# 10XGenomics/thermite

Hardware: AMD Instinct MI355X
Metric: aligned reads/sec (91 bp) (higher is better)
Workload: dtype i32

## Files before the change

### thermite_amd/csrc/aligner.hip

```cpp
#include <hip/hip_runtime.h>

#include <algorithm>
#include <cstdarg>
#include <cstdio>
#include <cstdlib>
#include <cstring>
#include <mutex>
#include <string>
#include <type_traits>
#include <vector>

#include "aligner_internal.h"

namespace thm {
const char* global_error_cstr();
}
using namespace thm;

static int swg_blocks_per_cu() {
  static const int v = [] {
    const char* e = getenv("THM_SWG_BPC");
    const int v = e ? atoi(e) : 4;
    return (v >= 1 && v <= 8) ? v : 4;
  }();
// ... 17 lines not shown
    auto* d = new thm_index::DevCopy();
    d->device = a->device;
    hipStream_t s = a->stream;
    hipError_t e = hipSuccess;
    auto up = [&](auto& buf, const auto& vec) {
      if (e == hipSuccess) e = upload(buf, vec, s);
    };
    d->wide = ix->wide;
    if (e == hipSuccess) e = d->text.ensure(ix->text.size() + 16 + 16);
    if (e == hipSuccess) e = hipMemsetAsync(d->text.p, '$', 16, s);
    if (e == hipSuccess && !ix->text.empty())
      e = hipMemcpyAsync(d->text.as<uint8_t>() + 16, ix->text.data(), ix->text.size(), hipMemcpyHostToDevice, s);
    if (ix->wide) {
      up(d->sa, ix->sa64);
      up(d->lut, ix->lut64);
    } else {
      up(d->sa, ix->sa);
      up(d->lut, ix->lut);
    }
    up(d->refs, ix->refs);
    up(d->name_rank, ix->name_rank);
    up(d->txs, ix->txs);
    up(d->exons, ix->exons);
    up(d->exon_txoff, ix->exon_txoff);
    if (e == hipSuccess) e = d->tx_seq.ensure(ix->tx_seq.size() + 32);
    if (e == hipSuccess) e = hipMemsetAsync(d->tx_seq.p, '$', 16, s);
    if (e == hipSuccess && !ix->tx_seq.empty())
      e = hipMemcpyAsync(d->tx_seq.as<uint8_t>() + 16, ix->tx_seq.data(), ix->tx_seq.size(), hipMemcpyHostToDevice, s);
    up(d->exon_grid_off, ix->exon_grid_off);
    up(d->gene_grid_off, ix->gene_grid_off);
    up(d->ref_bin, ix->ref_bin);
    if (ix->wide)
      up(d->ref_recs, ix->ref_recs64);
    else
      up(d->ref_recs, ix->ref_recs);
    if (ix->wide) {
      up(d->exon_grid, ix->exon_grid64);
      up(d->gene_grid, ix->gene_grid64);
    } else {
      up(d->exon_grid, ix->exon_grid);
      up(d->gene_grid, ix->gene_grid);
    }
    if (e == hipSuccess) e = hipStreamSynchronize(s);
    if (e != hipSuccess) {
      free_dev_copy(d);
      return fail(a, e == hipErrorOutOfMemory ? THM_ERR_OOM : THM_ERR_HIP, "index upload failed: %s",
                  hipGetErrorString(e));
    }
    auto fill_view = [&](auto& v) {
      typedef typename std::remove_reference<decltype(v)>::type::coord_t C;
      v.text = d->text.as<uint8_t>() + 16;
      v.sa = d->sa.as<C>();
      v.lut = d->lut.as<LutEntryT<C>>();
      v.refs = d->refs.as<thm_ref>();
      v.name_rank = d->name_rank.as<uint32_t>();
      v.ref_recs = d->ref_recs.as<RefRecT<C>>();
      v.ref_bin = d->ref_bin.as<uint32_t>();
      v.txs = d->txs.as<thm_tx>();
      v.exons = d->exons.as<thm_exon>();
      v.exon_txoff = d->exon_txoff.as<uint64_t>();
      v.tx_seq = d->tx_seq.as<uint8_t>() + 16;
      v.exon_grid_off = d->exon_grid_off.as<uint32_t>();
      v.exon_grid = d->exon_grid.as<ExonEntryT<C>>();
      v.gene_grid_off = d->gene_grid_off.as<uint32_t>();
      v.gene_grid = d->gene_grid.as<GridEntryT<C>>();
      v.n = ix->n;
      v.n_refs = (uint32_t)ix->refs.size();
      v.n_txs = (uint32_t)ix->txs.size();
      v.kt = ix->kt;
      v.max_tx_exons = ix->max_tx_exons;
    };
    memset(&d->view, 0, sizeof d->view);
    memset(&d->view64, 0, sizeof d->view64);
    if (ix->wide)
      fill_view(d->view64);
    else
      fill_view(d->view);
    ix->dev[a->device] = d;
  }
  a->dix = ix->dev[a->device];
  return THM_OK;
}

int reset_queue(thm_aligner* a) {
  HIPCHK(a, hipMemsetAsync(a->d_queue.p, 0, thm::QUEUE_BYTES, a->stream));
  HIPCHK(a, hipMemsetAsync(a->d_fault.p, 0, 64, a->stream));
  return THM_OK;
}

int grid_blocks(const thm_aligner* a, uint64_t n_items, int waves_per_block, int blocks_per_cu) {
  uint64_t need = (n_items + waves_per_block - 1) / waves_per_block;
  uint64_t cap = (uint64_t)a->n_cu * blocks_per_cu;
  return (int)std::max<uint64_t>(1, std::min(need, cap));
}

extern "C" {

const char* thm_version(void) { return "thermite_amd 0.1 (gfx950)"; }

int32_t thm_device_count(void) {
  int n = 0;
  if (hipGetDeviceCount(&n) != hipSuccess) return 0;
  return n;
}

void thm_index_free(thm_index* ix) {
  if (!ix) return;
  for (auto* d : ix->dev) free_dev_copy(d);
  delete (std::mutex*)ix->dev_mu;
  delete ix;
}

const char* thm_last_error(const thm_aligner* a) { return a ? a->err.c_str() : global_error_cstr(); }

int32_t thm_aligner_create(const thm_index* ix, const thm_align_opts* opts, int32_t device_id, thm_aligner** out) {
  if (!out) return THM_ERR_INVALID_ARG;
  *out = nullptr;
  if (!ix || !opts) return fail(nullptr, THM_ERR_INVALID_ARG, "thm_aligner_create: null index or opts");
  int n = 0;
  if (hipGetDeviceCount(&n) != hipSuccess || n <= 0)
    return fail(nullptr, THM_ERR_NO_DEVICE, "no HIP device visible: the MI355X path has no CPU fallback");
  if (device_id < 0 || device_id >= n) return fail(nullptr, THM_ERR_NO_DEVICE, "device id %d out of range", device_id);
  thm_aligner* a = new thm_aligner();
  a->ix = ix;
  a->device = device_id;
  a->opts = *opts;
  {
    const char* e = getenv("THM_TPR");
    if (e && e[0] == '0') a->use_tpr = false;
    if (e && e[0] == '1') a->use_tpr = true;
    e = getenv("THM_TPR_ROUNDS");
    if (e && atoi(e) >= 1 && atoi(e) <= TPR_MAX_ROUNDS) a->tpr_rounds = atoi(e);
  }
  auto bail = [&](int code) {
    thm_aligner_free(a);
    return code;
  };
  if (hipSetDevice(device_id) != hipSuccess) return bail(fail(nullptr, THM_ERR_HIP, "hipSetDevice failed"));
  hipDeviceProp_t prop;
  if (hipGetDeviceProperties(&prop, device_id) == hipSuccess) a->n_cu = prop.multiProcessorCount;
  if (hipStreamCreateWithFlags(&a->stream, hipStreamNonBlocking) != hipSuccess)
    return bail(fail(nullptr, THM_ERR_HIP, "hipStreamCreate failed"));
  for (auto& e : a->ev)
    if (hipEventCreate(&e) != hipSuccess) return bail(fail(nullptr, THM_ERR_HIP, "hipEventCreate failed"));
  if (hipStreamCreateWithFlags(&a->stream2, hipStreamNonBlocking) != hipSuccess ||
      hipStreamCreateWithFlags(&a->stream3, hipStreamNonBlocking) != hipSuccess ||
      hipStreamCreateWithFlags(&a->stream4, hipStreamNonBlocking) != hipSuccess ||
      hipEventCreateWithFlags(&a->ev_dpt_fork, hipEventDisableTiming) != hipSuccess ||
      hipEventCreateWithFlags(&a->ev_dpt_join, hipEventDisableTiming) != hipSuccess ||
      hipEventCreateWithFlags(&a->ev_join3, hipEventDisableTiming) != hipSuccess ||
      hipEventCreateWithFlags(&a->ev_fork, hipEventDisableTiming) != hipSuccess ||
      hipEventCreateWithFlags(&a->ev_join, hipEventDisableTiming) != hipSuccess)
    return bail(fail(nullptr, THM_ERR_HIP, "second stream / events: creation failed"));
  if (a->d_counters.ensure(THM_N_COUNTERS * 8 * 3) != hipSuccess || a->d_queue.ensure(thm::QUEUE_BYTES) != hipSuccess ||
      a->d_fault.ensure(64) != hipSuccess || a->d_cursors.ensure(64) != hipSuccess)
    return bail(fail(nullptr, THM_ERR_OOM, "scratch allocation failed"));
  (void)hipMemsetAsync(a->d_counters.p, 0, THM_N_COUNTERS * 8 * 3, a->stream);
  int rc = get_dev_copy(a);
  if (rc != THM_OK) return bail(rc);
  rc = thm_aligner_set_opts(a, opts);
  if (rc != THM_OK) return bail(rc);
  *out = a;
  return THM_OK;
}

void thm_aligner_free(thm_aligner* a) {
  if (!a) return;
  (void)hipSetDevice(a->device);
  if (a->stream) (void)hipStreamSynchronize(a->stream);
  if (a->stream2) (void)hipStreamSynchronize(a->stream2);
  if (a->stream3) (void)hipStreamSynchronize(a->stream3);
  if (a->stream4) (void)hipStreamSynchronize(a->stream4);
  DBuf* all[] = {&a->d_counters, &a->d_queue, &a->d_fault, &a->d_cursors, &a->b0, &a->b1, &a->b2, &a->b3, &a->b4,
                 &a->b5, &a->b6, &a->b7, &a->b8, &a->r_bases, &a->r_offsets, &a->r_san, &a->s_ms_end, &a->s_ms_lo, &a->s_ms_hi, &a->s_work_reads, &a->s_work_long, &a->s_work_cells, &a->s_work_counts, &a->s_fill_keys, &a->s_fill_perm, &a->s_fill_hist, &a->s_sel_scratch, &a->s_heavy, &a->s_slow, &a->s_team, &a->r_status, &a->e_slow, &a->e_recs, &a->e_wcnt, &a->t_memos, &a->t_recs, &a->t_dpops, &a->t_qlist, &a->t_act[0], &a->t_act[1], &a->t_ctl, &a->t_bail, &a->t_queue2, &a->t_trace, &a->t_ttrace, &a->t_hdr, &a->t_sums, &a->s_smems, &a->s_off, &a->s_cnt,
                 &a->s_hits, &a->s_cand_off, &a->scan_tmp, &a->e_cands, &a->e_heavy, &a->e_rel, &a->e_order, &a->e_ops, &a->e_nalns,
                 &a->e_nalns64, &a->e_opbytes, &a->e_aln_off, &a->e_ops_off, &a->e_trace, &a->o_alns, &a->o_ops, &a->o_mems,
                 &a->sh_bases, &a->sh_san, &a->sh_off, &a->sh_hits, &a->sh_read, &a->sh_bw, &a->sh_xd, &a->sh_list, &a->sh_out,
                 &a->sh_status, &a->sh_ops, &a->sh_ctl, &a->sh_trace, &a->sh_slow, &a->c_sums, &a->c_nwords, &a->c_woff,
                 &a->c_scan_tmp, &a->c_flags, &a->c_dig, &a->c_words, &a->c_in_ops, &a->c_in_off,
                 &a->bn_names, &a->bn_name_off, &a->bn_quals, &a->bt_tx_pool, &a->bt_tx_off, &a->bt_gid_pool, &a->bt_gid_off,
                 &a->bt_gname_pool, &a->bt_gname_off, &a->bt_tx_gene, &a->bt_ref_sq, &a->bm_cnt, &a->bm_first, &a->bm_qn,
                 &a->bm_rec_read, &a->bm_len, &a->bm_off, &a->bm_out, &a->bm_read_off, &a->bm_err, &a->bm_scan_tmp};
  for (DBuf* b : all) b->release();
  for (int k = 0; k < 2; k++) {
    a->r_off[k].release();
    a->r_alns[k].release();
    a->r_ops[k].release();
    a->r_stat[k].release();
    a->ch_off[k].release();
    a->ch_alns[k].release();
    a->ch_dig[k].release();
    a->ch_words[k].release();
    a->ch_stat[k].release();
    a->bh_data[k].release();
    a->bh_off[k].release();
    a->bh_stat[k].release();
  }
  for (auto& e : a->ev_cig)
    if (e) (void)hipEventDestroy(e);
  for (auto& e : a->ev_bam)
    if (e) (void)hipEventDestroy(e);
  for (auto& e : a->ev)
    if (e) (void)hipEventDestroy(e);
  if (a->ev_fork) (void)hipEventDestroy(a->ev_fork);
  if (a->ev_join) (void)hipEventDestroy(a->ev_join);
  if (a->ev_join3) (void)hipEventDestroy(a->ev_join3);
  if (a->ev_dpt_fork) (void)hipEventDestroy(a->ev_dpt_fork);
  if (a->ev_dpt_join) (void)hipEventDestroy(a->ev_dpt_join);
  if (a->stream4) (void)hipStreamDestroy(a->stream4);
  if (a->stream3) (void)hipStreamDestroy(a->stream3);
  if (a->stream2) (void)hipStreamDestroy(a->stream2);
  if (a->stream) (void)hipStreamDestroy(a->stream);
  delete a;
}

int32_t thm_aligner_set_opts(thm_aligner* a, const thm_align_opts* o) {
  if (!a || !o) return THM_ERR_INVALID_ARG;
  if (o->min_seed_len < 1 || o->min_seed_len > 65535) return fail(a, THM_ERR_INVALID_ARG, "min_seed_len out of range");
  if (!(o->min_aln_score_percent >= 0.0f && o->min_aln_score_percent <= 1.0f))
    return fail(a, THM_ERR_INVALID_ARG, "min_aln_score_percent must be within [0,1] (src/main.rs:46-49)");
  a->opts = *o;
  return THM_OK;
}

void* thm_aligner_stream(thm_aligner* a) { return a ? (void*)a->stream : nullptr; }

const thm_index* thm_aligner_index(const thm_aligner* a) { return a ? a->ix : nullptr; }

int32_t thm_counters_get(thm_aligner* a, uint64_t out[THM_N_COUNTERS]) {
  if (!a || !out) return THM_ERR_INVALID_ARG;
  HIPCHK(a, hipSetDevice(a->device));
  HIPCHK(a, hipMemcpyAsync(out, a->d_counters.p, THM_N_COUNTERS * 8, hipMemcpyDeviceToHost, a->stream));
  HIPCHK(a, hipStreamSynchronize(a->stream));
  return THM_OK;
}
int32_t thm_counters_reset(thm_aligner* a) {
  if (!a) return THM_ERR_INVALID_ARG;
  HIPCHK(a, hipSetDevice(a->device));
  HIPCHK(a, hipMemsetAsync(a->d_counters.p, 0, THM_N_COUNTERS * 8, a->stream));
  return THM_OK;
}
void* thm_counters_device_ptr(thm_aligner* a) { return a ? a->d_counters.p : nullptr; }

int32_t thm_timings_get(thm_aligner* a, float out[THM_N_TIMINGS]) {
  if (!a || !out) return THM_ERR_INVALID_ARG;
  memcpy(out, a->timings, sizeof(a->timings));
  return THM_OK;
}

int32_t thm_swg_extend_batch(thm_aligner* a, const uint8_t* x_bases, const uint64_t* x_off, const uint8_t* y_bases,
                             const uint64_t* y_off, const uint32_t* band_width, const int32_t* x_drop,
                             uint32_t max_band_width, uint64_t n, thm_swg_view* out) {
  if (!a || !out || !x_off || !y_off || !band_width || !x_drop) return THM_ERR_INVALID_ARG;
  memset(out, 0, sizeof(*out));
  if (n == 0) return THM_OK;
  if (n >= 0xFFFFFFFFull) return fail(a, THM_ERR_UNSUPPORTED, "more than 2^32-1 problems in one call");
  HIPCHK(a, hipSetDevice(a->device));
  uint32_t bw_max = 0, x_max = 0, y_max = 0;
  std::vector<uint64_t> ops_off(n + 1, 0);
  for (uint64_t i = 0; i < n; i++) {
    if (band_width[i] > max_band_width)
      return fail(a, THM_ERR_OUT_OF_CONTRACT, "problem %llu: band_width %u > max_band_width %u (src/swg.rs:32)",
                  (unsigned long long)i, band_width[i], max_band_width);
    if (x_drop[i] < (int64_t)band_width[i])
      return fail(a, THM_ERR_OUT_OF_CONTRACT, "problem %llu: x_drop < band_width is undefined in the reference",
                  (unsigned long long)i);
    uint64_t xl = x_off[i + 1] - x_off[i], yl = y_off[i + 1] - y_off[i];
    if (x_off[i + 1] < x_off[i] || y_off[i + 1] < y_off[i]) return fail(a, THM_ERR_INVALID_ARG, "offsets not monotone");
    if (xl > MAX_READ_LEN || band_width[i] > 2 * MAX_READ_LEN)
      return fail(a, THM_ERR_UNSUPPORTED, "x longer than %u or band wider than +-%u", MAX_READ_LEN, 2 * MAX_READ_LEN);
    uint64_t cols = std::min<uint64_t>(yl, xl + band_width[i] + 1);
    bw_max = std::max(bw_max, band_width[i]);
    x_max = std::max<uint32_t>(x_max, (uint32_t)xl);
    y_max = std::max<uint32_t>(y_max, (uint32_t)cols);
    ops_off[i + 1] = ops_off[i] + xl + cols + 8;
  }
  int cpl = (int)((2 * bw_max + 1 + 63) / 64);
  SwgBatchParams p;
  p.x_cap = (x_max + 15u) & ~15u;
  p.y_cap = (y_max + 15u) & ~15u;
  if (p.x_cap == 0) p.x_cap = 16;
  if (p.y_cap == 0) p.y_cap = 16;
  p.max_bw = bw_max;
  p.scratch = nullptr;
  p.scratch_per_wave = 0;
  if (cpl > 4 || swg_batch_lds_bytes(p, cpl) > EXTEND_LDS_LIMIT) cpl = 0;
  const uint64_t xb_n = x_off[n], yb_n = y_off[n], pool = ops_off[n];
  HIPCHK(a, a->b0.ensure(xb_n + 16));
  HIPCHK(a, a->b1.ensure((n + 1) * 8));
  HIPCHK(a, a->b2.ensure(yb_n + 16));
  HIPCHK(a, a->b3.ensure((n + 1) * 8));
  HIPCHK(a, a->b4.ensure(n * 4));
  HIPCHK(a, a->b5.ensure(n * 4));
  HIPCHK(a, a->b6.ensure((n + 1) * 8));
  HIPCHK(a, a->b7.ensure(pool + 16));
  HIPCHK(a, a->b8.ensure(n * sizeof(thm_swg_aln)));
  hipStream_t s = a->stream;
  if (xb_n) HIPCHK(a, hipMemcpyAsync(a->b0.p, x_bases, xb_n, hipMemcpyHostToDevice, s));
  HIPCHK(a, hipMemcpyAsync(a->b1.p, x_off, (n + 1) * 8, hipMemcpyHostToDevice, s));
  if (yb_n) HIPCHK(a, hipMemcpyAsync(a->b2.p, y_bases, yb_n, hipMemcpyHostToDevice, s));
  HIPCHK(a, hipMemcpyAsync(a->b3.p, y_off, (n + 1) * 8, hipMemcpyHostToDevice, s));
  HIPCHK(a, hipMemcpyAsync(a->b4.p, band_width, n * 4, hipMemcpyHostToDevice, s));
  HIPCHK(a, hipMemcpyAsync(a->b5.p, x_drop, n * 4, hipMemcpyHostToDevice, s));
  HIPCHK(a, hipMemcpyAsync(a->b6.p, ops_off.data(), (n + 1) * 8, hipMemcpyHostToDevice, s));
  int rc = reset_queue(a);
  if (rc != THM_OK) return rc;
  p.xb = a->b0.as<uint8_t>();
  p.xo = a->b1.as<uint64_t>();
  p.yb = a->b2.as<uint8_t>();
  p.yo = a->b3.as<uint64_t>();
  p.bw = a->b4.as<uint32_t>();
  p.xd = a->b5.as<int32_t>();
  p.ops_off = a->b6.as<uint64_t>();
  p.ops = a->b7.as<uint8_t>();
  p.out = a->b8.as<thm_swg_aln>();
  p.counters = a->d_counters.as<unsigned long long>();
  p.queue = a->d_queue.as<unsigned int>();
  p.fault = a->d_fault.as<int>();
  p.n = n;
  const int bpc = swg_blocks_per_cu();
  int n_blocks = grid_blocks(a, n, 4, bpc);
  if (cpl == 0) {
    p.scratch_per_wave = (swg_batch_scratch_bytes(p) + 255) & ~255ull;
    const uint64_t budget = 16ull << 30;
    if (p.scratch_per_wave > budget) return fail(a, THM_ERR_UNSUPPORTED, "DP trace of %llu bytes per problem exceeds the device-memory budget",
                                                 (unsigned long long)p.scratch_per_wave);
    n_blocks = (int)std::max<uint64_t>(1, std::min<uint64_t>((uint64_t)n_blocks, budget / p.scratch_per_wave / 4));
    HIPCHK(a, a->e_slow.ensure((size_t)n_blocks * 4 * p.scratch_per_wave + 256));
    p.scratch = a->e_slow.as<uint8_t>();
// ... 245 lines not shown
```

### thermite_amd/csrc/aligner_internal.h

```cpp
#ifndef THERMITE_ALIGNER_INTERNAL_H
#define THERMITE_ALIGNER_INTERNAL_H
#include <hip/hip_runtime.h>

#include <cstdarg>
#include <cstdio>
#include <string>
#include <vector>

#include "launch.h"
#include "thermite_internal.h"

struct DBuf {
  void* p = nullptr;
  size_t cap = 0;
  hipError_t ensure(size_t bytes) {
    if (bytes <= cap) return hipSuccess;
    if (p) (void)hipFree(p);
    p = nullptr;
    cap = 0;
    size_t want = bytes + bytes / 4 + 256;
    hipError_t e = hipMalloc(&p, want);
    if (e == hipSuccess) cap = want;
    return e;
  }
  void release() {
    if (p) (void)hipFree(p);
    p = nullptr;
    cap = 0;
  }
  template <class T>
  T* as() const {
    return (T*)p;
  }
};

struct HBuf {
  void* p = nullptr;
  size_t cap = 0;
  hipError_t ensure(size_t bytes) {
    if (bytes <= cap) return hipSuccess;
    if (p) (void)hipHostFree(p);
    p = nullptr;
    cap = 0;
    size_t want = bytes + bytes / 4 + 4096;
    hipError_t e = hipHostMalloc(&p, want, hipHostMallocDefault);
    if (e == hipSuccess) cap = want;
    return e;
  }
  void release() {
    if (p) (void)hipHostFree(p);
    p = nullptr;
    cap = 0;
  }
  template <class T>
  T* as() const {
    return (T*)p;
  }
};

struct thm_index::DevCopy {
  int device = -1;
  DBuf text, sa, lut, refs, name_rank, ref_recs, ref_bin, txs, exons, exon_txoff, tx_seq, exon_grid_off, exon_grid, gene_grid_off, gene_grid;
  bool wide = false;
  thm::DeviceIndexT<uint32_t> view;
  thm::DeviceIndexT<uint64_t> view64;
};

inline void free_dev_copy(thm_index::DevCopy* d) {
  if (!d) return;
  int cur = 0;
  (void)hipGetDevice(&cur);
  (void)hipSetDevice(d->device);
  DBuf* all[] = {&d->text, &d->sa,         &d->lut,    &d->refs,      &d->name_rank, &d->ref_recs, &d->ref_bin, &d->txs,
                 &d->exons, &d->exon_txoff, &d->tx_seq, &d->exon_grid_off, &d->exon_grid, &d->gene_grid_off, &d->gene_grid};
  for (DBuf* b : all) b->release();
  (void)hipSetDevice(cur);
  delete d;
}

struct thm_aligner {
  const thm_index* ix = nullptr;
  thm_index::DevCopy* dix = nullptr;
  int device = 0;
  int n_cu = 256;
  hipStream_t stream = nullptr;
  hipStream_t stream2 = nullptr;
  hipStream_t stream3 = nullptr;
  hipEvent_t ev_join3 = nullptr;
  hipStream_t stream4 = nullptr;
  hipEvent_t ev_dpt_fork = nullptr, ev_dpt_join = nullptr;
  hipEvent_t ev_fork = nullptr, ev_join = nullptr;
  thm_align_opts opts;
  std::string err;

  DBuf d_counters, d_queue, d_fault, d_cursors;
  DBuf b0, b1, b2, b3, b4, b5, b6, b7, b8;

  DBuf r_bases, r_offsets, r_san;
  DBuf r_status;
  uint64_t n_reads = 0, n_bases = 0;
  uint32_t max_read_len = 0;
  std::vector<std::pair<uint32_t, uint64_t>> len_hist;
  uint64_t n_over = 0;
  bool uploaded = false;
  DBuf s_smems, s_off, s_cnt, s_hits, s_cand_off, scan_tmp, s_ms_end, s_ms_lo, s_ms_hi, s_work_reads, s_work_long, s_work_cells,
      s_work_counts, s_sel_scratch, s_heavy, s_slow, s_team, s_fill_keys, s_fill_perm, s_fill_hist;
  uint64_t smem_cap = 0;
  DBuf e_heavy, e_rel;
  DBuf e_cands, e_order, e_ops, e_nalns, e_nalns64, e_opbytes, e_aln_off, e_ops_off, e_trace, e_slow, e_recs, e_wcnt;
  DBuf t_memos, t_recs, t_dpops, t_qlist, t_act[2], t_ctl, t_bail, t_queue2, t_trace, t_ttrace, t_hdr, t_sums;
  bool use_tpr = false;
  int tpr_rounds = 8;
  uint64_t n_slow_host = 0;
  uint32_t fast_max_len = 0, slow_max_len = 0;
  uint64_t cand_cap = 0, cand_ops_cap = 0;
  DBuf o_alns, o_ops, o_mems;
  uint64_t out_alns_cap = 0, out_ops_cap = 0;
  uint64_t dbg_smem_cap = 0, dbg_cand_cap = 0, dbg_ops_cap = 0;
  uint32_t dbg_band_clip = 0;
  bool dbg_seed_noinfer = false, dbg_seed_stats = false;
  uint32_t n_replays = 0;
  bool ran = false, synced = false;
  hipEvent_t ev[6] = {nullptr, nullptr, nullptr, nullptr, nullptr, nullptr};
  float timings[THM_N_TIMINGS] = {0};

  HBuf r_off[2], r_alns[2], r_ops[2], r_stat[2];
  int r_cur = 0;
  std::vector<uint64_t> h_off;
  std::vector<thm_aln> h_alns;
  std::vector<uint8_t> h_ops;
  std::vector<thm_mem> h_mems;
  std::vector<thm_swg_aln> h_swg;
  std::vector<thm_lr_aln> h_lr;
  DBuf sh_bases, sh_san, sh_off, sh_hits, sh_read, sh_bw, sh_xd, sh_list, sh_out, sh_status, sh_ops, sh_ctl, sh_trace, sh_slow;
  std::vector<thm_aln> h_hit_alns;
  std::vector<int32_t> h_hit_status;
  std::vector<uint8_t> h_hit_ops;
  DBuf c_sums, c_nwords, c_woff, c_scan_tmp, c_flags, c_dig, c_words, c_in_ops, c_in_off;
  HBuf ch_off[2], ch_alns[2], ch_dig[2], ch_words[2], ch_stat[2];
  int c_cur = 0;
  hipEvent_t ev_cig[4] = {nullptr, nullptr, nullptr, nullptr};
  std::vector<thm_aln_digest> h_cig_dig;
  std::vector<uint32_t> h_cig_words;
  DBuf bn_names, bn_name_off, bn_quals;
  bool reads_named = false, reads_have_quals = false;
  DBuf bt_tx_pool, bt_tx_off, bt_gid_pool, bt_gid_off, bt_gname_pool, bt_gname_off, bt_tx_gene, bt_ref_sq;
  bool bam_tables = false;
  DBuf bm_cnt, bm_first, bm_qn, bm_rec_read, bm_len, bm_off, bm_out, bm_read_off, bm_err, bm_scan_tmp;
  HBuf bh_data[2], bh_off[2], bh_stat[2];
  int b_cur = 0;
  int bam_stage = -1;
  hipEvent_t ev_bam[4] = {nullptr, nullptr, nullptr, nullptr};
};

inline int fail(thm_aligner* a, int code, const char* fmt, ...) {
  char buf[512];
  va_list ap;
  va_start(ap, fmt);
  vsnprintf(buf, sizeof buf, fmt, ap);
  va_end(ap);
  if (a) a->err = buf;
  thm::set_global_error(buf);
  return code;
}

#define HIPCHK(a, call)                                                                             \
  do {                                                                                              \
    hipError_t e_ = (call);                                                                         \
    if (e_ != hipSuccess)                                                                           \
      return fail(a, e_ == hipErrorOutOfMemory ? THM_ERR_OOM : THM_ERR_HIP, "%s failed: %s (%s:%d)", \
                  #call, hipGetErrorString(e_), __FILE__, __LINE__);                                \
  } while (0)

int run_cigar_passes(thm_aligner* a, thm::CigarParams p, uint64_t n_digests, uint64_t* n_words, unsigned* any_flags);
int cigar_ensure_events(thm_aligner* a);
int reset_queue(thm_aligner* a);
int grid_blocks(const thm_aligner* a, uint64_t n_items, int waves_per_block, int blocks_per_cu);
uint32_t seed_fill_mode();
unsigned team_div_per_cu();
#endif
```

### thermite_amd/csrc/kernels_extend.hip

```cpp
#include <hip/hip_runtime.h>

#include <cstdlib>

#include "launch.h"
#include "swg_device.h"

namespace thm {
namespace dev {

enum : int { FAULT_OPS_POOL = 1, FAULT_INTERNAL = 2, FAULT_CONTRACT = 4, FAULT_RETRY = 8, FAULT_BAND = 16 };

template <class C>
struct CoordTraits {
  typedef int S;
};
template <>
struct CoordTraits<uint64_t> {
  typedef long long S;
};
__device__ __forceinline__ uint32_t readlane_c(uint32_t v, int l) { return (uint32_t)__builtin_amdgcn_readlane((int)v, l); }
__device__ __forceinline__ uint64_t readlane_c(uint64_t v, int l) {
  return ((uint64_t)(unsigned)__builtin_amdgcn_readlane((int)(v >> 32), l) << 32) | (unsigned)__builtin_amdgcn_readlane((int)(v & 0xffffffffu), l);
}

// ... 1413 lines not shown
              less = b.ystart < a.ystart;
            else
              less = u < t;
            rank += less ? 1u : 0u;
          }
          lb[rank] = la[t];
        }
      }
      step();
      if (lead) {
      uint64_t max_end = 0;
      uint32_t l_rank = 0, l_strand = 0;
      int l_score = 0;
      uint64_t l_yend = 0;
      for (uint32_t s = 0; s < m; s++) {
        const uint32_t ci = (uint32_t)bcast_first((int)lb[s]);
        const Cand a = cands[ci];
        if (nres == 0 || a.ystart >= max_end || a.name_rank != l_rank || a.strand != l_strand) {
          max_end = a.yend;
          if (lane == 0) la[nres] = ci;
          nres++;
          l_rank = a.name_rank;
          l_strand = a.strand;
          l_score = a.score;
          l_yend = a.yend;
        } else {
          if (a.score > l_score) {
            if (lane == 0) la[nres - 1] = ci;
            l_score = a.score;
            l_yend = a.yend;
          }
          max_end = max(max_end, l_yend);
        }
      }
      if (TM && lane == 0) t_ctl[1] = nres;
      }
      step();
      if constexpr (TM) nres = t_ctl[1];
      #pragma unroll 1
      for (uint32_t t0 = t0_first; t0 < nres; t0 += t0_step) {
        const uint32_t t = t0 + lane;
        if (t < nres) {
          const int sa_ = cands[la[t]].score;
          uint32_t rank = 0;
          for (uint32_t u = 0; u < nres; u++) {
            const int sb = cands[la[u]].score;
            rank += (sb > sa_ || (sb == sa_ && u < t)) ? 1u : 0u;
          }
          lb[rank] = la[t];
        }
      }
      step();
      #pragma unroll 1
      for (uint32_t t = t0_first + lane; t < nres; t += t0_step) la[t] = lb[t];
      step();
    }
      #pragma unroll 1
      for (uint32_t t0 = 0; lead && t0 < nres; t0 += 64) {
        const uint32_t t = t0 + (uint32_t)lane;
        int ty = -1;
        if (t < nres) {
          const Cand a = cands[la[t]];
          opb += a.ops_len + a.tx_ops_len;
          ty = a.aln_type;
        }
        k_type[0] += (unsigned)__popcll(__ballot(ty == THM_ALN_EXONIC));
        k_type[1] += (unsigned)__popcll(__ballot(ty == THM_ALN_INTRONIC));
        k_type[2] += (unsigned)__popcll(__ballot(ty == THM_ALN_INTERGENIC));
      }
      for (int o = 32; o > 0; o >>= 1) opb += __shfl_xor(opb, o);
    }
#ifdef THM_PROF_FINAL
    const unsigned long long tf2 = __builtin_amdgcn_s_memtime();
#endif
    if (lead && lane == 0) {
      p.read_n_alns[idx] = nres;
      p.read_op_bytes[idx] = opb;
    }
#ifdef THM_PROF_FINAL
    {
      const unsigned long long tf3 = __builtin_amdgcn_s_memtime();
      c.prof_cols[3] += tf1 - tf0;
      c.prof_cols[4] += tf2 - tf1;
      c.prof_cols[5] += tf3 - tf2;
      c.prof_cols[1] += (n_acc > 1) ? 1 : 0;
      c.prof_cols[2] += 1;
    }
#endif
    PROF_MARK(c, PS_FINAL);
    if (lead) {
      k_reads++;
      if (nres)
        k_aligned++;
      else
        k_unmapped++;
      k_alns += nres;
      k_opb += opb;
    }
    k_cells += c.cells;
    k_cols += c.cols;
    k_calls += c.calls;
    k_win += c.winbytes;
    c.cells = c.cols = c.calls = c.winbytes = 0;
    wsync(c);
  }
#ifdef THM_TIMELINE
  if (!TM && !GS && lane == 0 && p.prof && tl_reads) {
    const unsigned long long tl_end = __builtin_amdgcn_s_memrealtime();
    atomicMax(&p.prof[0], ~tl_start);
    atomicMax(&p.prof[1], ~tl_end);
    atomicMax(&p.prof[2], tl_end);
    atomicMax(&p.prof[3], (tl_end << 20) | min((tl_end - tl_last) / 100ull, 1048575ull));
    tl_close(tl_end);
    atomicMax(&p.prof[4], tl_longest);
    atomicAdd(&p.prof[5], 1ull);
    atomicAdd(&p.prof[6], tl_end - tl_start);
    atomicAdd(&p.prof[7], (unsigned long long)tl_reads);
    if (p.list_only == 0) {
      const unsigned long long t0 = ~atomicMax(&p.prof[0], 0ull);
      const unsigned long long rel = (tl_end - t0) / 10000ull;
      const int b = rel < 30 ? 0 : (int)min(rel - 29ull, 7ull);
      atomicAdd(&p.prof[8 + b], 1ull);
    }
  }
#endif
#ifdef THM_PROF
  if (lane == 0 && p.prof)
    {
      for (int t = 0; t < 10; t++) atomicAdd(&p.prof[t], c.prof_acc[t]);
      for (int t = 0; t < 6; t++) atomicAdd(&p.prof[10 + t], c.prof_cols[t]);
    }
#endif
  batch_fault |= c.fault & (FAULT_OPS_POOL | FAULT_INTERNAL);
  if (lane == 0) {
    if (batch_fault) atomicOr(p.fault, batch_fault & (FAULT_OPS_POOL | FAULT_INTERNAL));
    if (k_reads | k_calls | k_cells | k_win) {
      unsigned long long* row = p.wave_counters + (size_t)wave_global * THM_N_COUNTERS;
      row[THM_CNT_READS] = k_reads;
      row[THM_CNT_ALIGNED] = k_aligned;
      row[THM_CNT_UNMAPPED] = k_unmapped;
      row[THM_CNT_ALNS] = k_alns;
      row[THM_CNT_EXONIC] = (unsigned long long)k_type[0];
      row[THM_CNT_INTRONIC] = (unsigned long long)k_type[1];
      row[THM_CNT_INTERGENIC] = (unsigned long long)k_type[2];
      row[THM_CNT_SWG_CALLS] = k_calls;
      row[THM_CNT_DP_CELLS] = k_cells;
      row[THM_CNT_DP_COLS] = k_cols;
      row[THM_CNT_OP_BYTES] = k_opb;
      row[THM_CNT_WINDOW_BYTES] = k_win;
    }
  }
}

__global__ __launch_bounds__(1024) void counters_reduce_kernel(const unsigned long long* rows, uint32_t n_rows, unsigned long long* counters) {
  __shared__ unsigned long long part[64][THM_N_COUNTERS];
  static_assert(THM_N_COUNTERS == 16, "one thread per counter and row group");
  const int k = (int)(threadIdx.x & 15u), g = (int)(threadIdx.x >> 4);
  unsigned long long sum = 0;
  for (uint32_t r = (uint32_t)g; r < n_rows; r += 64) sum += rows[(size_t)r * THM_N_COUNTERS + k];
  part[g][k] = sum;
  __syncthreads();
  if (g == 0) {
    unsigned long long t = 0;
    for (int i = 0; i < 64; i++) t += part[i][k];
    if (t) counters[k] += t;
  }
}

constexpr uint32_t COMPACT_HEAVY_N = 8, COMPACT_CHUNK = 4;

struct CandRegs {
  uint32_t lo, hi;
};
static_assert(sizeof(Cand) == 112 && sizeof(thm_aln) == 112, "compact_emit permutes the dwords of these layouts");
static_assert(offsetof(Cand, ops_off) == 48 && offsetof(Cand, tx_ops_off) == 56 && offsetof(Cand, score) == 64 &&
                  offsetof(Cand, ops_len) == 80 && offsetof(Cand, tx_ops_len) == 84 && offsetof(Cand, strand) == 108 &&
                  offsetof(thm_aln, ops_off) == 24 && offsetof(thm_aln, tx_ops_off) == 56 && offsetof(thm_aln, xlen) == 80 &&
                  offsetof(thm_aln, ops_len) == 84 && offsetof(thm_aln, tx_ops_len) == 104 && offsetof(thm_aln, strand) == 108,
              "compact_emit permutes the dwords of these layouts");

__device__ __forceinline__ CandRegs cand_load(const Cand* c, int sub) {
  const uint32_t* w = reinterpret_cast<const uint32_t*>(c);
  CandRegs r;
  r.lo = w[sub];
  r.hi = sub < 12 ? w[16 + sub] : 0u;
  return r;
}

__device__ __forceinline__ uint32_t compact_emit(const CompactParams& p, const CandRegs c, uint64_t ai, uint64_t o, uint32_t xlen, bool primary, int sub) {
  const uint64_t ops_off = (uint64_t)__shfl(c.lo, 12, 16) | ((uint64_t)__shfl(c.lo, 13, 16) << 32);
  const uint64_t tx_ops_off = (uint64_t)__shfl(c.lo, 14, 16) | ((uint64_t)__shfl(c.lo, 15, 16) << 32);
  const uint32_t ops_len = __shfl(c.hi, 4, 16), tx_ops_len = __shfl(c.hi, 5, 16), flags = __shfl(c.hi, 11, 16);
  if (ai >= p.alns_cap || o + ops_len + tx_ops_len > p.ops_cap) return ops_len + tx_ops_len;
  auto copy_ops = [&](const uint8_t* src, uint8_t* dst, uint32_t len) {
    #pragma unroll 1
    for (uint32_t b0 = 0; b0 < len; b0 += 64) {
      uint8_t v[4];
      #pragma unroll
      for (int k = 0; k < 4; k++) {
        const uint32_t b = b0 + (uint32_t)sub + 16u * (uint32_t)k;
        v[k] = (b < len) ? src[b] : (uint8_t)0;
      }
      #pragma unroll
      for (int k = 0; k < 4; k++) {
        const uint32_t b = b0 + (uint32_t)sub + 16u * (uint32_t)k;
        if (b < len) dst[b] = v[k];
      }
    }
  };
  copy_ops(p.cand_ops + ops_off, p.ops + o, ops_len);
  const uint64_t go = o, to = o + ops_len;
  copy_ops(p.cand_ops + tx_ops_off, p.ops + to, tx_ops_len);
  const int src_lo = (int)((0x00BA987600543210ull >> (4 * sub)) & 15u);
  const int src_hi = (int)((0x0000B59876403210ull >> (4 * sub)) & 15u);
  uint32_t w0 = __shfl(c.lo, src_lo, 16), w1 = __shfl(c.hi, src_hi, 16);
  const uint64_t txo = ((flags >> 8) & 0xFFu) == THM_ALN_EXONIC ? to : 0ull;
  if (sub == 6) w0 = (uint32_t)go;
  if (sub == 7) w0 = (uint32_t)(go >> 32);
  if (sub == 14) w0 = (uint32_t)txo;
  if (sub == 15) w0 = (uint32_t)(txo >> 32);
  if (sub == 4) w1 = xlen;
  if (sub == 11) w1 = (flags & 0xFFu) | ((primary ? 1u : 0u) << 8) | (((flags >> 8) & 0xFFu) << 16);
  uint32_t* out = reinterpret_cast<uint32_t*>(p.alns + ai);
  out[sub] = w0;
  if (sub < 12) out[16 + sub] = w1;
  return ops_len + tx_ops_len;
}

__device__ __forceinline__ bool compact_faulted(const CompactParams& p) { return p.fault[0] != 0 || (p.fault[1] & FAULT_OPS_POOL) != 0; }

template <int K>
__global__ __launch_bounds__(256) void compact_kernel(CompactParams p) {
  const int sub = (int)(threadIdx.x & 15u);
  if (compact_faulted(p)) return;
  const uint64_t n_groups = (uint64_t)gridDim.x * 16, g = ((uint64_t)blockIdx.x * 256 + threadIdx.x) >> 4;
  for (uint64_t rb = g; rb < p.n_reads; rb += (uint64_t)K * n_groups) {
    uint32_t n[K], xlen[K], l0[K];
    uint64_t cand0[K], a0[K], o[K];
    #pragma unroll
    for (int k = 0; k < K; k++) {
      const uint64_t r = rb + (uint64_t)k * n_groups;
      n[k] = r < p.n_reads ? p.read_n_alns[r] : 0u;
    }
    #pragma unroll
    for (int k = 0; k < K; k++) {
      const uint64_t r = rb + (uint64_t)k * n_groups;
      if (n[k] > COMPACT_HEAVY_N) {
        if (sub == 0) {
          const unsigned long long h = atomicAdd(&p.heavy_cnt[0], 1ull);
          if (h < p.heavy_cap) p.heavy_list[h] = r;
        }
        n[k] = 0;
      }
      if (n[k]) {
        cand0[k] = p.read_cand_off[r];
        a0[k] = p.read_aln_off[r];
        o[k] = p.read_ops_off[r];
        xlen[k] = (uint32_t)(p.read_offsets[r + 1] - p.read_offsets[r]);
      }
    }
    #pragma unroll
    for (int k = 0; k < K; k++)
      if (n[k]) l0[k] = p.order[2 * cand0[k]];
    CandRegs cd[K];
    #pragma unroll
    for (int k = 0; k < K; k++)
      if (n[k]) cd[k] = cand_load(p.cands + cand0[k] + l0[k], sub);
    #pragma unroll
    for (int k = 0; k < K; k++) {
      if (!n[k]) continue;
      uint64_t ok = o[k] + compact_emit(p, cd[k], a0[k], o[k], xlen[k], true, sub);
      const uint32_t* la = p.order + 2 * cand0[k];
      for (uint32_t t = 1; t < n[k]; t++)
        ok += compact_emit(p, cand_load(p.cands + cand0[k] + la[t], sub), a0[k] + t, ok, xlen[k], false, sub);
    }
  }
}

__global__ __launch_bounds__(256) void compact_heavy_scan_kernel(CompactParams p) {
  __shared__ uint32_t wave_sum[4];
  __shared__ unsigned long long desc_base;
  if (compact_faulted(p)) return;
  const uint64_t H = min((unsigned long long)p.heavy_cap, p.heavy_cnt[0]);
  const int tid = (int)threadIdx.x, lane = tid & 63, wv = tid >> 6;
  for (uint64_t h = blockIdx.x; h < H; h += gridDim.x) {
    const uint64_t r = p.heavy_list[h];
    const uint32_t n = p.read_n_alns[r];
    const uint64_t cand0 = p.read_cand_off[r], a0 = p.read_aln_off[r];
    const Cand* cands = p.cands + cand0;
    const uint32_t* la = p.order + 2 * cand0;
    uint32_t carry = 0;
    for (uint32_t tile = 0; tile < n; tile += 256) {
      const uint32_t t = tile + (uint32_t)tid;
      uint32_t len = 0;
      if (t < n) {
        const Cand* cd = &cands[la[t]];
        len = cd->ops_len + cd->tx_ops_len;
      }
      uint32_t inc = len;
      #pragma unroll
      for (int o = 1; o < 64; o <<= 1) {
        const uint32_t v = __shfl_up(inc, o);
        if (lane >= o) inc += v;
      }
      if (lane == 63) wave_sum[wv] = inc;
      __syncthreads();
      uint32_t before = carry, total = 0;
      #pragma unroll
      for (int k = 0; k < 4; k++) {
        if (k < wv) before += wave_sum[k];
        total += wave_sum[k];
      }
      if (t < n && a0 + t < p.alns_cap) p.rel[a0 + t] = before + inc - len;
      carry += total;
      __syncthreads();
    }
    const uint32_t nd = (n + COMPACT_CHUNK - 1) / COMPACT_CHUNK;
    if (tid == 0) desc_base = atomicAdd(&p.heavy_cnt[1], (unsigned long long)nd);
// ... 324 lines not shown
      atomicAdd(&p.counters[THM_CNT_SWG_CALLS], k_calls);
      atomicAdd(&p.counters[THM_CNT_DP_CELLS], k_cells);
      atomicAdd(&p.counters[THM_CNT_DP_COLS], k_cols);
      atomicAdd(&p.counters[THM_CNT_OP_BYTES], k_opb);
      atomicAdd(&p.counters[THM_CNT_WINDOW_BYTES], k_win);
    }
  }
}

}

template <class C>
static hipError_t launch_seed_hits_t(const SeedHitParamsT<C>& p, int cpl, int n_blocks, hipStream_t s) {
  const size_t lds = cpl == 0 ? 0 : extend_lds_bytes(p.max_read_len, p.max_bw, cpl);
  auto go = [&](auto kern) -> hipError_t {
    if (lds > 48 * 1024) {
      hipError_t e = hipFuncSetAttribute((const void*)kern, hipFuncAttributeMaxDynamicSharedMemorySize, (int)lds);
      if (e != hipSuccess) return e;
    }
    hipLaunchKernelGGL(kern, dim3(n_blocks), dim3(256), lds, s, p);
    return hipGetLastError();
  };
  switch (cpl) {
    case 0: return go(dev::seed_hit_kernel<C, 0>);
    case 1: return go(dev::seed_hit_kernel<C, 1>);
    case 2: return go(dev::seed_hit_kernel<C, 2>);
    case 3: return go(dev::seed_hit_kernel<C, 3>);
    case 4: return go(dev::seed_hit_kernel<C, 4>);
    default: return hipErrorInvalidValue;
  }
}
hipError_t launch_seed_hits(const SeedHitParamsT<uint32_t>& p, int cpl, int n_blocks, hipStream_t s) { return launch_seed_hits_t(p, cpl, n_blocks, s); }
hipError_t launch_seed_hits(const SeedHitParamsT<uint64_t>& p, int cpl, int n_blocks, hipStream_t s) { return launch_seed_hits_t(p, cpl, n_blocks, s); }

size_t extend_lds_bytes(uint32_t max_read_len, uint32_t max_bw, int cpl) {
  const dev::ExtCaps k = dev::ext_caps(max_read_len, max_bw, cpl);
  const uint32_t per_wave = k.lcap + 2u * k.wcap + k.trb + 3u * k.opcap + 8u * FAST_MAX_YCLIPS + (uint32_t)(dev::KEYCAP * sizeof(dev::CandKey));
  return 4 * (size_t)per_wave;
}

size_t extend_trace_scratch_bytes(uint32_t max_read_len, uint32_t max_bw, int cpl) {
  return cpl > 1 ? (size_t)(max_read_len + max_bw + 3u) * (size_t)cpl * 16u : 0;
}

size_t extend_slow_scratch_bytes(uint32_t max_read_len, uint32_t max_bw, uint32_t mk_cap) {
  return (size_t)dev::slow_layout(max_read_len, max_bw, mk_cap).total;
}

constexpr int EXT_MINW_CPL34 = 4;
static int ext_minw_env() {
  static const int v = [] {
    const char* e = getenv("THM_EXT_MINW");
    const int v = e ? atoi(e) : 0;
    return (v >= 4 && v <= 8) ? v : 0;
  }();
  return v;
}
static int ext_minw_cpl3_env() {
  static const int v = [] {
    const char* e = getenv("THM_EXT_MINW_CPL3");
    const int v = e ? atoi(e) : 0;
    return (v >= 3 && v <= 6) ? v : 0;
  }();
  return v;
}
static int ext_minw_wide_env() {
  static const int v = [] {
    const char* e = getenv("THM_EXT_MINW_WIDE");
    const int v = e ? atoi(e) : 0;
    return (v == 4 || v == 5) ? v : 0;
  }();
  return v;
}
int extend_waves_per_simd(int cpl, bool wide) {
  const int minw_env = ext_minw_env();
  if (cpl == 0) return 2;
  if (cpl > 2) {
    const int v34 = ext_minw_cpl3_env();
    return (v34 && !wide) ? v34 : EXT_MINW_CPL34;
  }
  if (wide) {
    const int wide_env = ext_minw_wide_env();
    return wide_env ? wide_env : 5;
  }
  if (minw_env) {
    if (cpl == 1) return (minw_env == 4 || minw_env == 5 || minw_env == 6) ? minw_env : 8;
    return (minw_env == 4 || minw_env == 5 || minw_env == 8) ? minw_env : 6;
  }
  return cpl == 1 ? 6 : 5;
}

template <class C>
static hipError_t launch_extend_t(const ExtendParamsT<C>& p, int cpl, int n_blocks, hipStream_t s, bool team) {
  const size_t lds4 = cpl == 0 ? 0 : extend_lds_bytes(p.max_read_len, p.max_bw, cpl);
  const size_t lds = team ? lds4 / 4 * TEAM_WAVES : lds4;
  const unsigned threads = team ? 64u * TEAM_WAVES : 256u;
  auto go = [&](auto kern) -> hipError_t {
    if (lds > 48 * 1024) {
      hipError_t e = hipFuncSetAttribute((const void*)kern, hipFuncAttributeMaxDynamicSharedMemorySize, (int)lds);
      if (e != hipSuccess) return e;
    }
    hipLaunchKernelGGL(kern, dim3(n_blocks), dim3(threads), lds, s, p);
    return hipGetLastError();
  };
  if (team) {
    if (cpl == 1) return go(dev::extend_kernel<C, 1, 4, TEAM_WAVES>);
    if (cpl == 2) return go(dev::extend_kernel<C, 2, 4, TEAM_WAVES>);
    return hipErrorInvalidValue;
  }
  if (cpl == 0) return go(dev::extend_kernel<C, 0, 2>);
  if constexpr (sizeof(C) == 8) {
    const int minw = extend_waves_per_simd(cpl, true);
    switch (cpl) {
      case 1: return minw == 5 ? go(dev::extend_kernel<C, 1, 5>) : go(dev::extend_kernel<C, 1, 4>);
      case 2: return minw == 5 ? go(dev::extend_kernel<C, 2, 5>) : go(dev::extend_kernel<C, 2, 4>);
      case 3: return go(dev::extend_kernel<C, 3, 4>);
      case 4: return go(dev::extend_kernel<C, 4, 4>);
      default: return hipErrorInvalidValue;
    }
  } else {
    const int minw = extend_waves_per_simd(cpl, false);
    switch (cpl) {
      case 1:
        if (minw == 4) return go(dev::extend_kernel<C, 1, 4>);
        if (minw == 5) return go(dev::extend_kernel<C, 1, 5>);
        if (minw == 6) return go(dev::extend_kernel<C, 1, 6>);
        return go(dev::extend_kernel<C, 1, 8>);
      case 2:
        if (minw == 4) return go(dev::extend_kernel<C, 2, 4>);
        if (minw == 5) return go(dev::extend_kernel<C, 2, 5>);
        if (minw == 8) return go(dev::extend_kernel<C, 2, 8>);
        return go(dev::extend_kernel<C, 2, 6>);
      case 3:
      case 4: {
        const int minw = extend_waves_per_simd(cpl, false);
        if (cpl == 3) {
          if (minw == 3) return go(dev::extend_kernel<C, 3, 3>);
          if (minw == 5) return go(dev::extend_kernel<C, 3, 5>);
          if (minw == 6) return go(dev::extend_kernel<C, 3, 6>);
          return go(dev::extend_kernel<C, 3, 4>);
        }
        if (minw == 3) return go(dev::extend_kernel<C, 4, 3>);
        if (minw == 5) return go(dev::extend_kernel<C, 4, 5>);
        if (minw == 6) return go(dev::extend_kernel<C, 4, 6>);
        return go(dev::extend_kernel<C, 4, 4>);
      }
      default: return hipErrorInvalidValue;
    }
  }
}
hipError_t launch_extend(const ExtendParamsT<uint32_t>& p, int cpl, int n_blocks, hipStream_t s, bool team) { return launch_extend_t(p, cpl, n_blocks, s, team); }
hipError_t launch_extend(const ExtendParamsT<uint64_t>& p, int cpl, int n_blocks, hipStream_t s, bool team) { return launch_extend_t(p, cpl, n_blocks, s, team); }

hipError_t launch_counters_reduce(const unsigned long long* wave_counters, uint32_t n_rows, unsigned long long* counters, hipStream_t s) {
  if (n_rows == 0) return hipSuccess;
  hipLaunchKernelGGL(dev::counters_reduce_kernel, dim3(1), dim3(1024), 0, s, wave_counters, n_rows, counters);
  return hipGetLastError();
}

int compact_k() {
  static const int v = [] {
    const char* e = getenv("THM_COMPACT_K");
    const int v = e ? atoi(e) : 2;
    return v == 1 || v == 2 || v == 4 ? v : 2;
  }();
  return v;
}

hipError_t launch_compact(const CompactParams& p, hipStream_t s) {
  static const unsigned n_cu = [] {
    int dev = 0, cu = 256;
    if (hipGetDevice(&dev) == hipSuccess) (void)hipDeviceGetAttribute(&cu, hipDeviceAttributeMultiprocessorCount, dev);
    return (unsigned)cu;
  }();
  const unsigned blocks = (unsigned)std::min<uint64_t>((p.n_reads + 15) / 16, (uint64_t)n_cu * 8);
  if (blocks == 0) return hipSuccess;
  const int k_reads = compact_k();
  if (k_reads == 1)
    hipLaunchKernelGGL(dev::compact_kernel<1>, dim3(blocks), dim3(256), 0, s, p);
  else if (k_reads == 2)
    hipLaunchKernelGGL(dev::compact_kernel<2>, dim3(blocks), dim3(256), 0, s, p);
  else
    hipLaunchKernelGGL(dev::compact_kernel<4>, dim3(blocks), dim3(256), 0, s, p);
  hipLaunchKernelGGL(dev::compact_heavy_scan_kernel, dim3(n_cu), dim3(256), 0, s, p);
  hipLaunchKernelGGL(dev::compact_heavy_copy_kernel, dim3(n_cu * 4), dim3(256), 0, s, p);
  return hipGetLastError();
}

}
```

### thermite_amd/csrc/kernels_seed.hip

```cpp
#include <hip/hip_runtime.h>

#include <algorithm>

#include "launch.h"
#include "swg_device.h"

namespace thm {
namespace dev {

__device__ __forceinline__ int base_code(uint8_t c) {
  return c == 'A' ? 0 : c == 'C' ? 1 : c == 'G' ? 2 : c == 'T' ? 3 : -1;
}
__device__ __forceinline__ uint8_t sanitize_base(uint8_t c) {
  if (c >= 'a' && c <= 'z') c = (uint8_t)(c - 32);
  return (c == 'A' || c == 'C' || c == 'G' || c == 'T' || c == 'N') ? c : (uint8_t)0;
}
__device__ __forceinline__ uint64_t load8_global(const uint8_t* p) {
  uint64_t v;
  __builtin_memcpy(&v, p, 8);
  return v;
}
__device__ __forceinline__ uint64_t load8_lds(const uint8_t* base16, int off) {
  const uint64_t* q = (const uint64_t*)(base16 + (off & ~7));
  const unsigned sh = (unsigned)(off & 7) * 8u;
// ... 16 lines not shown
      }
      return cap;
    }
    o = 8;
  }
  while (o < cap) {
    uint64_t tw[8];
#pragma unroll
    for (int u = 0; u < 8; u++) tw[u] = load8_global(tp + o + 8 * u);
#pragma unroll
    for (int u = 0; u < 8; u++) {
      const int oo = o + 8 * u;
      if (oo < cap) {
        const uint64_t qw = load8_global(q + oo);
        const uint64_t x = tw[u] ^ qw;
        if (x) {
          const int idx = __builtin_ctzll(x) >> 3;
          if (oo + idx < cap) {
            *less = ((tw[u] >> (8 * idx)) & 0xff) < ((qw >> (8 * idx)) & 0xff);
            return oo + idx;
          }
          return cap;
        }
      }
    }
    o += 64;
  }
  return cap;
}

template <class C>
__device__ bool ms_search(const DeviceIndexT<C>& ix, const uint8_t* rd, int L, int pos, int k, int known_end, int& out_d, C& out_lo,
                          C& out_hi) {
  C lo = 0, hi = (C)ix.n;
  int d = 0;
  const int kt = (int)ix.kt;
  if (kt <= k) {
    uint32_t code = 0;
    bool acgt = true;
    const uint64_t w0 = load8_global(rd + pos), w1 = load8_global(rd + pos + 8);
    for (int t = 0; t < kt; t++) {
      const int c = base_code((uint8_t)((t < 8 ? (w0 >> (8 * t)) : (w1 >> (8 * (t - 8)))) & 0xff));
      acgt = acgt && (c >= 0);
      code = (code << 2) | (uint32_t)(c & 3);
    }
    if (acgt) {
      const LutEntryT<C> e = ix.lut[code];
      lo = e.lo;
      hi = e.hi;
      d = kt;
      if (known_end != 0 && hi - lo == 1 && pos + kt <= known_end) {
        out_d = known_end - pos;
        out_lo = lo;
        out_hi = hi;
        return true;
      }
    }
  }
  if (lo < hi && pos + d < L) {
    const int cap = L - (pos + d);
    const uint8_t* q = rd + pos + d;
    bool less;
    const C sz = hi - lo;
    if (sz == 1) {
      d += lcp_cmp<false>(ix.text + ix.sa[lo] + d, q, cap, &less);
    } else if (q[0] != 0) {
      if (sz <= 8) {
        C sav[8];
        uint64_t tw[8];
        int lc[8];
#pragma unroll
        for (int u = 0; u < 8; u++) sav[u] = (lo + u < hi) ? ix.sa[lo + u] : (C)0;
#pragma unroll
        for (int u = 0; u < 8; u++) tw[u] = load8_global(ix.text + sav[u] + d);
        const uint64_t qw = load8_global(q);
        int ms = 0;
#pragma unroll
        for (int u = 0; u < 8; u++) {
          const uint64_t x = tw[u] ^ qw;
          int l = x ? (__builtin_ctzll(x) >> 3) : 8;
          l = min(l, cap);
          if (lo + u >= hi) l = -1;
          lc[u] = l;
        }
#pragma unroll
        for (int u = 0; u < 8; u++) {
          if (lc[u] == 8 && cap > 8) lc[u] = 8 + lcp_cmp<false>(ix.text + sav[u] + d + 8, q + 8, cap - 8, &less);
          ms = max(ms, lc[u]);
        }
        if (ms > 0) {
          C nlo = hi, nhi = lo;
#pragma unroll
          for (int u = 0; u < 8; u++) {
            if (lc[u] == ms) {
              nlo = min(nlo, (C)(lo + u));
              nhi = max(nhi, (C)(lo + u + 1));
            }
          }
          lo = nlo;
          hi = nhi;
          d += ms;
        }
      } else {
        C a = lo, b = hi;
        while (a < b) {
          const C m = a + ((b - a) >> 1);
          (void)lcp_cmp<true>(ix.text + ix.sa[m] + d, q, cap, &less);
          if (less)
            a = m + 1;
          else
            b = m;
        }
        int l1 = -1, l2 = -1;
        if (a > lo) l1 = lcp_cmp<true>(ix.text + ix.sa[a - 1] + d, q, cap, &less);
        if (a < hi) l2 = lcp_cmp<true>(ix.text + ix.sa[a] + d, q, cap, &less);
        const int ms = max(l1, l2);
        if (ms > 0) {
          C nlo = a, nhi = a;
          if (l1 >= ms) {
            C x = lo, y = a - 1;
            while (x < y) {
              const C m = x + ((y - x) >> 1);
              if (lcp_cmp<true>(ix.text + ix.sa[m] + d, q, ms, &less) >= ms)
                y = m;
              else
                x = m + 1;
            }
            nlo = x;
          }
          if (l2 >= ms) {
            C x = a + 1, y = hi;
            while (x < y) {
              const C m = x + ((y - x) >> 1);
              if (lcp_cmp<true>(ix.text + ix.sa[m] + d, q, ms, &less) >= ms)
                x = m + 1;
              else
                y = m;
            }
            nhi = x;
          }
          lo = nlo;
          hi = nhi;
          d += ms;
        }
      }
    }
  }
  out_d = (lo < hi) ? d : 0;
  out_lo = lo;
  out_hi = hi;
  return false;
}

__global__ void sanitize_kernel(const uint8_t* in, uint8_t* out, uint64_t n, uint64_t n_padded) {
  const uint64_t i = ((uint64_t)blockIdx.x * blockDim.x + threadIdx.x) * 16;
  if (i >= n_padded) return;
  uint4 v = make_uint4(0, 0, 0, 0);
  if (i < n) v = *(const uint4*)(in + i);
  uint32_t w[4] = {v.x, v.y, v.z, v.w};
#pragma unroll
  for (int j = 0; j < 4; j++) {
    uint32_t r = 0;
#pragma unroll
    for (int b = 0; b < 4; b++) {
      const uint64_t at = i + (uint64_t)(4 * j + b);
      const uint8_t c = (at < n) ? sanitize_base((uint8_t)(w[j] >> (8 * b))) : (uint8_t)0;
      r |= (uint32_t)c << (8 * b);
    }
    w[j] = r;
  }
  *(uint4*)(out + i) = make_uint4(w[0], w[1], w[2], w[3]);
}

constexpr int PROBE_STRIDE = 8;

__device__ __forceinline__ void block_append(bool flag, unsigned long long value, unsigned long long* list,
                                             unsigned long long* count) {
  __shared__ unsigned w_cnt[4];
  __shared__ unsigned long long b_base;
  const unsigned long long m = __ballot(flag);
  const int lane = lane_id(), wv = (int)(threadIdx.x >> 6);
  if (lane == 0) w_cnt[wv] = (unsigned)__popcll(m);
  __syncthreads();
  if (threadIdx.x == 0) {
    const unsigned total = w_cnt[0] + w_cnt[1] + w_cnt[2] + w_cnt[3];
    b_base = total ? atomicAdd(count, (unsigned long long)total) : 0ull;
  }
  __syncthreads();
  unsigned before = 0;
  for (int w = 0; w < wv; w++) before += w_cnt[w];
  if (flag) list[b_base + before + (unsigned long long)__popcll(m & ((1ull << lane) - 1ull))] = value;
  __syncthreads();
}

__device__ __forceinline__ unsigned* seed_stats_lds() {
  __shared__ unsigned s_cnt[2];
  return s_cnt;
}
__device__ __forceinline__ void seed_stats_begin() {
  unsigned* c = seed_stats_lds();
  if (threadIdx.x == 0) c[0] = c[1] = 0;
  __syncthreads();
}
__device__ __forceinline__ void seed_stats_note(bool decided) {
  const unsigned long long here = __ballot(1), dec = __ballot(decided);
  if (lane_id() == (int)__builtin_ctzll(here)) {
    unsigned* c = seed_stats_lds();
    if (dec) atomicAdd(&c[0], (unsigned)__popcll(dec));
    if (here & ~dec) atomicAdd(&c[1], (unsigned)__popcll(here & ~dec));
  }
}
template <class C>
__device__ __forceinline__ void seed_stats_end(const SeedParamsT<C>& p) {
  unsigned* c = seed_stats_lds();
  __syncthreads();
  if (threadIdx.x == 0) {
    if (c[0]) atomicAdd(&p.work_counts[8], (unsigned long long)c[0]);
    if (c[1]) atomicAdd(&p.work_counts[9], (unsigned long long)c[1]);
  }
}

template <class C>
__device__ __forceinline__ int probe_store(const SeedParamsT<C>& p, const uint8_t* rd, int L, int pos, uint64_t item0, int hint,
                                           bool& decided) {
  const int k = (int)p.min_seed_len;
  int d = 0;
  C lo = 0, hi = 0;
  decided = ms_search(p.ix, rd, L, pos, k, hint, d, lo, hi);
  if (p.flags & SEED_STATS) seed_stats_note(decided);
  const int e = (d >= k) ? pos + d : 0;
  const uint64_t item = item0 + (uint64_t)pos;
  p.ms_end[item] = (uint16_t)e;
  if (hint == 0 || e > hint) {
    p.ms_lo[item] = lo;
    p.ms_hi[item] = hi;
  }
  return e;
}

template <class C>
__global__ __launch_bounds__(256) void seed_first_kernel(SeedParamsT<C> p) {
  const uint64_t read = (uint64_t)blockIdx.x * 256 + threadIdx.x;
  const int lane = lane_id();
  const bool active = read < p.reads.n_reads;
  const int k = (int)p.min_seed_len;
  if (p.flags & SEED_STATS) seed_stats_begin();
  int d = 0, L = 0;
  C lo = 0, hi = 0;
  bool too_long = false;
  if (active) {
    const uint64_t r0 = p.reads.offsets[read];
    const uint64_t Lfull = p.reads.offsets[read + 1] - r0;
    too_long = Lfull > MAX_READ_LEN;
    L = too_long ? 0 : (int)Lfull;
    if (too_long) p.read_status[read] = THM_ERR_UNSUPPORTED;
    if (k <= L) (void)ms_search(p.ix, p.reads.bases + r0, L, 0, k, 0, d, lo, hi);
    if (L > 0) {
      const uint64_t item = ms_row(r0, read);
      p.ms_end[item] = (uint16_t)((d >= k) ? d : 0);
      p.ms_lo[item] = lo;
      p.ms_hi[item] = hi;
    }
  }
  if (p.flags & SEED_STATS) {
    if (active && k <= L) seed_stats_note(false);
    seed_stats_end(p);
  }
  const bool covered = active && d >= k && d == L;
  const bool more = active && !covered && L - k + 1 >= 1;
  block_append(more && L <= (int)SHORT_READ_MAX, read, p.work_short, &p.work_counts[0]);
  block_append(more && L > (int)SHORT_READ_MAX, read, p.work_long, &p.work_counts[4]);
  if (active && !covered && !more) {
    p.read_smem_off[read] = 0;
    p.read_smem_cnt[read] = 0;
    p.read_hits[read] = 0;
  }
  const unsigned long long m = __ballot(covered);
  if (m) {
    const int leader = (int)__builtin_ctzll(m);
    unsigned long long base = 0;
    if (lane == leader) base = atomicAdd(p.cursor, (unsigned long long)__popcll(m));
    base = ((unsigned long long)(unsigned)__shfl((int)(base >> 32), leader) << 32) | (unsigned)__shfl((int)(base & 0xffffffffu), leader);
    const bool fits = base + (unsigned long long)__popcll(m) <= p.smem_cap;
    unsigned long long hits = 0;
    if (covered) {
      const unsigned long long slot = base + (unsigned long long)__popcll(m & ((1ull << lane) - 1ull));
      if (fits) {
        SmemT<C> sm;
        sm.lo = lo;
        sm.hi = hi;
        sm.qpos = 0;
        sm.len = (uint16_t)L;
        p.smems[slot] = sm;
      }
      hits = (unsigned long long)(hi - lo);
      p.read_smem_off[read] = slot;
      p.read_smem_cnt[read] = 1u;
      p.read_hits[read] = hits;
    }
    for (int o = 32; o > 0; o >>= 1) hits += __shfl_xor(hits, o);
    if (lane == leader) {
      if (!fits) atomicExch(p.fault, 1);
      atomicAdd(&p.counters[THM_CNT_SMEMS], (unsigned long long)__popcll(m));
      atomicAdd(&p.counters[THM_CNT_HITS], hits);
    }
  }
}

template <class C>
__global__ __launch_bounds__(256) void seed_grid_kernel(SeedParamsT<C> p, const unsigned long long* list,
                                                        const unsigned long long* count, uint32_t G) {
  const uint64_t tid = (uint64_t)blockIdx.x * 256 + threadIdx.x;
  const uint64_t wi = tid / G;
  if (p.flags & SEED_STATS) seed_stats_begin();
  if (wi < *count) {
    const uint64_t read = list[wi];
    const int g = (int)(tid - wi * G);
    const uint64_t r0 = p.reads.offsets[read];
    const int L = (int)(p.reads.offsets[read + 1] - r0);
    const int k = (int)p.min_seed_len;
    const int npos = L - k + 1;
    const int pos = (g + 1 == (int)G) ? npos - 1 : g * PROBE_STRIDE;
    if (!(pos <= 0 || pos >= npos || (g + 1 != (int)G && pos == npos - 1))) {
      const uint64_t item0 = ms_row(r0, read);
// ... 334 lines not shown
    for (int t0 = 0; t0 < n_sm; t0 += 64) {
      const int t = t0 + lane;
      if (t < n_sm) {
        const int len = s_len[t], em = s_em[t];
        int rank = 0;
        for (int u = 0; u < n_sm; u++) {
          const int lu = s_len[u], eu = s_em[u];
          rank += (lu > len || (lu == len && eu > em)) ? 1 : 0;
        }
        if (fits) {
          SmemT<C> sm;
          sm.lo = s_lo[t];
          sm.hi = s_hi[t];
          sm.qpos = s_pos[t];
          sm.len = (uint16_t)len;
          p.smems[base_out + rank] = sm;
        }
        hits += (unsigned long long)(s_hi[t] - s_lo[t]);
      }
    }
    for (int o = 32; o > 0; o >>= 1) hits += __shfl_xor(hits, o);
    if (lane == 0) {
      if (!fits) atomicExch(p.fault, 1);
      p.read_smem_off[idx] = base_out;
      p.read_smem_cnt[idx] = (uint32_t)n_sm;
      p.read_hits[idx] = hits;
    }
    c_smems += (unsigned long long)n_sm;
    c_hits += hits;
    sync();
  }
  if (lane == 0 && (c_smems | c_hits)) {
    atomicAdd(&p.counters[THM_CNT_SMEMS], c_smems);
    atomicAdd(&p.counters[THM_CNT_HITS], c_hits);
  }
}

constexpr int SEL_CAP = 6;

template <class C>
__global__ __launch_bounds__(256) void seed_select_thread_kernel(SeedParamsT<C> p, unsigned long long* over_list,
                                                                 unsigned long long* over_count) {
  extern __shared__ __attribute__((aligned(16))) uint8_t smem[];
  const unsigned T = blockDim.x, tid = threadIdx.x;
  C* l_lo = (C*)smem;
  C* l_hi = l_lo + (size_t)SEL_CAP * T;
  uint32_t* l_pl = (uint32_t*)(l_hi + (size_t)SEL_CAP * T);
  const int lane = lane_id();
  const uint64_t wi = (uint64_t)blockIdx.x * T + tid;
  const bool active = wi < p.work_counts[0];
  const int k = (int)p.min_seed_len;
  int n_sm = 0;
  bool overflow = false;
  uint64_t read = 0;
  if (active) {
    read = p.work_short[wi];
    const uint64_t r0 = p.reads.offsets[read];
    const int L = (int)(p.reads.offsets[read + 1] - r0);
    const int npos = max(L - k + 1, 0);
    const uint64_t item0 = ms_row(r0, read);
    int prev = 0;
    const uint4* row = (const uint4*)(p.ms_end + item0);
    for (int c0 = 0; c0 < npos; c0 += 8) {
      const uint4 v = row[c0 >> 3];
      const uint32_t w[4] = {v.x, v.y, v.z, v.w};
#pragma unroll
      for (int j = 0; j < 8; j++) {
        const int pos = c0 + j;
        const int e = (int)((w[j >> 1] >> (16 * (j & 1))) & 0xffffu);
        if (pos < npos && e > 0 && e > prev) {
          if (n_sm < SEL_CAP) {
            l_lo[(size_t)n_sm * T + tid] = p.ms_lo[item0 + (uint64_t)pos];
            l_hi[(size_t)n_sm * T + tid] = p.ms_hi[item0 + (uint64_t)pos];
            l_pl[(size_t)n_sm * T + tid] = (uint32_t)pos | ((uint32_t)(e - pos) << 8);
          } else {
            overflow = true;
          }
          n_sm++;
        }
        prev = e;
      }
    }
    if (overflow) n_sm = 0;
  }
  block_append(overflow, read, over_list, over_count);

  if (n_sm > 1) {
    int t = 0, em = 0, i0 = 0;
    while (t < n_sm) {
      const int st = (int)(l_pl[(size_t)t * T + tid] & 0xffu);
      if (st > i0) i0 = st;
      int u = t;
      while (u < n_sm && (int)(l_pl[(size_t)u * T + tid] & 0xffu) <= i0) u++;
      for (int v = u - 1; v >= t; v--) l_pl[(size_t)v * T + tid] |= (uint32_t)(em + (u - 1 - v)) << 16;
      em += u - t;
      const uint32_t z = l_pl[(size_t)(u - 1) * T + tid];
      i0 = (int)(z & 0xffu) + (int)((z >> 8) & 0xffu);
      t = u;
    }
  }
  int incl = n_sm;
  for (int o = 1; o < 64; o <<= 1) {
    const int v = __shfl_up(incl, o);
    if (lane >= o) incl += v;
  }
  const int total = __shfl(incl, 63);
  unsigned long long base = 0;
  if (total > 0) {
    if (lane == 0) base = atomicAdd(p.cursor, (unsigned long long)total);
    base = ((unsigned long long)(unsigned)bcast_first((int)(base >> 32)) << 32) | (unsigned)bcast_first((int)(base & 0xffffffffu));
  }
  const bool fits = base + (unsigned long long)total <= p.smem_cap;
  const unsigned long long mine = base + (unsigned long long)(incl - n_sm);
  unsigned long long hits = 0;
  for (int t = 0; t < n_sm; t++) {
    const uint32_t a = l_pl[(size_t)t * T + tid];
    const int len = (int)((a >> 8) & 0xffu), em = (int)(a >> 16);
    int rank = 0;
    for (int u = 0; u < n_sm; u++) {
      const uint32_t b = l_pl[(size_t)u * T + tid];
      const int lu = (int)((b >> 8) & 0xffu), eu = (int)(b >> 16);
      rank += (lu > len || (lu == len && eu > em)) ? 1 : 0;
    }
    const C slo = l_lo[(size_t)t * T + tid], shi = l_hi[(size_t)t * T + tid];
    if (fits) {
      SmemT<C> sm;
      sm.lo = slo;
      sm.hi = shi;
      sm.qpos = (uint16_t)(a & 0xffu);
      sm.len = (uint16_t)len;
      p.smems[mine + rank] = sm;
    }
    hits += (unsigned long long)(shi - slo);
  }
  if (active && !overflow) {
    p.read_smem_off[read] = mine;
    p.read_smem_cnt[read] = (uint32_t)n_sm;
    p.read_hits[read] = hits;
  }
  int fault = (total > 0 && !fits) ? 1 : 0;
  for (int o = 32; o > 0; o >>= 1) {
    hits += __shfl_xor(hits, o);
    fault |= __shfl_xor(fault, o);
  }
  if (lane == 0) {
    if (fault) atomicExch(p.fault, 1);
    if (total > 0) {
      atomicAdd(&p.counters[THM_CNT_SMEMS], (unsigned long long)total);
      atomicAdd(&p.counters[THM_CNT_HITS], hits);
    }
  }
}

__global__ __launch_bounds__(256) void plan_kernel(PlanParams p) {
  const uint64_t r = (uint64_t)blockIdx.x * 256 + threadIdx.x;
  const bool active = r < p.n_reads;
  uint64_t L = 0, hits = 0;
  if (active) {
    L = p.offsets[r + 1] - p.offsets[r];
    hits = p.read_hits[r];
  }
  const bool fast = active && L <= p.fast_max_len;
  const bool slow = active && !fast && L <= p.slow_max_len;
  if (active && !fast && !slow) {
    p.read_status[r] = THM_ERR_UNSUPPORTED;
    p.read_n_alns[r] = 0;
    p.read_op_bytes[r] = 0;
  }
  const uint64_t team_thr = p.tpr_max_hits ? (uint64_t)max(p.tpr_max_hits, TEAM_MIN_HITS)
                                           : min((uint64_t)TEAM_HITS, max((uint64_t)TEAM_MIN_HITS, *p.total_hits / max(p.team_div, 1u)));
  const bool team = fast && p.team_ok && hits >= team_thr && hits <= TEAM_MAX_HITS;
  block_append(fast && !team && hits >= (p.tpr_max_hits ? (uint64_t)p.tpr_max_hits : (uint64_t)HEAVY_HITS), r, p.heavy, &p.counts[2]);
  block_append(slow, r, p.slow, &p.counts[5]);
  block_append(team, r, p.team, &p.counts[7]);
}

template <class C>
__global__ __launch_bounds__(256) void pack_reads_kernel(PackParamsT<C> p) {
  const uint64_t r = (uint64_t)blockIdx.x * 256 + threadIdx.x;
  if (r >= p.n_reads) return;
  ReadRecT<C> rec;
  const uint64_t b0 = p.offsets[r], L = p.offsets[r + 1] - b0;
  rec.base_off = b0;
  rec.len = L > 0xFFFFFFFEull ? 0xFFFFFFFFu : (uint32_t)L;
  rec.smem_off = p.read_smem_off[r];
  rec.smem_cnt = p.read_smem_cnt[r];
  const uint64_t c0 = p.read_cand_off[r], nh = p.read_cand_off[r + 1] - c0;
  rec.cand_off = c0;
  rec.n_hits = nh > 0xFFFFFFFFull ? 0xFFFFFFFFu : (uint32_t)nh;
  rec.qpos0 = rec.len0 = 0;
  rec.lo0 = rec.hi0 = rec.sa0 = 0;
  if (rec.smem_cnt > 0 && *p.fault_seed == 0) {
    const SmemT<C> sm = p.smems[rec.smem_off];
    rec.qpos0 = sm.qpos;
    rec.len0 = sm.len;
    rec.lo0 = sm.lo;
    rec.hi0 = sm.hi;
    if (sm.hi > sm.lo) rec.sa0 = p.sa[sm.hi - 1];
  }
  p.recs[r] = rec;
}

template <class C>
__global__ __launch_bounds__(256) void expand_kernel(ExpandParamsT<C> p) {
  const int lane = lane_id();
  const uint64_t r = (uint64_t)blockIdx.x * 4 + (threadIdx.x >> 6);
  if (r >= p.n_reads) return;
  const uint64_t s0 = p.read_smem_off[r];
  const uint32_t ns = p.read_smem_cnt[r];
  uint64_t out = p.read_mem_off[r];
  for (uint32_t s = 0; s < ns; s++) {
    const SmemT<C> sm = p.smems[s0 + s];
    const uint64_t cnt = (uint64_t)(sm.hi - sm.lo);
    for (uint64_t t = lane; t < cnt; t += 64) {
      thm_mem m;
      m.ref_idx = p.ix.sa[sm.hi - 1 - t];
      m.query_idx = sm.qpos;
      m.len = sm.len;
      p.mems[out + t] = m;
    }
    out += cnt;
  }
}

}

static uint32_t sel_lcap(uint32_t max_read_len) { return (max_read_len + 31u) & ~15u; }
size_t seed_select_scratch_bytes(uint32_t max_read_len) { return (size_t)sel_lcap(max_read_len) * (2 * 8 + 8); }
size_t seed_select_lds_bytes(uint32_t max_read_len) { return 4 * seed_select_scratch_bytes(max_read_len); }

hipError_t launch_sanitize(const uint8_t* in, uint8_t* out, uint64_t n, uint64_t n_padded, hipStream_t s) {
  if (n_padded == 0) return hipSuccess;
  hipLaunchKernelGGL(dev::sanitize_kernel, dim3((unsigned)((n_padded / 16 + 255) / 256 + 1)), dim3(256), 0, s, in, out, n, n_padded);
  return hipGetLastError();
}

template <class C>
static hipError_t launch_seed_t(const SeedParamsT<C>& p, int n_blocks, hipStream_t s) {
  const uint64_t n = p.reads.n_reads;
  if (n == 0) return hipSuccess;
  const uint32_t k = p.min_seed_len;
  auto blocks = [](uint64_t threads) { return dim3((unsigned)((threads + 255) / 256)); };
  auto cells_of = [&](uint32_t max_len) -> uint64_t {
    const uint32_t P = (max_len >= k) ? max_len - k + 1 : 1;
    return (P + dev::PROBE_STRIDE - 1) / dev::PROBE_STRIDE;
  };
  hipError_t e;
  hipLaunchKernelGGL(dev::seed_first_kernel<C>, blocks(n), dim3(256), 0, s, p);
  if ((e = hipGetLastError()) != hipSuccess) return e;
  const uint64_t n_short = n - p.n_long;
  struct Cls {
    uint64_t n;
    uint32_t max_len;
    const unsigned long long* list;
    const unsigned long long* count;
    bool fused;
  } cls[2] = {{n_short, p.max_len_short, p.work_short, p.work_counts + 0, true},
              {p.n_long, p.max_len_long, p.work_long, p.work_counts + 4, false}};
  uint64_t fill_cells = 0;
  for (const Cls& c : cls) {
    if (c.n == 0 || c.max_len < k + 1) continue;
    const uint64_t NC = cells_of(c.max_len), G = NC + 1;
    if (c.fused && G <= 256) {
      const uint64_t per = 256 / G;
      hipLaunchKernelGGL(dev::seed_grid_cells_kernel<C>, dim3((unsigned)((c.n + per - 1) / per)), dim3(256), 0, s, p, c.list, c.count,
                         (uint32_t)G);
      if ((e = hipGetLastError()) != hipSuccess) return e;
    } else {
      hipLaunchKernelGGL(dev::seed_grid_kernel<C>, blocks(c.n * G), dim3(256), 0, s, p, c.list, c.count, (uint32_t)G);
      if ((e = hipGetLastError()) != hipSuccess) return e;
      hipLaunchKernelGGL(dev::seed_cells_kernel<C>, blocks(c.n * NC), dim3(256), 0, s, p, c.list, c.count, (uint32_t)NC);
      if ((e = hipGetLastError()) != hipSuccess) return e;
    }
    fill_cells += c.n * NC;
  }
  if (fill_cells) {
    const dim3 worst = blocks(fill_cells * dev::PROBE_STRIDE);
    const dim3 fixed(std::min<unsigned>(worst.x, 256u * 8u * 4u));
    if (p.fill_mode == 2 && fill_cells * dev::PROBE_STRIDE < (1ull << 32)) {
      hipLaunchKernelGGL(dev::seed_fill_keys_kernel<C>, fixed, dim3(256), 0, s, p);
      hipLaunchKernelGGL(dev::seed_fill_scan_kernel, dim3(1), dim3(1024), 0, s, p.fill_hist);
      hipLaunchKernelGGL(dev::seed_fill_scatter_kernel<C>, fixed, dim3(256), 0, s, p);
      hipLaunchKernelGGL(dev::seed_fill_bucketed_kernel<C>, fixed, dim3(256), 0, s, p);
    } else {
      hipLaunchKernelGGL(dev::seed_fill_kernel<C>, p.fill_mode == 1 ? fixed : worst, dim3(256), 0, s, p);
    }
    if ((e = hipGetLastError()) != hipSuccess) return e;
  }
  auto select_waves = [&](const unsigned long long* list, const unsigned long long* count, unsigned int* queue, uint32_t max_len,
                          int nb) -> hipError_t {
    const uint32_t lcap = sel_lcap(max_len);
    const size_t lds = 4 * (size_t)lcap * (2 * sizeof(C) + 8);
    if (lds <= SEED_SELECT_LDS_LIMIT) {
      hipLaunchKernelGGL((dev::seed_select_kernel<C, false>), dim3(nb), dim3(256), lds, s, p, list, count, queue, lcap);
    } else {
      hipLaunchKernelGGL((dev::seed_select_kernel<C, true>), dim3(nb), dim3(256), 0, s, p, list, count, queue, lcap);
    }
    return hipGetLastError();
  };
  if (n_short) {
    unsigned long long* over_list = p.work_cells;
    unsigned long long* over_count = p.work_counts + 3;
    hipLaunchKernelGGL(dev::seed_select_thread_kernel<C>, dim3((unsigned)((n_short + 255) / 256)), dim3(256),
                       (size_t)256 * (2 * sizeof(C) + 4) * dev::SEL_CAP, s, p, over_list, over_count);
    if ((e = hipGetLastError()) != hipSuccess) return e;
    if ((e = select_waves(over_list, over_count, p.queue, p.max_len_short, std::min(n_blocks, 256))) != hipSuccess) return e;
  }
  if (p.n_long) {
    const int nb = (int)std::min<uint64_t>((uint64_t)n_blocks, (p.n_long + 3) / 4);
    if ((e = select_waves(p.work_long, p.work_counts + 4, p.queue + 1, p.max_len_long, std::max(nb, 1))) != hipSuccess) return e;
  }
  return hipSuccess;
}
hipError_t launch_seed(const SeedParamsT<uint32_t>& p, int n_blocks, hipStream_t s) { return launch_seed_t(p, n_blocks, s); }
hipError_t launch_seed(const SeedParamsT<uint64_t>& p, int n_blocks, hipStream_t s) { return launch_seed_t(p, n_blocks, s); }

hipError_t launch_plan(const PlanParams& p, hipStream_t s) {
  if (p.n_reads == 0) return hipSuccess;
  hipLaunchKernelGGL(dev::plan_kernel, dim3((unsigned)((p.n_reads + 255) / 256)), dim3(256), 0, s, p);
  return hipGetLastError();
}

template <class C>
static hipError_t launch_pack_reads_t(const PackParamsT<C>& p, hipStream_t s) {
  if (p.n_reads == 0) return hipSuccess;
  hipLaunchKernelGGL(dev::pack_reads_kernel<C>, dim3((unsigned)((p.n_reads + 255) / 256)), dim3(256), 0, s, p);
  return hipGetLastError();
}
hipError_t launch_pack_reads(const PackParamsT<uint32_t>& p, hipStream_t s) { return launch_pack_reads_t(p, s); }
hipError_t launch_pack_reads(const PackParamsT<uint64_t>& p, hipStream_t s) { return launch_pack_reads_t(p, s); }

template <class C>
static hipError_t launch_expand_t(const ExpandParamsT<C>& p, hipStream_t s) {
  const unsigned blocks = (unsigned)((p.n_reads + 3) / 4);
  if (blocks == 0) return hipSuccess;
  hipLaunchKernelGGL(dev::expand_kernel<C>, dim3(blocks), dim3(256), 0, s, p);
  return hipGetLastError();
}
hipError_t launch_expand(const ExpandParamsT<uint32_t>& p, hipStream_t s) { return launch_expand_t(p, s); }
hipError_t launch_expand(const ExpandParamsT<uint64_t>& p, hipStream_t s) { return launch_expand_t(p, s); }

}
```

### thermite_amd/csrc/kernels_util.hip

```cpp
#include <hip/hip_runtime.h>

#include "launch.h"

namespace thm {
namespace dev {

constexpr int SCAN_THREADS = 256;
constexpr int SCAN_ITEMS = 8;
constexpr int SCAN_TILE = SCAN_THREADS * SCAN_ITEMS;

__device__ uint64_t block_excl_scan(uint64_t v, uint64_t* sh, uint64_t* tot) {
  const int t = (int)threadIdx.x;
  sh[t] = v;
  __syncthreads();
  for (int o = 1; o < SCAN_THREADS; o <<= 1) {
    uint64_t a = (t >= o) ? sh[t - o] : 0;
    __syncthreads();
    sh[t] += a;
    __syncthreads();
  }
  const uint64_t incl = sh[t];
  *tot = sh[SCAN_THREADS - 1];
  __syncthreads();
  return incl - v;
}

__global__ __launch_bounds__(SCAN_THREADS) void scan_tiles_kernel(const uint64_t* in, uint64_t* out, uint64_t n,
                                                                  uint64_t* tile_sums) {
  __shared__ uint64_t sh[SCAN_THREADS];
  const uint64_t base = (uint64_t)blockIdx.x * SCAN_TILE + (uint64_t)threadIdx.x * SCAN_ITEMS;
  uint64_t v[SCAN_ITEMS], s = 0;
#pragma unroll
  for (int k = 0; k < SCAN_ITEMS; k++) {
    v[k] = (base + k < n) ? in[base + k] : 0;
    s += v[k];
  }
  uint64_t tot;
  uint64_t pre = block_excl_scan(s, sh, &tot);
#pragma unroll
  for (int k = 0; k < SCAN_ITEMS; k++) {
    if (base + k < n) out[base + k] = pre;
    pre += v[k];
  }
  if (threadIdx.x == 0) tile_sums[blockIdx.x] = tot;
}

__global__ __launch_bounds__(SCAN_THREADS) void scan_sums_kernel(uint64_t* tile_sums, uint64_t n_tiles,
                                                                 uint64_t* total_out) {
  __shared__ uint64_t sh[SCAN_THREADS];
  uint64_t carry = 0;
  for (uint64_t b0 = 0; b0 < n_tiles; b0 += SCAN_THREADS) {
    const uint64_t i = b0 + threadIdx.x;
    const uint64_t v = (i < n_tiles) ? tile_sums[i] : 0;
    uint64_t tot;
    const uint64_t pre = block_excl_scan(v, sh, &tot);
    if (i < n_tiles) tile_sums[i] = carry + pre;
    carry += tot;
  }
  if (threadIdx.x == 0) *total_out = carry;
}

__global__ __launch_bounds__(SCAN_THREADS) void scan_add_kernel(uint64_t* out, uint64_t n, const uint64_t* tile_offs) {
  const uint64_t base = (uint64_t)blockIdx.x * SCAN_TILE + (uint64_t)threadIdx.x * SCAN_ITEMS;
  const uint64_t add = tile_offs[blockIdx.x];
#pragma unroll
  for (int k = 0; k < SCAN_ITEMS; k++)
    if (base + k < n) out[base + k] += add;
}

__global__ void widen_kernel(const uint32_t* in, uint64_t* out, uint64_t n) {
  const uint64_t i = (uint64_t)blockIdx.x * blockDim.x + threadIdx.x;
  if (i < n) out[i] = in[i];
}

__device__ __forceinline__ uint64_t mix64(uint64_t x) {
  x ^= x >> 33;
  x *= 0xff51afd7ed558ccdull;
  x ^= x >> 33;
  x *= 0xc4ceb9fe1a85ec53ull;
  x ^= x >> 33;
  return x;
}
__global__ __launch_bounds__(256) void calib_gather_kernel(const uint8_t* table, uint64_t span, uint64_t n_threads, int pattern,
                                                           unsigned long long* sink) {
  const uint64_t tid = (uint64_t)blockIdx.x * 256 + threadIdx.x;
  if (tid >= n_threads) return;
  unsigned long long acc = 0;
  if (pattern == 0) {
    const uint64_t o = (mix64(tid) % (span / 8)) * 8;
    acc = *(const unsigned long long*)(table + o);
  } else if (pattern == 1) {
    const uint64_t o = (mix64(tid) % (span / 4)) * 4;
    acc = *(const unsigned*)(table + o);
  } else {
    const uint64_t o = (mix64(tid >> 4) % ((span - 256) / 16)) * 16 + (tid & 15) * 16;
    const uint4 v = *(const uint4*)(table + o);
    acc = v.x ^ v.y ^ v.z ^ v.w;
  }
  if (acc == 0x7f4a7c15ull) *sink = acc;
}

}

hipError_t launch_calib_gather(const uint8_t* table, uint64_t span, uint64_t n_threads, int pattern, unsigned long long* sink,
                               hipStream_t s) {
  if (n_threads == 0) return hipSuccess;
  hipLaunchKernelGGL(dev::calib_gather_kernel, dim3((unsigned)((n_threads + 255) / 256)), dim3(256), 0, s, table, span, n_threads,
                     pattern, sink);
  return hipGetLastError();
}

size_t scan_tmp_entries(uint64_t n) { return (size_t)((n + dev::SCAN_TILE - 1) / dev::SCAN_TILE) + 1; }

hipError_t launch_exclusive_scan_u64(const uint64_t* in, uint64_t* out, uint64_t n, uint64_t* tmp, hipStream_t s) {
  if (n == 0) return hipMemsetAsync(out, 0, 8, s);
  const uint64_t tiles = (n + dev::SCAN_TILE - 1) / dev::SCAN_TILE;
  hipLaunchKernelGGL(dev::scan_tiles_kernel, dim3((unsigned)tiles), dim3(dev::SCAN_THREADS), 0, s, in, out, n, tmp);
  hipLaunchKernelGGL(dev::scan_sums_kernel, dim3(1), dim3(dev::SCAN_THREADS), 0, s, tmp, tiles, out + n);
  hipLaunchKernelGGL(dev::scan_add_kernel, dim3((unsigned)tiles), dim3(dev::SCAN_THREADS), 0, s, out, n, tmp);
  return hipGetLastError();
}

hipError_t launch_widen_u32_to_u64(const uint32_t* in, uint64_t* out, uint64_t n, hipStream_t s) {
  if (n == 0) return hipSuccess;
  hipLaunchKernelGGL(dev::widen_kernel, dim3((unsigned)((n + 255) / 256)), dim3(256), 0, s, in, out, n);
  return hipGetLastError();
}

}
```

### thermite_amd/csrc/launch.h

```cpp
#ifndef THERMITE_LAUNCH_H
#define THERMITE_LAUNCH_H

#include <hip/hip_runtime.h>

#include "thermite_internal.h"

namespace thm {

struct SwgBatchParams {
  const uint8_t* xb;
  const uint64_t* xo;
  const uint8_t* yb;
  const uint64_t* yo;
  const uint32_t* bw;
  const int32_t* xd;
  const uint64_t* ops_off;
  uint8_t* ops;
  thm_swg_aln* out;
  unsigned long long* counters;
  unsigned int* queue;
  int* fault;
  uint64_t n;
  uint32_t x_cap, y_cap;
  uint8_t* scratch;
  uint64_t scratch_per_wave;
  uint32_t max_bw;
};
size_t swg_batch_lds_bytes(const SwgBatchParams& p, int cpl);
size_t swg_batch_scratch_bytes(const SwgBatchParams& p);
hipError_t launch_swg_batch(const SwgBatchParams& p, int cpl, int n_blocks, hipStream_t s);
hipError_t launch_wave_prims(const int* in, int* out, hipStream_t s);

struct ElrBatchParams {
  const uint8_t* xb;
  const uint64_t* xo;
  const uint8_t* yb;
  const uint64_t* yo;
  const thm_mem* hits;
  const uint32_t* bw;
  const int32_t* xd;
  const uint64_t* ops_off;
  uint8_t* ops;
  thm_lr_aln* out;
  unsigned long long* counters;
  unsigned int* queue;
  int* fault;
  uint64_t n;
  uint32_t x_cap, y_cap;
  uint8_t* scratch;
  uint64_t scratch_per_wave;
  uint32_t max_bw;
};
size_t elr_batch_lds_bytes(const ElrBatchParams& p, int cpl);
size_t elr_batch_scratch_bytes(const ElrBatchParams& p);
hipError_t launch_elr_batch(const ElrBatchParams& p, int cpl, int n_blocks, hipStream_t s);

struct ReadBatch {
  const uint8_t* bases;
  const uint64_t* offsets;
  uint64_t n_reads;
};

constexpr uint32_t MAX_READ_LEN = 65535;
constexpr uint32_t SHORT_READ_MAX = 255;

__host__ __device__ inline uint64_t ms_row(uint64_t base_off, uint64_t r) { return (base_off + 8 * r) & ~7ull; }

template <class C>
struct SeedParamsT {
  DeviceIndexT<C> ix;
  ReadBatch reads;
  uint32_t min_seed_len;
  uint32_t max_len_short;
  uint32_t max_len_long;
  uint64_t n_long;
  uint16_t* ms_end;
  C* ms_lo;
  C* ms_hi;
  unsigned long long* work_short;
  unsigned long long* work_long;
  unsigned long long* work_cells;
  unsigned long long* work_counts;
  uint32_t flags;
  SmemT<C>* smems;
  uint64_t smem_cap;
  unsigned long long* cursor;
  uint64_t* read_smem_off;
  uint32_t* read_smem_cnt;
  uint64_t* read_hits;
  int32_t* read_status;
  unsigned long long* counters;
  unsigned int* queue;
  int* fault;
  uint8_t* sel_scratch;
  uint64_t sel_scratch_per_wave;
  uint32_t fill_mode;
  uint16_t* fill_keys;
  uint32_t* fill_perm;
  unsigned int* fill_hist;
};
constexpr uint32_t SEED_INFER = 1u, SEED_STATS = 2u;
constexpr int FILL_KEY_BASES = 7;
constexpr unsigned FILL_BUCKETS = 1u << (2 * FILL_KEY_BASES);
size_t seed_select_lds_bytes(uint32_t max_read_len);
size_t seed_select_scratch_bytes(uint32_t max_read_len);
constexpr size_t SEED_SELECT_LDS_LIMIT = 64 * 1024;
hipError_t launch_seed(const SeedParamsT<uint32_t>& p, int n_blocks, hipStream_t s);
hipError_t launch_seed(const SeedParamsT<uint64_t>& p, int n_blocks, hipStream_t s);
hipError_t launch_sanitize(const uint8_t* in, uint8_t* out, uint64_t n, uint64_t n_padded, hipStream_t s);

struct PlanParams {
  const uint64_t* offsets;
  const uint64_t* read_hits;
  uint64_t n_reads;
  uint32_t fast_max_len;
  uint32_t slow_max_len;
  unsigned long long* heavy;
  unsigned long long* slow;
  unsigned long long* team;
  uint32_t team_ok;
  const uint64_t* total_hits;
  uint32_t team_div;
  uint32_t tpr_max_hits;
  unsigned long long* counts;
  int32_t* read_status;
  uint32_t* read_n_alns;
  uint64_t* read_op_bytes;
};
hipError_t launch_plan(const PlanParams& p, hipStream_t s);

template <class C>
struct ReadRecT {
  uint64_t base_off;
  uint64_t smem_off;
  uint64_t cand_off;
  uint32_t len;
  uint32_t smem_cnt;
  uint32_t n_hits;
  uint16_t qpos0, len0;
  C lo0, hi0;
  C sa0;
};
static_assert(sizeof(ReadRecT<uint32_t>) == 56 && sizeof(ReadRecT<uint64_t>) == 64, "ReadRec layout");
template <class C>
struct PackParamsT {
  const C* sa;
  const uint64_t* offsets;
  uint64_t n_reads;
  const SmemT<C>* smems;
  const uint64_t* read_smem_off;
  const uint32_t* read_smem_cnt;
  const uint64_t* read_cand_off;
  const int* fault_seed;
  ReadRecT<C>* recs;
};
hipError_t launch_pack_reads(const PackParamsT<uint32_t>& p, hipStream_t s);
hipError_t launch_pack_reads(const PackParamsT<uint64_t>& p, hipStream_t s);

template <class C>
struct ExpandParamsT {
  DeviceIndexT<C> ix;
  uint64_t n_reads;
  const SmemT<C>* smems;
  const uint64_t* read_smem_off;
  const uint32_t* read_smem_cnt;
  const uint64_t* read_mem_off;
  thm_mem* mems;
};
hipError_t launch_expand(const ExpandParamsT<uint32_t>& p, hipStream_t s);
hipError_t launch_expand(const ExpandParamsT<uint64_t>& p, hipStream_t s);

hipError_t launch_exclusive_scan_u64(const uint64_t* in, uint64_t* out, uint64_t n, uint64_t* block_tmp,
                                     hipStream_t s);
size_t scan_tmp_entries(uint64_t n);

struct Cand {
  uint64_t ystart, yend, ylen;
  uint64_t tx_ystart, tx_yend, tx_ylen;
  uint64_t ops_off;
  uint64_t tx_ops_off;
  int32_t score;
  uint32_t ref_id;
  uint32_t xstart, xend;
  uint32_t ops_len, tx_ops_len;
  uint32_t tx_or_gene_idx;
  int32_t tx_score;
  uint32_t tx_xstart, tx_xend;
  uint32_t name_rank;
  uint8_t strand, aln_type, primary, pad_;
};

constexpr unsigned EXT_NQ = 8, EXT_QSTRIDE = 64;
constexpr size_t QUEUE_BYTES = (EXT_NQ + 3) * EXT_QSTRIDE * 4;
constexpr unsigned HEAVY_HITS = 8;
constexpr unsigned TEAM_HITS = 256;
constexpr unsigned TEAM_MIN_HITS = 32;
constexpr unsigned TEAM_DIV_PER_CU = 22;
constexpr int TEAM_WAVES = 16;
constexpr unsigned TEAM_MAX_HITS = 60000;
constexpr int FAST_MAX_YCLIPS = 64;

template <class C>
struct ExtendParamsT {
  DeviceIndexT<C> ix;
  ReadBatch reads;
  thm_align_opts opts;
  const SmemT<C>* smems;
  const ReadRecT<C>* read_recs;
  const unsigned long long* heavy;
  const unsigned long long* heavy_count;
  const unsigned long long* team;
  const unsigned long long* team_count;
  uint32_t team_limit;
  Cand* cands;
  uint64_t cand_cap;
  uint32_t* order;
  uint8_t* cand_ops;
  uint64_t cand_ops_cap;
  unsigned long long* ops_cursor;
  uint32_t* read_n_alns;
  uint64_t* read_op_bytes;
  int32_t* read_status;
  unsigned long long* retry;
  unsigned long long* retry_count;
  unsigned long long* n_contract;
  unsigned long long* counters;
  unsigned long long* wave_counters;
  unsigned int* queue;
  int* fault;
  const int* fault_seed;
  uint32_t max_read_len;
  uint32_t max_bw;
  uint32_t mk_cap;
  uint32_t list_only;
  uint32_t skip_scan;
  unsigned long long* trace_scratch;
  uint8_t* slow_scratch;
  uint64_t slow_scratch_per_wave;
  unsigned long long* prof;
};
size_t extend_lds_bytes(uint32_t max_read_len, uint32_t max_bw, int cpl);
int extend_waves_per_simd(int cpl, bool wide);
int compact_k();
int hit_gl();
size_t extend_trace_scratch_bytes(uint32_t max_read_len, uint32_t max_bw, int cpl);
size_t extend_slow_scratch_bytes(uint32_t max_read_len, uint32_t max_bw, uint32_t mk_cap);
constexpr size_t EXTEND_LDS_LIMIT = 160 * 1024;
constexpr size_t TEAM_STATIC_LDS = 16384 + TEAM_WAVES * 32 + 64;
inline bool team_fits_lds(size_t lds4) { return lds4 / 4 * TEAM_WAVES + TEAM_STATIC_LDS + 256 <= EXTEND_LDS_LIMIT; }
hipError_t launch_extend(const ExtendParamsT<uint32_t>& p, int cpl, int n_blocks, hipStream_t s, bool team = false);
hipError_t launch_extend(const ExtendParamsT<uint64_t>& p, int cpl, int n_blocks, hipStream_t s, bool team = false);
enum : uint16_t {
  SK_EMPTY = 0,
  SK_SINGLE = 1,
  SK_SHORTCUT = 2,
  SK_UNK_DEL = 3,
  SK_UNK = 4,
  SK_UNK_EQ = 5
};
struct HitSide {
  uint16_t kind;
  uint16_t eq;
  uint32_t A;
};
struct HitTgt {
  uint32_t tx, ent;
  int32_t tr;
  uint16_t t_q, t_len;
  HitSide r, l;
  uint32_t pos;
};
constexpr int HIT_MAX_OPEN = 3;
constexpr int HIT_MAX_VAR = 4;
enum : uint8_t { HF_COMPLEX = 1, HF_KNOWN = 2 };
struct HitSum {
  uint64_t hr;
  uint32_t ref_id;
  uint16_t q, len;
  HitSide gr, gl;
  uint32_t win_fixed;
  uint8_t win_nl, win_nr, win_nvl, win_nvr;
  uint16_t win_var[HIT_MAX_VAR];
  uint8_t n_tgt;
  uint8_t n_open;
  uint8_t flags;
  uint8_t why;
  HitTgt known;
  HitTgt open[HIT_MAX_OPEN];
  uint32_t pad_;
};
static_assert(sizeof(HitSide) == 8 && sizeof(HitTgt) == 36 && sizeof(HitSum) == 200, "hit summary layout");
struct HitHdr {
  uint64_t hr;
  uint32_t read;
  uint16_t q, len;
};
template <class C>
struct HitParamsT {
  DeviceIndexT<C> ix;
  ReadBatch reads;
  thm_align_opts opts;
  const SmemT<C>* smems;
  const ReadRecT<C>* read_recs;
  uint32_t max_read_len, max_hits;
  HitHdr* hdr;
  HitSum* sums;
  const uint64_t* total_hits;
  uint64_t slot_cap;
  const int* fault_seed;
};
hipError_t launch_hit_expand(const HitParamsT<uint32_t>& p, hipStream_t s);
hipError_t launch_hit_expand(const HitParamsT<uint64_t>& p, hipStream_t s);
hipError_t launch_hit_summaries(const HitParamsT<uint32_t>& p, int n_blocks, hipStream_t s);
hipError_t launch_hit_summaries(const HitParamsT<uint64_t>& p, int n_blocks, hipStream_t s);

constexpr int DP_MAX_EDITS = 8;
struct DpRec {
  const uint8_t* x0;
  const uint8_t* y0;
  uint64_t pad0_;
  uint16_t xlen, ylen, bw, xd;
  int8_t dir;
  uint8_t cls;
  uint16_t n_edits;
  uint32_t read;
  int32_t score;
  uint16_t xend, yend, nops;
  uint16_t done;
  uint32_t cells, cols;
  uint32_t pad2_;
};
static_assert(sizeof(DpRec) == 64, "DpRec layout");
constexpr int DPT_SLOTS = 16;
constexpr int DP_NQ = 5;
constexpr int TPR_MAX_ROUNDS = 8;
constexpr unsigned TPR_MAX_HITS = 32;
struct ReadMemo {
  uint32_t base[TPR_MAX_ROUNDS];
  uint16_t cnt[TPR_MAX_ROUNDS];
  uint16_t first_hit[TPR_MAX_ROUNDS];
  uint8_t n_rounds;
  uint8_t pad_[7];
};
static_assert(sizeof(ReadMemo) == 72, "ReadMemo layout");
template <class C>
struct TprParamsT {
  ReadRecT<C>* recs_rw;
  ReadMemo* memos;
  DpRec* recs;
  uint64_t rec_cap;
  unsigned long long* rec_cursor;
  uint32_t* q_list;
  uint64_t q_stride;
  unsigned long long* q_cur;
  const uint32_t* act_in;
  const unsigned long long* n_act_in;
  uint32_t* act_out;
  unsigned long long* n_act_out;
  unsigned long long* bail;
  unsigned long long* bail_count;
  unsigned long long* team;
  unsigned long long* team_count;
  uint32_t max_hits;
  uint32_t dpt_cols;
  const HitSum* sums;
  uint32_t round;
  uint32_t last_round;
  unsigned long long* stats;
};
struct DpParams {
  DpRec* recs;
  const uint32_t* q_list;
  uint64_t q_stride;
  const unsigned long long* q_cur;
  const unsigned long long* q_done;
  unsigned int* work;
  int* fault;
  uint32_t x_cap, y_cap;
  unsigned long long* trace_scratch;
  uint64_t trace_per_wave;
  uint32_t tcols;
};
size_t extend_dpt_lds_bytes(uint32_t tcols);
hipError_t launch_extend_dpt(const DpParams& p, int n_blocks, hipStream_t s);
size_t extend_dp_lds_bytes(uint32_t x_cap, uint32_t y_cap);
size_t extend_dp_trace_bytes(uint32_t y_cap, int cpl_max);
hipError_t launch_extend_ctl(const ExtendParamsT<uint32_t>& p, const TprParamsT<uint32_t>& tp, int n_blocks, hipStream_t s);
hipError_t launch_extend_ctl(const ExtendParamsT<uint64_t>& p, const TprParamsT<uint64_t>& tp, int n_blocks, hipStream_t s);
hipError_t launch_extend_dp(const DpParams& p, int cpl_max, int n_blocks, hipStream_t s);
hipError_t launch_tpr_order(const ReadRecT<uint32_t>* recs, uint64_t n, uint32_t max_len, uint32_t max_hits, unsigned long long* bins, uint32_t* out,
                            unsigned long long* n_out, const int* fault_seed, hipStream_t s);
hipError_t launch_tpr_order(const ReadRecT<uint64_t>* recs, uint64_t n, uint32_t max_len, uint32_t max_hits, unsigned long long* bins, uint32_t* out,
                            unsigned long long* n_out, const int* fault_seed, hipStream_t s);
constexpr int TPR_CTL_BLOCKS_PER_CU = 4, TPR_DP_BLOCKS_PER_CU = 8;
enum { TPRC_REC_CUR = 0, TPRC_Q_CUR = 2 , TPRC_Q_DONE = 7 , TPRC_N_ACT = 12 , TPRC_STATS = 24 , TPRC_BAIL_CNT = 23,
       TPRC_BINS = 40 ,
       TPRC_WORK_BYTES = 2048  };
constexpr size_t TPRC_BYTES = TPRC_WORK_BYTES + (size_t)(TPR_MAX_ROUNDS + 1) * 4 * 64;

struct CompactParams {
  uint64_t n_reads;
  const uint64_t* read_cand_off;
  const Cand* cands;
  const uint32_t* order;
  const uint8_t* cand_ops;
  const uint32_t* read_n_alns;
  const uint64_t* read_aln_off;
  const uint64_t* read_ops_off;
  const uint64_t* read_offsets;
  thm_aln* alns;
  uint8_t* ops;
  const int* fault;
  uint64_t alns_cap, ops_cap;
  unsigned long long* heavy_cnt;
  uint64_t* heavy_list;
  uint64_t* heavy_desc;
  uint32_t* rel;
  uint64_t heavy_cap;
};
hipError_t launch_compact(const CompactParams& p, hipStream_t s);
hipError_t launch_counters_reduce(const unsigned long long* wave_counters, uint32_t n_rows, unsigned long long* counters, hipStream_t s);

template <class C>
struct SeedHitParamsT {
  DeviceIndexT<C> ix;
  ReadBatch reads;
  const thm_mem* hits;
  const uint32_t* hit_read;
  const uint32_t* bw;
  const int32_t* xd;
  const uint32_t* list;
  uint64_t n_list;
  const unsigned long long* n_list_dev;
  uint32_t* retry;
  unsigned long long* retry_count;
  thm_aln* out;
  int32_t* status;
  uint8_t* cand_ops;
  uint64_t cand_ops_cap;
  unsigned long long* ops_cursor;
  unsigned long long* counters;
  unsigned int* queue;
  int* fault;
  uint32_t max_read_len, max_bw, mk_cap;
  unsigned long long* trace_scratch;
  uint8_t* slow_scratch;
  uint64_t slow_scratch_per_wave;
};
hipError_t launch_seed_hits(const SeedHitParamsT<uint32_t>& p, int cpl, int n_blocks, hipStream_t s);
hipError_t launch_seed_hits(const SeedHitParamsT<uint64_t>& p, int cpl, int n_blocks, hipStream_t s);

hipError_t launch_calib_gather(const uint8_t* table, uint64_t span, uint64_t n_threads, int pattern, unsigned long long* sink,
                               hipStream_t s);
hipError_t launch_widen_u32_to_u64(const uint32_t* in, uint64_t* out, uint64_t n, hipStream_t s);

struct CigarSum {
  uint64_t ref_len;
  uint32_t n_match, n_subst, n_not_yclip, flags;
};
struct CigarParams {
  const uint8_t* ops;
  uint64_t ops_bytes;
  uint64_t n_streams;
  const thm_aln* alns;
  const uint64_t* off;
  CigarSum* sums;
  uint64_t* n_words;
  const uint64_t* word_off;
  uint32_t* words;
  thm_aln_digest* digests;
  unsigned int* any_flags;
};
hipError_t launch_cigar_count(const CigarParams& p, int n_cu, hipStream_t s);
hipError_t launch_cigar_emit(const CigarParams& p, int n_cu, hipStream_t s);

constexpr uint32_t THM_BAM_FLAG_NO_ANNOTATION = 1u;
constexpr unsigned BAM_ERR_QNAME = 1u, BAM_ERR_CIGAR_WORDS = 2u, BAM_ERR_DIGEST_FLAGS = 4u, BAM_ERR_RANGE = 8u;
struct BamParams {
  uint64_t n_reads, n_rec;
  uint32_t flags;
  uint32_t n_refs, n_txs, n_genes;
  const uint8_t* bases;
  const uint64_t* offsets;
  const uint8_t* quals;
  const uint8_t* names;
  const uint64_t* name_off;
  const uint64_t* aln_off;
  const thm_aln* alns;
  const thm_aln_digest* digests;
  const uint32_t* words;
  uint64_t n_words;
  const uint8_t *tx_pool, *gid_pool, *gname_pool;
  const uint32_t *tx_off, *gid_off, *gname_off;
  const uint32_t* tx_gene;
  const int32_t* ref_sq;
  uint64_t* rec_cnt;
  const uint64_t* rec_first;
  uint32_t* qn;
  uint32_t* rec_read;
  uint64_t* rec_len;
  const uint64_t* rec_off;
  uint8_t* out;
  uint64_t* read_rec_off;
  unsigned int* err;
};
hipError_t launch_bam_prep(const BamParams& p, hipStream_t s);
hipError_t launch_bam_size(const BamParams& p, hipStream_t s);
hipError_t launch_bam_emit(const BamParams& p, bool stage, int n_cu, hipStream_t s);
hipError_t launch_bam_offsets(const BamParams& p, hipStream_t s);

}
#endif
```

### thermite_amd/csrc/pipeline.hip

```cpp
#include <hip/hip_runtime.h>

#include <algorithm>
#include <cstring>

#include "aligner_internal.h"

using namespace thm;

uint32_t seed_fill_mode() {
  static const uint32_t v = [] {
    const char* e = getenv("THM_SEED_FILL");
    const int v = e ? atoi(e) : 0;
    return (uint32_t)(v >= 0 && v <= 2 ? v : 0);
  }();
  return v;
}
unsigned team_div_per_cu() {
  static const unsigned v = [] {
    const char* e = getenv("THM_TEAM_DIV_PER_CU");
    const int v = e ? atoi(e) : 0;
    return v > 0 ? (unsigned)v : TEAM_DIV_PER_CU;
  }();
  return v;
}

namespace {

int band_for_len(const thm_align_opts& o, uint32_t L) {
  volatile float prod = o.min_aln_score_percent * (float)L;
  float pv = prod;
  int pct = (pv != pv) ? 0 : (pv >= 2147483648.0f ? 2147483647 : (pv <= -2147483648.0f ? (-2147483647 - 1) : (int)pv));
  int ms = std::max(pct, o.min_aln_score);
  if (ms < 0) return 0;
  return std::max((int)L - ms, 0);
}

int blocks_for(const thm_aligner* a, uint64_t n, size_t lds_per_block) {
  int per_cu = 8;
  if (lds_per_block > 0) per_cu = (int)std::min<size_t>(8, (160 * 1024) / lds_per_block);
  if (per_cu < 1) per_cu = 1;
  return grid_blocks(a, n, 4, per_cu);
}

constexpr uint64_t SLOW_SCRATCH_BUDGET = 24ull << 30;

template <class C>
const DeviceIndexT<C>& dev_view(const thm_aligner* a);
template <>
const DeviceIndexT<uint32_t>& dev_view<uint32_t>(const thm_aligner* a) {
  return a->dix->view;
}
template <>
const DeviceIndexT<uint64_t>& dev_view<uint64_t>(const thm_aligner* a) {
  return a->dix->view64;
}

template <class C>
int enqueue_seed_t(thm_aligner* a, uint32_t min_seed_len) {
  const uint64_t n = a->n_reads;
  hipStream_t s = a->stream;
  HIPCHK(a, a->s_off.ensure((n + 1) * 8));
  HIPCHK(a, a->s_cnt.ensure((n + 1) * 4));
  HIPCHK(a, a->s_hits.ensure((n + 1) * 8));
  HIPCHK(a, a->s_cand_off.ensure((n + 2) * 8));
  HIPCHK(a, a->scan_tmp.ensure(scan_tmp_entries(n + 1) * 8 + 64));
  HIPCHK(a, a->r_status.ensure((n + 1) * 4));
  HIPCHK(a, hipMemsetAsync(a->r_status.p, 0, (n + 1) * 4, s));
  const uint64_t smem_min = a->dbg_smem_cap ? a->dbg_smem_cap : n * 4 + (4u << 20);
  if (a->smem_cap < smem_min) a->smem_cap = smem_min;
  HIPCHK(a, a->s_smems.ensure(a->smem_cap * sizeof(SmemT<C>)));
  if (!a->dbg_smem_cap) a->smem_cap = std::max<uint64_t>(a->smem_cap, a->s_smems.cap / sizeof(SmemT<C>));
  HIPCHK(a, a->r_san.ensure(a->n_bases + 256 + 16));
  HIPCHK(a, hipMemsetAsync(a->r_san.p, 0, 16, s));
  HIPCHK(a, launch_sanitize(a->r_bases.as<uint8_t>(), a->r_san.as<uint8_t>() + 16, a->n_bases, a->n_bases + 128, s));
  uint64_t n_long = 0;
  uint32_t max_short = 0, max_long = 0;
  for (const auto& lc : a->len_hist) {
    if (lc.first <= SHORT_READ_MAX) {
      max_short = std::max(max_short, lc.first);
    } else {
      max_long = std::max(max_long, lc.first);
      n_long += lc.second;
    }
  }
  const uint64_t n_short = n - n_long;
  const uint64_t items = ms_row(a->n_bases, n) + 64;
  HIPCHK(a, a->s_ms_end.ensure(items * 2 + 64));
  HIPCHK(a, a->s_ms_lo.ensure(items * sizeof(C) + 64));
  HIPCHK(a, a->s_ms_hi.ensure(items * sizeof(C) + 64));
  auto cells_of = [&](uint32_t max_len) -> uint64_t {
    const uint32_t P = (max_len >= min_seed_len) ? max_len - min_seed_len + 1 : 1;
    return (P + 7) / 8;
  };
  const uint64_t cells = n_short * cells_of(max_short) + n_long * cells_of(max_long);
  HIPCHK(a, a->s_work_reads.ensure((n + 1) * 8));
  HIPCHK(a, a->s_work_long.ensure((n_long + 1) * 8));
  HIPCHK(a, a->s_work_cells.ensure((std::max(cells, n) + 1) * 8));
  HIPCHK(a, a->s_work_counts.ensure(128));
  HIPCHK(a, hipMemsetAsync(a->s_work_counts.p, 0, 128, s));
  int rc = reset_queue(a);
  if (rc != THM_OK) return rc;
  HIPCHK(a, hipMemsetAsync(a->d_cursors.p, 0, 64, s));
  const int n_blocks = blocks_for(a, n, std::min(seed_select_lds_bytes(std::max(max_short, 1u)), SEED_SELECT_LDS_LIMIT));
  SeedParamsT<C> sp;
  sp.ix = dev_view<C>(a);
  sp.reads.bases = a->r_san.as<uint8_t>() + 16;
  sp.reads.offsets = a->r_offsets.as<uint64_t>();
  sp.reads.n_reads = n;
  sp.min_seed_len = min_seed_len;
  sp.max_len_short = max_short;
  sp.max_len_long = max_long;
  sp.n_long = n_long;
  sp.ms_end = a->s_ms_end.as<uint16_t>();
  sp.ms_lo = a->s_ms_lo.as<C>();
  sp.ms_hi = a->s_ms_hi.as<C>();
  sp.work_short = a->s_work_reads.as<unsigned long long>();
  sp.work_long = a->s_work_long.as<unsigned long long>();
  sp.work_cells = a->s_work_cells.as<unsigned long long>();
  sp.work_counts = a->s_work_counts.as<unsigned long long>();
  sp.flags = (a->dbg_seed_noinfer ? 0u : SEED_INFER) | (a->dbg_seed_stats ? SEED_STATS : 0u);
  sp.smems = a->s_smems.as<SmemT<C>>();
  sp.smem_cap = a->smem_cap;
  sp.cursor = a->d_cursors.as<unsigned long long>();
  sp.read_smem_off = a->s_off.as<uint64_t>();
  sp.read_smem_cnt = a->s_cnt.as<uint32_t>();
  sp.read_hits = a->s_hits.as<uint64_t>();
  sp.read_status = a->r_status.as<int32_t>();
  sp.counters = a->d_counters.as<unsigned long long>();
  sp.queue = a->d_queue.as<unsigned int>();
  sp.fault = a->d_fault.as<int>();
  sp.sel_scratch = nullptr;
  sp.sel_scratch_per_wave = 0;
  const uint32_t fill_mode = seed_fill_mode();
  sp.fill_mode = fill_mode;
  sp.fill_keys = nullptr;
  sp.fill_perm = nullptr;
  sp.fill_hist = nullptr;
  if (fill_mode == 2) {
    const uint64_t slots = (std::max(cells, n) + 1) * 8;
    HIPCHK(a, a->s_fill_keys.ensure(slots * 2));
    HIPCHK(a, a->s_fill_perm.ensure(slots * 4));
    HIPCHK(a, a->s_fill_hist.ensure((2 * (FILL_BUCKETS + 1) + 1) * 4));
    HIPCHK(a, hipMemsetAsync(a->s_fill_hist.p, 0, (2 * (FILL_BUCKETS + 1) + 1) * 4, s));
    sp.fill_keys = a->s_fill_keys.as<uint16_t>();
    sp.fill_perm = a->s_fill_perm.as<uint32_t>();
    sp.fill_hist = a->s_fill_hist.as<unsigned int>();
  }
  if (n_long && seed_select_lds_bytes(max_long) > SEED_SELECT_LDS_LIMIT) {
    const int nb = (int)std::max<uint64_t>(1, std::min<uint64_t>((uint64_t)n_blocks, (n_long + 3) / 4));
    sp.sel_scratch_per_wave = (seed_select_scratch_bytes(max_long) + 255) & ~255ull;
    HIPCHK(a, a->s_sel_scratch.ensure((size_t)nb * 4 * sp.sel_scratch_per_wave + 256));
    sp.sel_scratch = a->s_sel_scratch.as<uint8_t>();
  }
  HIPCHK(a, launch_seed(sp, n_blocks, s));
  HIPCHK(a, launch_exclusive_scan_u64(a->s_hits.as<uint64_t>(), a->s_cand_off.as<uint64_t>(), n,
                                      a->scan_tmp.as<uint64_t>(), s));
  return THM_OK;
}

int enqueue_seed(thm_aligner* a, uint32_t min_seed_len) {
  return a->dix->wide ? enqueue_seed_t<uint64_t>(a, min_seed_len) : enqueue_seed_t<uint32_t>(a, min_seed_len);
}

struct ExtClasses {
  uint32_t fast_max = 0, fast_len = 0, fast_bw = 0;
  uint32_t slow_max = 0, slow_len = 0, slow_bw = 0;
  uint64_t n_slow = 0;
};
ExtClasses classify(const thm_aligner* a, uint32_t mk_cap_slow) {
  ExtClasses c;
  bool fast_open = true;
  for (const auto& lc : a->len_hist) {
    const uint32_t L = lc.first;
    const uint32_t bw = (uint32_t)band_for_len(a->opts, L);
    const int cpl = (int)((2 * bw + 1 + 63) / 64);
    if (fast_open && cpl <= 4 && extend_lds_bytes(L, bw, cpl) <= EXTEND_LDS_LIMIT) {
      c.fast_len = L;
      c.fast_bw = bw;
      continue;
    }
    fast_open = false;
    if (extend_slow_scratch_bytes(L, bw, mk_cap_slow) > SLOW_SCRATCH_BUDGET) break;
    c.slow_len = L;
    c.slow_bw = bw;
    c.n_slow += lc.second;
  }
  c.fast_max = c.fast_len;
  c.slow_max = std::max(c.slow_len, c.fast_len);
  return c;
}

template <class C>
int enqueue_extend_t(thm_aligner* a, const ExtClasses& cls, uint32_t mk_cap_slow, bool retry_possible) {
  const uint64_t n = a->n_reads;
  hipStream_t s = a->stream;
  ExtendParamsT<C> ep;
  ep.ix = dev_view<C>(a);
  ep.reads.bases = a->r_san.as<uint8_t>() + 16;
  ep.reads.offsets = a->r_offsets.as<uint64_t>();
  ep.reads.n_reads = n;
  ep.opts = a->opts;
  ep.smems = a->s_smems.as<SmemT<C>>();
  HIPCHK(a, a->e_recs.ensure((n + 1) * sizeof(ReadRecT<C>)));
  {
    PackParamsT<C> pk;
    pk.sa = ep.ix.sa;
    pk.offsets = a->r_offsets.as<uint64_t>();
    pk.n_reads = n;
    pk.smems = ep.smems;
    pk.read_smem_off = a->s_off.as<uint64_t>();
    pk.read_smem_cnt = a->s_cnt.as<uint32_t>();
    pk.read_cand_off = a->s_cand_off.as<uint64_t>();
    pk.fault_seed = a->d_fault.as<int>();
    pk.recs = a->e_recs.as<ReadRecT<C>>();
    HIPCHK(a, launch_pack_reads(pk, s));
  }
  ep.read_recs = a->e_recs.as<ReadRecT<C>>();
  ep.heavy = a->s_heavy.as<unsigned long long>();
  ep.heavy_count = a->s_work_counts.as<unsigned long long>() + 2;
  ep.team = a->s_team.as<unsigned long long>();
  ep.team_count = a->s_work_counts.as<unsigned long long>() + 7;
  ep.team_limit = 2u * (uint32_t)a->n_cu;
  ep.cands = a->e_cands.as<Cand>();
  ep.cand_cap = a->cand_cap;
  ep.order = a->e_order.as<uint32_t>();
  ep.cand_ops = a->e_ops.as<uint8_t>();
  ep.cand_ops_cap = a->cand_ops_cap;
  ep.ops_cursor = a->d_cursors.as<unsigned long long>() + 1;
  ep.read_n_alns = a->e_nalns.as<uint32_t>();
  ep.read_op_bytes = a->e_opbytes.as<uint64_t>();
  ep.read_status = a->r_status.as<int32_t>();
  ep.retry = a->s_slow.as<unsigned long long>();
  ep.retry_count = a->s_work_counts.as<unsigned long long>() + 5;
  ep.n_contract = a->s_work_counts.as<unsigned long long>() + 6;
  ep.counters = a->d_counters.as<unsigned long long>();
  ep.queue = a->d_queue.as<unsigned int>();
  ep.fault = a->d_fault.as<int>() + 1;
  ep.fault_seed = a->d_fault.as<int>();
  ep.prof = a->d_counters.as<unsigned long long>() + 2 * THM_N_COUNTERS;
  ep.slow_scratch = nullptr;
  ep.slow_scratch_per_wave = 0;
  ep.trace_scratch = nullptr;
  ep.max_read_len = cls.fast_len;
  ep.max_bw = cls.fast_bw;
  if (a->dbg_band_clip) ep.max_bw = std::min<uint32_t>(ep.max_bw, a->dbg_band_clip - 1);
  ep.mk_cap = FAST_MAX_YCLIPS;
  ep.list_only = 0;
  const int cpl = std::max(1, (int)((2 * cls.fast_bw + 1 + 63) / 64));
  const size_t lds = extend_lds_bytes(cls.fast_len, cls.fast_bw, cpl);
  const int ext_blocks = std::min(blocks_for(a, n, lds), a->n_cu * extend_waves_per_simd(cpl, sizeof(C) == 8));
  const bool team_ok = cpl <= 2 && team_fits_lds(lds);
  const size_t trace_per_wave = extend_trace_scratch_bytes(cls.fast_len, cls.fast_bw, cpl);
  const size_t main_trace_waves = (size_t)ext_blocks * 4, team_trace_waves = team_ok ? (size_t)a->n_cu * TEAM_WAVES : 0;
  HIPCHK(a, a->e_trace.ensure((main_trace_waves + team_trace_waves) * trace_per_wave + 64));
  ep.trace_scratch = a->e_trace.as<unsigned long long>();
  uint64_t slow_waves = 0, slow_per_wave = 0;
  if (cls.n_slow || retry_possible) {
    const uint32_t sl_len = std::max(cls.slow_len, cls.fast_len), sl_bw = std::max(cls.slow_bw, cls.fast_bw);
    slow_per_wave = (extend_slow_scratch_bytes(sl_len, sl_bw, mk_cap_slow) + 255) & ~255ull;
    slow_waves = std::max<uint64_t>(1, std::min<uint64_t>(SLOW_SCRATCH_BUDGET / std::max<uint64_t>(slow_per_wave, 1), (uint64_t)a->n_cu * 8));
    if (!retry_possible) slow_waves = std::min(slow_waves, std::max<uint64_t>(cls.n_slow, 1));
    slow_waves = (slow_waves + 3) / 4 * 4;
  }
  const uint64_t main_rows = (uint64_t)ext_blocks * 4, team_rows = team_ok ? (uint64_t)a->n_cu * TEAM_WAVES : 0;
  const bool tpr = a->use_tpr && n > 0 && cpl <= 4;
  const int ctl_blocks = tpr ? (int)std::min<uint64_t>((n + 255) / 256, (uint64_t)a->n_cu * TPR_CTL_BLOCKS_PER_CU) : 0;
  const uint32_t dp_x_cap = (cls.fast_len + 64u + 15u) & ~15u, dp_y_cap = (cls.fast_len + cls.fast_bw + 2u + 64u + 15u) & ~15u;
  const int dp_per_cu = (int)std::max<size_t>(1, std::min<size_t>(TPR_DP_BLOCKS_PER_CU, EXTEND_LDS_LIMIT / std::max<size_t>(1, extend_dp_lds_bytes(dp_x_cap, dp_y_cap))));
  const int dp_blocks = tpr ? a->n_cu * dp_per_cu : 0;
  const uint32_t dpt_tcols = std::min<uint32_t>(std::min<uint32_t>(dp_y_cap, 128u), std::max<uint32_t>(cls.fast_len + DPT_SLOTS / 2 + 2, DPT_SLOTS + cls.fast_bw + 2));
  const int dpt_per_cu = (int)std::max<size_t>(1, std::min<size_t>(8, EXTEND_LDS_LIMIT / std::max<size_t>(1, extend_dpt_lds_bytes(dpt_tcols))));
  const int dpt_blocks = tpr ? a->n_cu * dpt_per_cu : 0;
  const int bail_blocks = tpr ? std::min(ext_blocks, a->n_cu) : 0;
  const uint64_t tpr_rows = (uint64_t)ctl_blocks + (uint64_t)bail_blocks * 4;
  const uint64_t n_rows = main_rows + team_rows + slow_waves + tpr_rows;
  HIPCHK(a, a->e_wcnt.ensure(n_rows * THM_N_COUNTERS * 8 + 64));
  HIPCHK(a, hipMemsetAsync(a->e_wcnt.p, 0, n_rows * THM_N_COUNTERS * 8, s));
  ep.wave_counters = a->e_wcnt.as<unsigned long long>();
  ep.skip_scan = 0;
  if (tpr) {
    const uint64_t rec_cap = std::min<uint64_t>(4 * n + 65536, 64ull << 20);
    HIPCHK(a, a->t_memos.ensure(n * sizeof(ReadMemo) + 64));
    HIPCHK(a, a->t_recs.ensure(rec_cap * sizeof(DpRec) + 64));
    HIPCHK(a, a->t_qlist.ensure((size_t)DP_NQ * rec_cap * 4 + 64));
    HIPCHK(a, a->t_act[0].ensure(n * 4 + 64));
    HIPCHK(a, a->t_act[1].ensure(n * 4 + 64));
    HIPCHK(a, a->t_bail.ensure((n + 1) * 8));
    HIPCHK(a, a->t_queue2.ensure(thm::QUEUE_BYTES));
    HIPCHK(a, hipMemsetAsync(a->t_queue2.p, 0, thm::QUEUE_BYTES, s));
    HIPCHK(a, a->t_ctl.ensure(TPRC_BYTES));
    HIPCHK(a, hipMemsetAsync(a->t_ctl.p, 0, TPRC_BYTES, s));
    unsigned long long* ctl = a->t_ctl.as<unsigned long long>();
    TprParamsT<C> tq;
    tq.recs_rw = a->e_recs.as<ReadRecT<C>>();
    tq.memos = a->t_memos.as<ReadMemo>();
    tq.recs = a->t_recs.as<DpRec>();
    tq.rec_cap = rec_cap;
    tq.rec_cursor = ctl + TPRC_REC_CUR;
    tq.q_list = a->t_qlist.as<uint32_t>();
    tq.q_stride = rec_cap;
    tq.q_cur = ctl + TPRC_Q_CUR;
    tq.bail = a->t_bail.as<unsigned long long>();
    tq.bail_count = ctl + TPRC_BAIL_CNT;
    tq.team = nullptr;
    tq.team_count = nullptr;
    tq.max_hits = TPR_MAX_HITS;
    tq.dpt_cols = dpt_tcols;
    tq.stats = ctl + TPRC_STATS;
    ExtendParamsT<C> zp = ep;
    zp.wave_counters = ep.wave_counters + (main_rows + team_rows + slow_waves) * THM_N_COUNTERS;
    DpParams dq;
    dq.recs = tq.recs;
    dq.q_list = tq.q_list;
    dq.q_stride = tq.q_stride;
    dq.q_cur = ctl + TPRC_Q_CUR;
    dq.q_done = ctl + TPRC_Q_DONE;
    dq.fault = ep.fault;
    dq.x_cap = dp_x_cap;
    dq.y_cap = dp_y_cap;
    {
      const size_t tb = extend_dp_trace_bytes(dp_y_cap, cpl);
      HIPCHK(a, a->t_trace.ensure((size_t)dp_blocks * 4 * tb + 64));
      dq.trace_scratch = a->t_trace.as<unsigned long long>();
      dq.trace_per_wave = tb / 8;
      dq.tcols = dpt_tcols;
    }
    {
      const uint64_t slot_cap = a->cand_cap;
      HIPCHK(a, a->t_hdr.ensure(slot_cap * sizeof(HitHdr) + 64));
      HIPCHK(a, a->t_sums.ensure(slot_cap * sizeof(HitSum) + 64));
      HIPCHK(a, hipMemsetAsync(a->t_hdr.p, 0xFF, slot_cap * sizeof(HitHdr), s));
      HitParamsT<C> hq;
      hq.ix = ep.ix;
      hq.reads = ep.reads;
      hq.opts = ep.opts;
      hq.smems = ep.smems;
      hq.read_recs = ep.read_recs;
      hq.max_read_len = cls.fast_len;
      hq.max_hits = TPR_MAX_HITS;
      hq.hdr = a->t_hdr.as<HitHdr>();
      hq.sums = a->t_sums.as<HitSum>();
      hq.total_hits = a->s_cand_off.as<uint64_t>() + n;
      hq.slot_cap = slot_cap;
      hq.fault_seed = a->d_fault.as<int>();
      HIPCHK(a, launch_hit_expand(hq, s));
      HIPCHK(a, launch_hit_summaries(hq, a->n_cu * 12, s));
      tq.sums = a->t_sums.as<HitSum>();
    }
    {
      ExtendParamsT<C> hp = ep;
      hp.skip_scan = 1;
      hp.team_limit = 16u * (uint32_t)a->n_cu;
      HIPCHK(a, hipEventRecord(a->ev_fork, s));
      HIPCHK(a, hipStreamWaitEvent(a->stream2, a->ev_fork, 0));
      HIPCHK(a, hipStreamWaitEvent(a->stream3, a->ev_fork, 0));
      if (team_ok) {
        ExtendParamsT<C> tp = hp;
        tp.list_only = 1;
        tp.wave_counters = ep.wave_counters + main_rows * THM_N_COUNTERS;
        tp.trace_scratch = ep.trace_scratch + main_trace_waves * trace_per_wave / 8;
        HIPCHK(a, launch_extend(tp, cpl, a->n_cu, a->stream2, true));
      }
      HIPCHK(a, launch_extend(hp, cpl, std::min(ext_blocks, a->n_cu), a->stream3));
      HIPCHK(a, hipEventRecord(a->ev_join, a->stream2));
      HIPCHK(a, hipEventRecord(a->ev_join3, a->stream3));
    }
    HIPCHK(a, launch_tpr_order(a->e_recs.as<ReadRecT<C>>(), n, cls.fast_len, TPR_MAX_HITS, ctl + TPRC_BINS, a->t_act[0].as<uint32_t>(), ctl + TPRC_N_ACT,
                               a->d_fault.as<int>(), s));
    const int n_rounds = a->tpr_rounds;
    for (int r = 0; r <= n_rounds; r++) {
      tq.round = (uint32_t)r;
      tq.act_in = a->t_act[r & 1].as<uint32_t>();
      tq.n_act_in = ctl + TPRC_N_ACT + r;
      tq.act_out = a->t_act[(r + 1) & 1].as<uint32_t>();
      tq.n_act_out = ctl + TPRC_N_ACT + r + 1;
      tq.last_round = r == n_rounds ? 1u : 0u;
      HIPCHK(a, launch_extend_ctl(zp, tq, ctl_blocks, s));
      if (r == n_rounds) break;
      dq.work = (unsigned int*)((uint8_t*)a->t_ctl.p + TPRC_WORK_BYTES + (size_t)r * 4 * 64);
      HIPCHK(a, hipEventRecord(a->ev_dpt_fork, s));
      HIPCHK(a, hipStreamWaitEvent(a->stream4, a->ev_dpt_fork, 0));
      HIPCHK(a, launch_extend_dpt(dq, dpt_blocks, a->stream4));
      HIPCHK(a, hipEventRecord(a->ev_dpt_join, a->stream4));
      HIPCHK(a, launch_extend_dp(dq, cpl, dp_blocks, s));
      HIPCHK(a, hipStreamWaitEvent(s, a->ev_dpt_join, 0));
      HIPCHK(a, hipMemcpyAsync(ctl + TPRC_Q_DONE, ctl + TPRC_Q_CUR, DP_NQ * 8, hipMemcpyDeviceToDevice, s));
    }
    HIPCHK(a, hipStreamWaitEvent(s, a->ev_join, 0));
    HIPCHK(a, hipStreamWaitEvent(s, a->ev_join3, 0));
    {
      ExtendParamsT<C> bp = ep;
      bp.skip_scan = 1;
      bp.heavy = a->t_bail.as<unsigned long long>();
      bp.heavy_count = ctl + TPRC_BAIL_CNT;
      bp.team = nullptr;
      bp.team_count = nullptr;
      bp.queue = a->t_queue2.as<unsigned int>();
      bp.wave_counters = zp.wave_counters + (uint64_t)ctl_blocks * THM_N_COUNTERS;
      HIPCHK(a, launch_extend(bp, cpl, bail_blocks, s));
    }
  } else if (team_ok) {
    ExtendParamsT<C> tp = ep;
    tp.list_only = 1;
    tp.wave_counters = ep.wave_counters + main_rows * THM_N_COUNTERS;
    tp.trace_scratch = ep.trace_scratch + main_trace_waves * trace_per_wave / 8;
    HIPCHK(a, hipEventRecord(a->ev_fork, s));
    HIPCHK(a, launch_extend(tp, cpl, a->n_cu, s, true));
    HIPCHK(a, hipStreamWaitEvent(a->stream2, a->ev_fork, 0));
    HIPCHK(a, launch_extend(ep, cpl, ext_blocks, a->stream2));
    HIPCHK(a, hipEventRecord(a->ev_join, a->stream2));
    HIPCHK(a, hipStreamWaitEvent(s, a->ev_join, 0));
  } else {
    HIPCHK(a, launch_extend(ep, cpl, ext_blocks, s));
  }
  if (cls.n_slow || retry_possible) {
    const uint32_t sl_len = std::max(cls.slow_len, cls.fast_len), sl_bw = std::max(cls.slow_bw, cls.fast_bw);
    const uint64_t per_wave = slow_per_wave;
    const int blocks = (int)(slow_waves / 4);
    ep.wave_counters = a->e_wcnt.as<unsigned long long>() + (main_rows + team_rows) * THM_N_COUNTERS;
    HIPCHK(a, a->e_slow.ensure((size_t)blocks * 4 * per_wave + 256));
    ep.max_read_len = sl_len;
    ep.max_bw = sl_bw;
    ep.mk_cap = mk_cap_slow;
    ep.list_only = 1;
    ep.heavy = a->s_slow.as<unsigned long long>();
    ep.heavy_count = a->s_work_counts.as<unsigned long long>() + 5;
    ep.team = nullptr;
    ep.team_count = nullptr;
    ep.slow_scratch = a->e_slow.as<uint8_t>();
    ep.slow_scratch_per_wave = per_wave;
    HIPCHK(a, launch_extend(ep, 0, blocks, s));
  }
  HIPCHK(a, launch_counters_reduce(a->e_wcnt.as<unsigned long long>(), (uint32_t)n_rows, a->d_counters.as<unsigned long long>(), s));
  return THM_OK;
}

int enqueue_run(thm_aligner* a) {
  const uint64_t n = a->n_reads;
  hipStream_t s = a->stream;
  HIPCHK(a, hipMemcpyAsync(a->d_counters.as<uint8_t>() + THM_N_COUNTERS * 8, a->d_counters.p, THM_N_COUNTERS * 8,
                           hipMemcpyDeviceToDevice, s));
  HIPCHK(a, hipEventRecord(a->ev[0], s));
  int rc = enqueue_seed(a, (uint32_t)a->opts.min_seed_len);
  if (rc != THM_OK) return rc;
  HIPCHK(a, hipEventRecord(a->ev[1], s));

  const uint64_t cand_min = a->dbg_cand_cap ? a->dbg_cand_cap : n * 3 + 1024;
  const uint64_t ops_min = a->dbg_ops_cap ? a->dbg_ops_cap : std::max<uint64_t>(n * 384, a->n_bases * 3) + 65536;
  if (a->cand_cap < cand_min) a->cand_cap = cand_min;
  if (a->cand_ops_cap < ops_min) a->cand_ops_cap = ops_min;
  HIPCHK(a, a->e_cands.ensure(a->cand_cap * sizeof(Cand)));
  HIPCHK(a, a->e_order.ensure(a->cand_cap * 2 * 4));
  HIPCHK(a, a->e_heavy.ensure((a->cand_cap / 2 + 16) * 2 * 8));
  HIPCHK(a, a->e_rel.ensure(a->cand_cap * 4));
  HIPCHK(a, a->e_ops.ensure(a->cand_ops_cap + 64));
  HIPCHK(a, a->e_nalns.ensure((n + 1) * 4));
  HIPCHK(a, a->e_nalns64.ensure((n + 1) * 8));
  HIPCHK(a, a->e_opbytes.ensure((n + 1) * 8));
  HIPCHK(a, a->e_aln_off.ensure((n + 2) * 8));
  HIPCHK(a, a->e_ops_off.ensure((n + 2) * 8));
  HIPCHK(a, a->o_alns.ensure(a->cand_cap * sizeof(thm_aln)));
  HIPCHK(a, a->o_ops.ensure(a->cand_ops_cap + 64));
  HIPCHK(a, a->s_heavy.ensure((n + 1) * 8));
  HIPCHK(a, a->s_slow.ensure((n + 1) * 8));
  HIPCHK(a, a->s_team.ensure((n + 1) * 8));
  HIPCHK(a, hipMemsetAsync(a->d_queue.p, 0, thm::QUEUE_BYTES, s));

  const uint32_t mk_cap_slow = std::max<uint32_t>(a->ix->max_tx_exons, 1);
  const bool retry_possible = a->ix->max_tx_exons > (uint32_t)FAST_MAX_YCLIPS + 1;
  const ExtClasses cls = classify(a, mk_cap_slow);
  a->n_slow_host = cls.n_slow;
  a->fast_max_len = cls.fast_max;
  a->slow_max_len = cls.slow_max;
  PlanParams pp;
  pp.offsets = a->r_offsets.as<uint64_t>();
  pp.read_hits = a->s_hits.as<uint64_t>();
  pp.n_reads = n;
  pp.fast_max_len = cls.fast_max;
  pp.slow_max_len = cls.slow_max;
  pp.heavy = a->s_heavy.as<unsigned long long>();
  pp.slow = a->s_slow.as<unsigned long long>();
  pp.team = a->s_team.as<unsigned long long>();
  {
    const int cpl_f = std::max(1, (int)((2 * cls.fast_bw + 1 + 63) / 64));
    pp.team_ok = (cpl_f <= 2 && team_fits_lds(extend_lds_bytes(cls.fast_len, cls.fast_bw, cpl_f))) ? 1u : 0u;
  }
  pp.total_hits = a->s_cand_off.as<uint64_t>() + n;
  pp.team_div = team_div_per_cu() * (uint32_t)std::max(a->n_cu, 1);
  pp.tpr_max_hits = (a->use_tpr && std::max(1, (int)((2 * cls.fast_bw + 1 + 63) / 64)) <= 4) ? TPR_MAX_HITS : 0u;
  pp.counts = a->s_work_counts.as<unsigned long long>();
  pp.read_status = a->r_status.as<int32_t>();
  pp.read_n_alns = a->e_nalns.as<uint32_t>();
  pp.read_op_bytes = a->e_opbytes.as<uint64_t>();
  HIPCHK(a, launch_plan(pp, s));
  HIPCHK(a, hipEventRecord(a->ev[2], s));

  rc = a->dix->wide ? enqueue_extend_t<uint64_t>(a, cls, mk_cap_slow, retry_possible)
                    : enqueue_extend_t<uint32_t>(a, cls, mk_cap_slow, retry_possible);
  if (rc != THM_OK) return rc;
  HIPCHK(a, hipEventRecord(a->ev[3], s));

  HIPCHK(a, launch_widen_u32_to_u64(a->e_nalns.as<uint32_t>(), a->e_nalns64.as<uint64_t>(), n, s));
  HIPCHK(a, launch_exclusive_scan_u64(a->e_nalns64.as<uint64_t>(), a->e_aln_off.as<uint64_t>(), n,
                                      a->scan_tmp.as<uint64_t>(), s));
  HIPCHK(a, launch_exclusive_scan_u64(a->e_opbytes.as<uint64_t>(), a->e_ops_off.as<uint64_t>(), n,
                                      a->scan_tmp.as<uint64_t>(), s));
  CompactParams cp;
  cp.n_reads = n;
  cp.read_cand_off = a->s_cand_off.as<uint64_t>();
  cp.cands = a->e_cands.as<Cand>();
  cp.order = a->e_order.as<uint32_t>();
  cp.cand_ops = a->e_ops.as<uint8_t>();
  cp.read_n_alns = a->e_nalns.as<uint32_t>();
  cp.read_aln_off = a->e_aln_off.as<uint64_t>();
  cp.read_ops_off = a->e_ops_off.as<uint64_t>();
  cp.read_offsets = a->r_offsets.as<uint64_t>();
  cp.alns = a->o_alns.as<thm_aln>();
  cp.ops = a->o_ops.as<uint8_t>();
  cp.fault = a->d_fault.as<int>();
  cp.alns_cap = a->cand_cap;
  cp.ops_cap = a->cand_ops_cap;
  cp.heavy_cap = a->cand_cap / 2 + 16;
  cp.heavy_cnt = a->d_cursors.as<unsigned long long>() + 2;
  cp.heavy_list = a->e_heavy.as<uint64_t>();
  cp.heavy_desc = a->e_heavy.as<uint64_t>() + cp.heavy_cap;
  cp.rel = a->e_rel.as<uint32_t>();
  HIPCHK(a, launch_compact(cp, s));
  HIPCHK(a, hipEventRecord(a->ev[4], s));
  return THM_OK;
}

struct RunStatus {
  int fault_seed = 0, fault_ext = 0;
  unsigned long long smem_used = 0, ops_used = 0, total_hits = 0;
};
int read_status(thm_aligner* a, RunStatus* st) {
  hipStream_t s = a->stream;
  int f[2] = {0, 0};
  unsigned long long cur[2] = {0, 0};
  HIPCHK(a, hipMemcpyAsync(f, a->d_fault.p, 8, hipMemcpyDeviceToHost, s));
  HIPCHK(a, hipMemcpyAsync(cur, a->d_cursors.p, 16, hipMemcpyDeviceToHost, s));
  HIPCHK(a, hipMemcpyAsync(&st->total_hits, a->s_cand_off.as<uint64_t>() + a->n_reads, 8, hipMemcpyDeviceToHost, s));
  HIPCHK(a, hipStreamSynchronize(s));
  st->fault_seed = f[0];
  st->fault_ext = f[1];
  st->smem_used = cur[0];
  st->ops_used = cur[1];
  return THM_OK;
}

template <class C>
int expand_mems_t(thm_aligner* a, uint64_t n) {
  ExpandParamsT<C> xp;
  xp.ix = dev_view<C>(a);
  xp.n_reads = n;
  xp.smems = a->s_smems.as<SmemT<C>>();
  xp.read_smem_off = a->s_off.as<uint64_t>();
  xp.read_smem_cnt = a->s_cnt.as<uint32_t>();
  xp.read_mem_off = a->s_cand_off.as<uint64_t>();
  xp.mems = a->o_mems.as<thm_mem>();
  HIPCHK(a, launch_expand(xp, a->stream));
  return THM_OK;
}

}

extern "C" {

int32_t thm_batch_upload(thm_aligner* a, const uint8_t* bases, const uint64_t* offsets, uint64_t n_reads) {
  if (!a || !offsets || (!bases && n_reads && offsets[n_reads] > 0)) return THM_ERR_INVALID_ARG;
  HIPCHK(a, hipSetDevice(a->device));
  a->uploaded = a->ran = a->synced = false;
  a->reads_named = false;
  if (n_reads >= 0xFFFFFFF0ull) return fail(a, THM_ERR_UNSUPPORTED, "more than 2^32-16 reads in one batch");
  if (offsets[0] != 0) return fail(a, THM_ERR_INVALID_ARG, "offsets[0] must be 0");
  uint32_t lmax = 0;
  uint64_t n_over = 0;
  a->len_hist.clear();
  {
    std::vector<uint64_t> cnt(1024, 0);
    std::vector<std::pair<uint32_t, uint64_t>> big;
    for (uint64_t i = 0; i < n_reads; i++) {
      if (offsets[i + 1] < offsets[i]) return fail(a, THM_ERR_INVALID_ARG, "read offsets are not monotone");
      const uint64_t L = offsets[i + 1] - offsets[i];
      if (L > MAX_READ_LEN) {
        n_over++;
        continue;
      }
      if (L < cnt.size())
        cnt[L]++;
      else
        big.emplace_back((uint32_t)L, 1);
      lmax = std::max<uint32_t>(lmax, (uint32_t)L);
    }
    for (uint32_t L = 0; L < cnt.size(); L++)
      if (cnt[L]) a->len_hist.emplace_back(L, cnt[L]);
    std::sort(big.begin(), big.end());
    for (const auto& b : big) {
      if (!a->len_hist.empty() && a->len_hist.back().first == b.first)
        a->len_hist.back().second++;
      else
        a->len_hist.push_back(b);
    }
  }
  a->n_over = n_over;
  a->n_reads = n_reads;
  a->n_bases = offsets[n_reads];
  a->max_read_len = lmax;
  HIPCHK(a, a->r_bases.ensure(a->n_bases + 64));
  HIPCHK(a, a->r_offsets.ensure((n_reads + 1) * 8));
  if (a->n_bases) HIPCHK(a, hipMemcpyAsync(a->r_bases.p, bases, a->n_bases, hipMemcpyHostToDevice, a->stream));
  HIPCHK(a, hipMemcpyAsync(a->r_offsets.p, offsets, (n_reads + 1) * 8, hipMemcpyHostToDevice, a->stream));
  HIPCHK(a, hipStreamSynchronize(a->stream));
  a->uploaded = true;
  return THM_OK;
}

int32_t thm_batch_run(thm_aligner* a) {
  if (!a) return THM_ERR_INVALID_ARG;
  if (!a->uploaded) return fail(a, THM_ERR_INVALID_ARG, "thm_batch_run before thm_batch_upload");
  HIPCHK(a, hipSetDevice(a->device));
  a->ran = false;
  a->synced = false;
  int rc = enqueue_run(a);
  if (rc == THM_OK) a->ran = true;
  return rc;
}

int32_t thm_batch_sync(thm_aligner* a) {
  if (!a) return THM_ERR_INVALID_ARG;
  if (!a->ran) return fail(a, THM_ERR_INVALID_ARG, "thm_batch_sync before thm_batch_run");
  if (a->synced) return THM_OK;
  HIPCHK(a, hipSetDevice(a->device));
  for (int attempt = 0; attempt < 6; attempt++) {
    RunStatus st;
    int rc = read_status(a, &st);
    if (rc != THM_OK) return rc;
    if (!st.fault_seed && (st.fault_ext & 2)) return fail(a, THM_ERR_INTERNAL, "extend kernel reported an internal inconsistency (fault word 0x%x)", st.fault_ext);
    const bool grow = st.fault_seed || (st.fault_ext & 1);
    if (!grow) {
      float ms = 0;
      for (int k = 0; k < 4; k++) {
        if (hipEventElapsedTime(&ms, a->ev[k], a->ev[k + 1]) == hipSuccess) a->timings[k] = ms;
      }
      if (hipEventElapsedTime(&ms, a->ev[0], a->ev[4]) == hipSuccess) a->timings[THM_T_TOTAL] = ms;
      a->synced = true;
      return THM_OK;
    }
    if (st.fault_seed) a->smem_cap = std::max<uint64_t>(a->smem_cap * 2, st.smem_used + 1024);
    if (st.total_hits > a->cand_cap) a->cand_cap = st.total_hits + st.total_hits / 8 + 1024;
    if (st.ops_used > a->cand_ops_cap) a->cand_ops_cap = st.ops_used + st.ops_used / 2 + 65536;
    if (a->cand_cap * sizeof(Cand) > (160ull << 30))
      return fail(a, THM_ERR_OOM, "batch has %llu seed hits: candidate pool would exceed 160 GiB", st.total_hits);
    HIPCHK(a, hipMemcpyAsync(a->d_counters.p, a->d_counters.as<uint8_t>() + THM_N_COUNTERS * 8, THM_N_COUNTERS * 8,
                             hipMemcpyDeviceToDevice, a->stream));
    a->n_replays++;
    rc = enqueue_run(a);
    if (rc != THM_OK) return rc;
  }
  return fail(a, THM_ERR_INTERNAL, "pools kept overflowing after 6 attempts");
}

int32_t thm_batch_fetch(thm_aligner* a, thm_batch_view* out) {
  if (!a || !out) return THM_ERR_INVALID_ARG;
  memset(out, 0, sizeof(*out));
  int rc = thm_batch_sync(a);
  if (rc != THM_OK) return rc;
  const uint64_t n = a->n_reads;
  hipStream_t s = a->stream;
  const int k = a->r_cur ^= 1;
  HBuf& h_off = a->r_off[k];
  HBuf& h_alns = a->r_alns[k];
  HBuf& h_ops = a->r_ops[k];
  HBuf& h_stat = a->r_stat[k];
  HIPCHK(a, h_off.ensure((n + 2) * 8));
  HIPCHK(a, hipMemcpyAsync(h_off.p, a->e_aln_off.p, (n + 1) * 8, hipMemcpyDeviceToHost, s));
  HIPCHK(a, hipMemcpyAsync(h_off.as<uint64_t>() + n + 1, a->e_ops_off.as<uint64_t>() + n, 8, hipMemcpyDeviceToHost, s));
  unsigned long long n_contract = 0;
  HIPCHK(a, hipMemcpyAsync(&n_contract, a->s_work_counts.as<unsigned long long>() + 6, 8, hipMemcpyDeviceToHost, s));
  HIPCHK(a, hipStreamSynchronize(s));
  const uint64_t n_alns = h_off.as<uint64_t>()[n];
  const uint64_t n_ops = h_off.as<uint64_t>()[n + 1];
  HIPCHK(a, h_alns.ensure(n_alns * sizeof(thm_aln)));
  HIPCHK(a, h_ops.ensure(n_ops));
  if (n_alns) HIPCHK(a, hipMemcpyAsync(h_alns.p, a->o_alns.p, n_alns * sizeof(thm_aln), hipMemcpyDeviceToHost, s));
  if (n_ops) HIPCHK(a, hipMemcpyAsync(h_ops.p, a->o_ops.p, n_ops, hipMemcpyDeviceToHost, s));
  uint64_t n_beyond = a->n_over;
  for (const auto& lc : a->len_hist)
    if (lc.first > a->slow_max_len) n_beyond += lc.second;
  const bool any_failed = n_beyond || n_contract;
  if (any_failed) {
    HIPCHK(a, h_stat.ensure((n + 1) * 4));
    HIPCHK(a, hipMemcpyAsync(h_stat.p, a->r_status.p, n * 4, hipMemcpyDeviceToHost, s));
  }
  HIPCHK(a, hipStreamSynchronize(s));
  out->n_reads = n;
  out->n_alns = n_alns;
  out->n_op_bytes = n_ops;
  out->read_aln_off = h_off.as<uint64_t>();
  out->alns = h_alns.as<thm_aln>();
  out->ops = h_ops.as<uint8_t>();
  out->n_failed_reads = 0;
  out->read_status = nullptr;
  if (any_failed) {
    const int32_t* st = h_stat.as<int32_t>();
    uint64_t bad = 0;
    for (uint64_t i = 0; i < n; i++) bad += st[i] != THM_OK;
    out->n_failed_reads = bad;
    out->read_status = bad ? st : nullptr;
  }
  return THM_OK;
}

int32_t thm_align_batch(thm_aligner* a, const uint8_t* bases, const uint64_t* offsets, uint64_t n_reads,
                        thm_batch_view* out) {
  int rc = thm_batch_upload(a, bases, offsets, n_reads);
  if (rc != THM_OK) return rc;
  rc = thm_batch_run(a);
  if (rc != THM_OK) return rc;
  return thm_batch_fetch(a, out);
}

int32_t thm_smems_batch(thm_aligner* a, const uint8_t* bases, const uint64_t* offsets, uint64_t n_reads,
                        uint64_t min_seed_len, thm_mems_view* out) {
  if (!a || !out) return THM_ERR_INVALID_ARG;
  memset(out, 0, sizeof(*out));
  if (min_seed_len < 1 || min_seed_len > 65535) return fail(a, THM_ERR_INVALID_ARG, "min_seed_len out of range");
  int rc = thm_batch_upload(a, bases, offsets, n_reads);
  if (rc != THM_OK) return rc;
  const uint64_t n = n_reads;
  hipStream_t s = a->stream;
  RunStatus st;
  for (int attempt = 0;; attempt++) {
    if (attempt == 0)
      HIPCHK(a, hipMemcpyAsync(a->d_counters.as<uint8_t>() + THM_N_COUNTERS * 8, a->d_counters.p, THM_N_COUNTERS * 8,
                               hipMemcpyDeviceToDevice, s));
    else
      HIPCHK(a, hipMemcpyAsync(a->d_counters.p, a->d_counters.as<uint8_t>() + THM_N_COUNTERS * 8, THM_N_COUNTERS * 8,
                               hipMemcpyDeviceToDevice, s));
    rc = enqueue_seed(a, (uint32_t)min_seed_len);
    if (rc != THM_OK) return rc;
    rc = read_status(a, &st);
    if (rc != THM_OK) return rc;
    if (!st.fault_seed) break;
    if (attempt >= 6) return fail(a, THM_ERR_INTERNAL, "smem pool kept overflowing");
    a->n_replays++;
    a->smem_cap = std::max<uint64_t>(a->smem_cap * 2, st.smem_used + 1024);
  }
  a->uploaded = false;
  const uint64_t n_mems = st.total_hits;
  if (n_mems * sizeof(thm_mem) > (64ull << 30)) return fail(a, THM_ERR_OOM, "%llu seed hits in one batch", st.total_hits);
  HIPCHK(a, a->o_mems.ensure(n_mems * sizeof(thm_mem) + 64));
  rc = a->dix->wide ? expand_mems_t<uint64_t>(a, n) : expand_mems_t<uint32_t>(a, n);
  if (rc != THM_OK) return rc;
  a->h_off.assign(n + 1, 0);
  a->h_mems.resize(n_mems);
  HIPCHK(a, hipMemcpyAsync(a->h_off.data(), a->s_cand_off.p, (n + 1) * 8, hipMemcpyDeviceToHost, s));
  if (n_mems) HIPCHK(a, hipMemcpyAsync(a->h_mems.data(), a->o_mems.p, n_mems * sizeof(thm_mem), hipMemcpyDeviceToHost, s));
  HIPCHK(a, hipStreamSynchronize(s));
  out->n_reads = n;
  out->n_mems = n_mems;
  out->read_mem_off = a->h_off.data();
  out->mems = a->h_mems.data();
  return THM_OK;
}

}
```

Baseline: 88.07 million.

## Fuse small setup kernels and memsets to cut per-batch launch overhead

Merges the control scratch buffers into one block that is zeroed by a fused sanitize-and-reset kernel, replacing several memsets and a counter-snapshot memcpy. Fuses the plan and pack kernels, folding the final scan-offset addition into the pack step. Replaces widen plus two scans with one dual scan. Makes the counters reduce multi-block and self-zeroing, so the per-run memset of the wave-counter buffer is skipped. All of this targets the launch and small-op overhead in the per-batch pipeline, at the cost of more intricate state invariants, for example the wave counters must be left zero after each reduce.

```diff
diff --git a/thermite_amd/csrc/aligner.hip b/thermite_amd/csrc/aligner.hip
--- a/thermite_amd/csrc/aligner.hip
+++ b/thermite_amd/csrc/aligner.hip
@@ -193,10 +193,18 @@
       hipEventCreateWithFlags(&a->ev_fork, hipEventDisableTiming) != hipSuccess ||
       hipEventCreateWithFlags(&a->ev_join, hipEventDisableTiming) != hipSuccess)
     return bail(fail(nullptr, THM_ERR_HIP, "second stream / events: creation failed"));
-  if (a->d_counters.ensure(THM_N_COUNTERS * 8 * 3) != hipSuccess || a->d_queue.ensure(thm::QUEUE_BYTES) != hipSuccess ||
-      a->d_fault.ensure(64) != hipSuccess || a->d_cursors.ensure(64) != hipSuccess)
+  if (a->d_counters.ensure(THM_N_COUNTERS * 8 * 3) != hipSuccess || a->d_ctl.ensure(thm_aligner::CTL_BYTES) != hipSuccess)
     return bail(fail(nullptr, THM_ERR_OOM, "scratch allocation failed"));
+  {
+    uint8_t* ctl = a->d_ctl.as<uint8_t>();
+    a->s_work_counts = {ctl + thm_aligner::CTL_WORK_COUNTS, 128};
+    a->d_cursors = {ctl + thm_aligner::CTL_CURSORS, 64};
+    a->d_fault = {ctl + thm_aligner::CTL_FAULT, 64};
+    a->d_queue = {ctl + thm_aligner::CTL_QUEUE, thm::QUEUE_BYTES};
+    a->d_queue_ext = {ctl + thm_aligner::CTL_QUEUE_EXT, thm::QUEUE_BYTES};
+  }
   (void)hipMemsetAsync(a->d_counters.p, 0, THM_N_COUNTERS * 8 * 3, a->stream);
+  (void)hipMemsetAsync(a->d_ctl.p, 0, thm_aligner::CTL_BYTES, a->stream);
   int rc = get_dev_copy(a);
   if (rc != THM_OK) return bail(rc);
   rc = thm_aligner_set_opts(a, opts);
@@ -212,10 +220,10 @@
   if (a->stream2) (void)hipStreamSynchronize(a->stream2);
   if (a->stream3) (void)hipStreamSynchronize(a->stream3);
   if (a->stream4) (void)hipStreamSynchronize(a->stream4);
-  DBuf* all[] = {&a->d_counters, &a->d_queue, &a->d_fault, &a->d_cursors, &a->b0, &a->b1, &a->b2, &a->b3, &a->b4,
-                 &a->b5, &a->b6, &a->b7, &a->b8, &a->r_bases, &a->r_offsets, &a->r_san, &a->s_ms_end, &a->s_ms_lo, &a->s_ms_hi, &a->s_work_reads, &a->s_work_long, &a->s_work_cells, &a->s_work_counts, &a->s_fill_keys, &a->s_fill_perm, &a->s_fill_hist, &a->s_sel_scratch, &a->s_heavy, &a->s_slow, &a->s_team, &a->r_status, &a->e_slow, &a->e_recs, &a->e_wcnt, &a->t_memos, &a->t_recs, &a->t_dpops, &a->t_qlist, &a->t_act[0], &a->t_act[1], &a->t_ctl, &a->t_bail, &a->t_queue2, &a->t_trace, &a->t_ttrace, &a->t_hdr, &a->t_sums, &a->s_smems, &a->s_off, &a->s_cnt,
+  DBuf* all[] = {&a->d_counters, &a->d_ctl, &a->b0, &a->b1, &a->b2, &a->b3, &a->b4,
+                 &a->b5, &a->b6, &a->b7, &a->b8, &a->r_bases, &a->r_offsets, &a->r_san, &a->s_ms_end, &a->s_ms_lo, &a->s_ms_hi, &a->s_work_reads, &a->s_work_long, &a->s_work_cells, &a->s_fill_keys, &a->s_fill_perm, &a->s_fill_hist, &a->s_sel_scratch, &a->s_heavy, &a->s_slow, &a->s_team, &a->r_status, &a->e_slow, &a->e_recs, &a->e_wcnt, &a->t_memos, &a->t_recs, &a->t_dpops, &a->t_qlist, &a->t_act[0], &a->t_act[1], &a->t_ctl, &a->t_bail, &a->t_queue2, &a->t_trace, &a->t_ttrace, &a->t_hdr, &a->t_sums, &a->s_smems, &a->s_off, &a->s_cnt,
                  &a->s_hits, &a->s_cand_off, &a->scan_tmp, &a->e_cands, &a->e_heavy, &a->e_rel, &a->e_order, &a->e_ops, &a->e_nalns,
-                 &a->e_nalns64, &a->e_opbytes, &a->e_aln_off, &a->e_ops_off, &a->e_trace, &a->o_alns, &a->o_ops, &a->o_mems,
+                 &a->e_opbytes, &a->e_aln_off, &a->e_ops_off, &a->e_trace, &a->o_alns, &a->o_ops, &a->o_mems,
                  &a->sh_bases, &a->sh_san, &a->sh_off, &a->sh_hits, &a->sh_read, &a->sh_bw, &a->sh_xd, &a->sh_list, &a->sh_out,
                  &a->sh_status, &a->sh_ops, &a->sh_ctl, &a->sh_trace, &a->sh_slow, &a->c_sums, &a->c_nwords, &a->c_woff,
                  &a->c_scan_tmp, &a->c_flags, &a->c_dig, &a->c_words, &a->c_in_ops, &a->c_in_off,
diff --git a/thermite_amd/csrc/aligner_internal.h b/thermite_amd/csrc/aligner_internal.h
--- a/thermite_amd/csrc/aligner_internal.h
+++ b/thermite_amd/csrc/aligner_internal.h
@@ -28,6 +28,15 @@
     p = nullptr;
     cap = 0;
   }
+  template <class T>
+  T* as() const {
+    return (T*)p;
+  }
+};
+
+struct DView {
+  void* p = nullptr;
+  size_t cap = 0;
   template <class T>
   T* as() const {
     return (T*)p;
@@ -93,7 +102,15 @@
   thm_align_opts opts;
   std::string err;
 
-  DBuf d_counters, d_queue, d_fault, d_cursors;
+  DBuf d_counters;
+  DBuf d_ctl;
+  static constexpr size_t CTL_WORK_COUNTS = 0, CTL_CURSORS = 128, CTL_FAULT = 192, CTL_QUEUE = 256,
+                          CTL_QUEUE_EXT = CTL_QUEUE + thm::QUEUE_BYTES, CTL_BYTES = CTL_QUEUE_EXT + thm::QUEUE_BYTES;
+  static_assert(CTL_BYTES % 16 == 0 && thm::QUEUE_BYTES % 16 == 0, "the block is zeroed 16 bytes at a time");
+  DView d_queue;
+  DView d_queue_ext;
+  DView d_fault, d_cursors;
+  DView s_work_counts;
   DBuf b0, b1, b2, b3, b4, b5, b6, b7, b8;
 
   DBuf r_bases, r_offsets, r_san;
@@ -104,10 +121,11 @@
   uint64_t n_over = 0;
   bool uploaded = false;
   DBuf s_smems, s_off, s_cnt, s_hits, s_cand_off, scan_tmp, s_ms_end, s_ms_lo, s_ms_hi, s_work_reads, s_work_long, s_work_cells,
-      s_work_counts, s_sel_scratch, s_heavy, s_slow, s_team, s_fill_keys, s_fill_perm, s_fill_hist;
+      s_sel_scratch, s_heavy, s_slow, s_team, s_fill_keys, s_fill_perm, s_fill_hist;
   uint64_t smem_cap = 0;
   DBuf e_heavy, e_rel;
-  DBuf e_cands, e_order, e_ops, e_nalns, e_nalns64, e_opbytes, e_aln_off, e_ops_off, e_trace, e_slow, e_recs, e_wcnt;
+  DBuf e_cands, e_order, e_ops, e_nalns, e_opbytes, e_aln_off, e_ops_off, e_trace, e_slow, e_recs, e_wcnt;
+  size_t wcnt_clean_cap = 0;
   DBuf t_memos, t_recs, t_dpops, t_qlist, t_act[2], t_ctl, t_bail, t_queue2, t_trace, t_ttrace, t_hdr, t_sums;
   bool use_tpr = false;
   int tpr_rounds = 8;
diff --git a/thermite_amd/csrc/kernels_extend.hip b/thermite_amd/csrc/kernels_extend.hip
--- a/thermite_amd/csrc/kernels_extend.hip
+++ b/thermite_amd/csrc/kernels_extend.hip
@@ -1589,18 +1589,35 @@
   }
 }
 
-__global__ __launch_bounds__(1024) void counters_reduce_kernel(const unsigned long long* rows, uint32_t n_rows, unsigned long long* counters) {
-  __shared__ unsigned long long part[64][THM_N_COUNTERS];
+constexpr int REDUCE_GROUPS = 64, REDUCE_MAX_BLOCKS = 32;
+__global__ __launch_bounds__(REDUCE_GROUPS * THM_N_COUNTERS) void counters_reduce_kernel(unsigned long long* rows, uint32_t n_rows,
+                                                                                       unsigned long long* counters) {
+  __shared__ unsigned long long part[REDUCE_GROUPS][THM_N_COUNTERS];
   static_assert(THM_N_COUNTERS == 16, "one thread per counter and row group");
   const int k = (int)(threadIdx.x & 15u), g = (int)(threadIdx.x >> 4);
+  const uint32_t step = gridDim.x * REDUCE_GROUPS;
   unsigned long long sum = 0;
-  for (uint32_t r = (uint32_t)g; r < n_rows; r += 64) sum += rows[(size_t)r * THM_N_COUNTERS + k];
+  for (uint32_t r0 = blockIdx.x * REDUCE_GROUPS + (uint32_t)g; r0 < n_rows; r0 += 4 * step) {
+    unsigned long long v[4];
+#pragma unroll
+    for (int j = 0; j < 4; j++) {
+      const uint64_t r = (uint64_t)r0 + (uint64_t)j * step;
+      v[j] = r < n_rows ? rows[r * THM_N_COUNTERS + k] : 0ull;
+    }
+#pragma unroll
+    for (int j = 0; j < 4; j++) {
+      if (v[j]) {
+        sum += v[j];
+        rows[((uint64_t)r0 + (uint64_t)j * step) * THM_N_COUNTERS + k] = 0;
+      }
+    }
+  }
   part[g][k] = sum;
   __syncthreads();
   if (g == 0) {
     unsigned long long t = 0;
-    for (int i = 0; i < 64; i++) t += part[i][k];
-    if (t) counters[k] += t;
+    for (int i = 0; i < REDUCE_GROUPS; i++) t += part[i][k];
+    if (t) atomicAdd(&counters[k], t);
   }
 }
 
@@ -2231,9 +2248,11 @@
 hipError_t launch_extend(const ExtendParamsT<uint32_t>& p, int cpl, int n_blocks, hipStream_t s, bool team) { return launch_extend_t(p, cpl, n_blocks, s, team); }
 hipError_t launch_extend(const ExtendParamsT<uint64_t>& p, int cpl, int n_blocks, hipStream_t s, bool team) { return launch_extend_t(p, cpl, n_blocks, s, team); }
 
-hipError_t launch_counters_reduce(const unsigned long long* wave_counters, uint32_t n_rows, unsigned long long* counters, hipStream_t s) {
+hipError_t launch_counters_reduce(unsigned long long* wave_counters, uint32_t n_rows, unsigned long long* counters, hipStream_t s) {
   if (n_rows == 0) return hipSuccess;
-  hipLaunchKernelGGL(dev::counters_reduce_kernel, dim3(1), dim3(1024), 0, s, wave_counters, n_rows, counters);
+  const unsigned blocks = std::min<unsigned>((n_rows + dev::REDUCE_GROUPS - 1) / dev::REDUCE_GROUPS, dev::REDUCE_MAX_BLOCKS);
+  hipLaunchKernelGGL(dev::counters_reduce_kernel, dim3(blocks), dim3(dev::REDUCE_GROUPS * THM_N_COUNTERS), 0, s, wave_counters, n_rows,
+                     counters);
   return hipGetLastError();
 }
 
diff --git a/thermite_amd/csrc/kernels_seed.hip b/thermite_amd/csrc/kernels_seed.hip
--- a/thermite_amd/csrc/kernels_seed.hip
+++ b/thermite_amd/csrc/kernels_seed.hip
@@ -192,8 +192,7 @@
   return false;
 }
 
-__global__ void sanitize_kernel(const uint8_t* in, uint8_t* out, uint64_t n, uint64_t n_padded) {
-  const uint64_t i = ((uint64_t)blockIdx.x * blockDim.x + threadIdx.x) * 16;
+__device__ __forceinline__ void sanitize16(const uint8_t* in, uint8_t* out, uint64_t n, uint64_t n_padded, uint64_t i) {
   if (i >= n_padded) return;
   uint4 v = make_uint4(0, 0, 0, 0);
   if (i < n) v = *(const uint4*)(in + i);
@@ -210,6 +209,18 @@
     w[j] = r;
   }
   *(uint4*)(out + i) = make_uint4(w[0], w[1], w[2], w[3]);
+}
+__global__ void sanitize_kernel(const uint8_t* in, uint8_t* out, uint64_t n, uint64_t n_padded) {
+  sanitize16(in, out, n, n_padded, ((uint64_t)blockIdx.x * blockDim.x + threadIdx.x) * 16);
+}
+__global__ void sanitize_reset_kernel(const uint8_t* in, uint8_t* out, uint64_t n, uint64_t n_padded, RunResetParams rp) {
+  const uint64_t t = (uint64_t)blockIdx.x * blockDim.x + threadIdx.x;
+  const uint4 zero = make_uint4(0, 0, 0, 0);
+  if (t < rp.status_vec4) rp.status[t] = zero;
+  if (t < rp.ctl_vec4) rp.ctl[t] = zero;
+  if (t < THM_N_COUNTERS) rp.counters[THM_N_COUNTERS + t] = rp.counters[t];
+  if (t == 0) *rp.san_head = zero;
+  sanitize16(in, out, n, n_padded, t * 16);
 }
 
 constexpr int PROBE_STRIDE = 8;
@@ -850,12 +861,14 @@
   }
 }
 
-__global__ __launch_bounds__(256) void plan_kernel(PlanParams p) {
+template <class C>
+__global__ __launch_bounds__(256) void plan_pack_kernel(PlanParams p, PackParamsT<C> q) {
   const uint64_t r = (uint64_t)blockIdx.x * 256 + threadIdx.x;
   const bool active = r < p.n_reads;
-  uint64_t L = 0, hits = 0;
+  uint64_t b0 = 0, L = 0, hits = 0;
   if (active) {
-    L = p.offsets[r + 1] - p.offsets[r];
+    b0 = p.offsets[r];
+    L = p.offsets[r + 1] - b0;
     hits = p.read_hits[r];
   }
   const bool fast = active && L <= p.fast_max_len;
@@ -871,32 +884,27 @@
   block_append(fast && !team && hits >= (p.tpr_max_hits ? (uint64_t)p.tpr_max_hits : (uint64_t)HEAVY_HITS), r, p.heavy, &p.counts[2]);
   block_append(slow, r, p.slow, &p.counts[5]);
   block_append(team, r, p.team, &p.counts[7]);
-}
-
-template <class C>
-__global__ __launch_bounds__(256) void pack_reads_kernel(PackParamsT<C> p) {
-  const uint64_t r = (uint64_t)blockIdx.x * 256 + threadIdx.x;
-  if (r >= p.n_reads) return;
+  if (!active) return;
   ReadRecT<C> rec;
-  const uint64_t b0 = p.offsets[r], L = p.offsets[r + 1] - b0;
   rec.base_off = b0;
   rec.len = L > 0xFFFFFFFEull ? 0xFFFFFFFFu : (uint32_t)L;
-  rec.smem_off = p.read_smem_off[r];
-  rec.smem_cnt = p.read_smem_cnt[r];
-  const uint64_t c0 = p.read_cand_off[r], nh = p.read_cand_off[r + 1] - c0;
+  rec.smem_off = q.read_smem_off[r];
+  rec.smem_cnt = q.read_smem_cnt[r];
+  const uint64_t c0 = q.read_cand_off[r] + q.tile_offs[r / SCAN_TILE];
+  q.read_cand_off[r] = c0;
   rec.cand_off = c0;
-  rec.n_hits = nh > 0xFFFFFFFFull ? 0xFFFFFFFFu : (uint32_t)nh;
+  rec.n_hits = hits > 0xFFFFFFFFull ? 0xFFFFFFFFu : (uint32_t)hits;
   rec.qpos0 = rec.len0 = 0;
   rec.lo0 = rec.hi0 = rec.sa0 = 0;
-  if (rec.smem_cnt > 0 && *p.fault_seed == 0) {
-    const SmemT<C> sm = p.smems[rec.smem_off];
+  if (rec.smem_cnt > 0 && *q.fault_seed == 0) {
+    const SmemT<C> sm = q.smems[rec.smem_off];
     rec.qpos0 = sm.qpos;
     rec.len0 = sm.len;
     rec.lo0 = sm.lo;
     rec.hi0 = sm.hi;
-    if (sm.hi > sm.lo) rec.sa0 = p.sa[sm.hi - 1];
-  }
-  p.recs[r] = rec;
+    if (sm.hi > sm.lo) rec.sa0 = q.sa[sm.hi - 1];
+  }
+  q.recs[r] = rec;
 }
 
 template <class C>
@@ -930,6 +938,12 @@
 hipError_t launch_sanitize(const uint8_t* in, uint8_t* out, uint64_t n, uint64_t n_padded, hipStream_t s) {
   if (n_padded == 0) return hipSuccess;
   hipLaunchKernelGGL(dev::sanitize_kernel, dim3((unsigned)((n_padded / 16 + 255) / 256 + 1)), dim3(256), 0, s, in, out, n, n_padded);
+  return hipGetLastError();
+}
+
+hipError_t launch_sanitize_reset(const uint8_t* in, uint8_t* out, uint64_t n, uint64_t n_padded, const RunResetParams& rp, hipStream_t s) {
+  const uint64_t threads = std::max<uint64_t>(std::max<uint64_t>(n_padded / 16 + 1, rp.status_vec4), std::max<uint64_t>(rp.ctl_vec4, THM_N_COUNTERS));
+  hipLaunchKernelGGL(dev::sanitize_reset_kernel, dim3((unsigned)((threads + 255) / 256)), dim3(256), 0, s, in, out, n, n_padded, rp);
   return hipGetLastError();
 }
 
@@ -1013,20 +1027,14 @@
 hipError_t launch_seed(const SeedParamsT<uint32_t>& p, int n_blocks, hipStream_t s) { return launch_seed_t(p, n_blocks, s); }
 hipError_t launch_seed(const SeedParamsT<uint64_t>& p, int n_blocks, hipStream_t s) { return launch_seed_t(p, n_blocks, s); }
 
-hipError_t launch_plan(const PlanParams& p, hipStream_t s) {
-  if (p.n_reads == 0) return hipSuccess;
-  hipLaunchKernelGGL(dev::plan_kernel, dim3((unsigned)((p.n_reads + 255) / 256)), dim3(256), 0, s, p);
+template <class C>
+static hipError_t launch_plan_pack_t(const PlanParams& pl, const PackParamsT<C>& pk, hipStream_t s) {
+  if (pl.n_reads == 0) return hipSuccess;
+  hipLaunchKernelGGL(dev::plan_pack_kernel<C>, dim3((unsigned)((pl.n_reads + 255) / 256)), dim3(256), 0, s, pl, pk);
   return hipGetLastError();
 }
-
-template <class C>
-static hipError_t launch_pack_reads_t(const PackParamsT<C>& p, hipStream_t s) {
-  if (p.n_reads == 0) return hipSuccess;
-  hipLaunchKernelGGL(dev::pack_reads_kernel<C>, dim3((unsigned)((p.n_reads + 255) / 256)), dim3(256), 0, s, p);
-  return hipGetLastError();
-}
-hipError_t launch_pack_reads(const PackParamsT<uint32_t>& p, hipStream_t s) { return launch_pack_reads_t(p, s); }
-hipError_t launch_pack_reads(const PackParamsT<uint64_t>& p, hipStream_t s) { return launch_pack_reads_t(p, s); }
+hipError_t launch_plan_pack(const PlanParams& pl, const PackParamsT<uint32_t>& pk, hipStream_t s) { return launch_plan_pack_t(pl, pk, s); }
+hipError_t launch_plan_pack(const PlanParams& pl, const PackParamsT<uint64_t>& pk, hipStream_t s) { return launch_plan_pack_t(pl, pk, s); }
 
 template <class C>
 static hipError_t launch_expand_t(const ExpandParamsT<C>& p, hipStream_t s) {
diff --git a/thermite_amd/csrc/kernels_util.hip b/thermite_amd/csrc/kernels_util.hip
--- a/thermite_amd/csrc/kernels_util.hip
+++ b/thermite_amd/csrc/kernels_util.hip
@@ -7,7 +7,7 @@
 
 constexpr int SCAN_THREADS = 256;
 constexpr int SCAN_ITEMS = 8;
-constexpr int SCAN_TILE = SCAN_THREADS * SCAN_ITEMS;
+static_assert(SCAN_TILE == SCAN_THREADS * SCAN_ITEMS, "launch.h: SCAN_TILE");
 
 __device__ uint64_t block_excl_scan(uint64_t v, uint64_t* sh, uint64_t* tot) {
   const int t = (int)threadIdx.x;
@@ -68,9 +68,61 @@
     if (base + k < n) out[base + k] += add;
 }
 
-__global__ void widen_kernel(const uint32_t* in, uint64_t* out, uint64_t n) {
-  const uint64_t i = (uint64_t)blockIdx.x * blockDim.x + threadIdx.x;
-  if (i < n) out[i] = in[i];
+__global__ __launch_bounds__(SCAN_THREADS) void scan2_tiles_kernel(const uint32_t* in_a, const uint64_t* in_b, uint64_t* out_a,
+                                                                   uint64_t* out_b, uint64_t n, uint64_t* tile_sums) {
+  __shared__ uint64_t sh[SCAN_THREADS];
+  const uint64_t base = (uint64_t)blockIdx.x * SCAN_TILE + (uint64_t)threadIdx.x * SCAN_ITEMS;
+  uint64_t va[SCAN_ITEMS], vb[SCAN_ITEMS], sa = 0, sb = 0;
+#pragma unroll
+  for (int k = 0; k < SCAN_ITEMS; k++) {
+    va[k] = (base + k < n) ? (uint64_t)in_a[base + k] : 0;
+    vb[k] = (base + k < n) ? in_b[base + k] : 0;
+    sa += va[k];
+    sb += vb[k];
+  }
+  uint64_t tot_a, tot_b;
+  uint64_t pre_a = block_excl_scan(sa, sh, &tot_a);
+  uint64_t pre_b = block_excl_scan(sb, sh, &tot_b);
+#pragma unroll
+  for (int k = 0; k < SCAN_ITEMS; k++) {
+    if (base + k < n) {
+      out_a[base + k] = pre_a;
+      out_b[base + k] = pre_b;
+    }
+    pre_a += va[k];
+    pre_b += vb[k];
+  }
+  if (threadIdx.x == 0) {
+    tile_sums[blockIdx.x] = tot_a;
+    tile_sums[gridDim.x + blockIdx.x] = tot_b;
+  }
+}
+
+__global__ __launch_bounds__(SCAN_THREADS) void scan2_sums_kernel(uint64_t* tile_sums, uint64_t n_tiles, uint64_t* total_a,
+                                                                  uint64_t* total_b) {
+  __shared__ uint64_t sh[SCAN_THREADS];
+  uint64_t* sums = tile_sums + (uint64_t)blockIdx.x * n_tiles;
+  uint64_t carry = 0;
+  for (uint64_t b0 = 0; b0 < n_tiles; b0 += SCAN_THREADS) {
+    const uint64_t i = b0 + threadIdx.x;
+    const uint64_t v = (i < n_tiles) ? sums[i] : 0;
+    uint64_t tot;
+    const uint64_t pre = block_excl_scan(v, sh, &tot);
+    if (i < n_tiles) sums[i] = carry + pre;
+    carry += tot;
+  }
+  if (threadIdx.x == 0) *(blockIdx.x ? total_b : total_a) = carry;
+}
+
+__global__ __launch_bounds__(SCAN_THREADS) void scan2_add_kernel(uint64_t* out_a, uint64_t* out_b, uint64_t n, const uint64_t* tile_offs) {
+  const uint64_t base = (uint64_t)blockIdx.x * SCAN_TILE + (uint64_t)threadIdx.x * SCAN_ITEMS;
+  const uint64_t add_a = tile_offs[blockIdx.x], add_b = tile_offs[gridDim.x + blockIdx.x];
+#pragma unroll
+  for (int k = 0; k < SCAN_ITEMS; k++)
+    if (base + k < n) {
+      out_a[base + k] += add_a;
+      out_b[base + k] += add_b;
+    }
 }
 
 __device__ __forceinline__ uint64_t mix64(uint64_t x) {
@@ -110,20 +162,35 @@
   return hipGetLastError();
 }
 
-size_t scan_tmp_entries(uint64_t n) { return (size_t)((n + dev::SCAN_TILE - 1) / dev::SCAN_TILE) + 1; }
+size_t scan_tmp_entries(uint64_t n) { return (size_t)((n + SCAN_TILE - 1) / SCAN_TILE) + 1; }
 
 hipError_t launch_exclusive_scan_u64(const uint64_t* in, uint64_t* out, uint64_t n, uint64_t* tmp, hipStream_t s) {
   if (n == 0) return hipMemsetAsync(out, 0, 8, s);
-  const uint64_t tiles = (n + dev::SCAN_TILE - 1) / dev::SCAN_TILE;
+  const uint64_t tiles = (n + SCAN_TILE - 1) / SCAN_TILE;
   hipLaunchKernelGGL(dev::scan_tiles_kernel, dim3((unsigned)tiles), dim3(dev::SCAN_THREADS), 0, s, in, out, n, tmp);
   hipLaunchKernelGGL(dev::scan_sums_kernel, dim3(1), dim3(dev::SCAN_THREADS), 0, s, tmp, tiles, out + n);
   hipLaunchKernelGGL(dev::scan_add_kernel, dim3((unsigned)tiles), dim3(dev::SCAN_THREADS), 0, s, out, n, tmp);
   return hipGetLastError();
 }
 
-hipError_t launch_widen_u32_to_u64(const uint32_t* in, uint64_t* out, uint64_t n, hipStream_t s) {
-  if (n == 0) return hipSuccess;
-  hipLaunchKernelGGL(dev::widen_kernel, dim3((unsigned)((n + 255) / 256)), dim3(256), 0, s, in, out, n);
+hipError_t launch_scan_tiles_sums_u64(const uint64_t* in, uint64_t* out, uint64_t n, uint64_t* tmp, hipStream_t s) {
+  if (n == 0) return hipMemsetAsync(out, 0, 8, s);
+  const uint64_t tiles = (n + SCAN_TILE - 1) / SCAN_TILE;
+  hipLaunchKernelGGL(dev::scan_tiles_kernel, dim3((unsigned)tiles), dim3(dev::SCAN_THREADS), 0, s, in, out, n, tmp);
+  hipLaunchKernelGGL(dev::scan_sums_kernel, dim3(1), dim3(dev::SCAN_THREADS), 0, s, tmp, tiles, out + n);
+  return hipGetLastError();
+}
+
+hipError_t launch_exclusive_scan2(const uint32_t* in_a, const uint64_t* in_b, uint64_t* out_a, uint64_t* out_b, uint64_t n,
+                                  uint64_t* tmp, hipStream_t s) {
+  if (n == 0) {
+    hipError_t e = hipMemsetAsync(out_a, 0, 8, s);
+    return e != hipSuccess ? e : hipMemsetAsync(out_b, 0, 8, s);
+  }
+  const uint64_t tiles = (n + SCAN_TILE - 1) / SCAN_TILE;
+  hipLaunchKernelGGL(dev::scan2_tiles_kernel, dim3((unsigned)tiles), dim3(dev::SCAN_THREADS), 0, s, in_a, in_b, out_a, out_b, n, tmp);
+  hipLaunchKernelGGL(dev::scan2_sums_kernel, dim3(2), dim3(dev::SCAN_THREADS), 0, s, tmp, tiles, out_a + n, out_b + n);
+  hipLaunchKernelGGL(dev::scan2_add_kernel, dim3((unsigned)tiles), dim3(dev::SCAN_THREADS), 0, s, out_a, out_b, n, tmp);
   return hipGetLastError();
 }
 
diff --git a/thermite_amd/csrc/launch.h b/thermite_amd/csrc/launch.h
--- a/thermite_amd/csrc/launch.h
+++ b/thermite_amd/csrc/launch.h
@@ -109,6 +109,16 @@
 hipError_t launch_seed(const SeedParamsT<uint64_t>& p, int n_blocks, hipStream_t s);
 hipError_t launch_sanitize(const uint8_t* in, uint8_t* out, uint64_t n, uint64_t n_padded, hipStream_t s);
 
+struct RunResetParams {
+  uint4* ctl;
+  uint32_t ctl_vec4;
+  uint4* status;
+  uint64_t status_vec4;
+  uint4* san_head;
+  unsigned long long* counters;
+};
+hipError_t launch_sanitize_reset(const uint8_t* in, uint8_t* out, uint64_t n, uint64_t n_padded, const RunResetParams& rp, hipStream_t s);
+
 struct PlanParams {
   const uint64_t* offsets;
   const uint64_t* read_hits;
@@ -127,7 +137,6 @@
   uint32_t* read_n_alns;
   uint64_t* read_op_bytes;
 };
-hipError_t launch_plan(const PlanParams& p, hipStream_t s);
 
 template <class C>
 struct ReadRecT {
@@ -150,12 +159,13 @@
   const SmemT<C>* smems;
   const uint64_t* read_smem_off;
   const uint32_t* read_smem_cnt;
-  const uint64_t* read_cand_off;
+  uint64_t* read_cand_off;
+  const uint64_t* tile_offs;
   const int* fault_seed;
   ReadRecT<C>* recs;
 };
-hipError_t launch_pack_reads(const PackParamsT<uint32_t>& p, hipStream_t s);
-hipError_t launch_pack_reads(const PackParamsT<uint64_t>& p, hipStream_t s);
+hipError_t launch_plan_pack(const PlanParams& pl, const PackParamsT<uint32_t>& pk, hipStream_t s);
+hipError_t launch_plan_pack(const PlanParams& pl, const PackParamsT<uint64_t>& pk, hipStream_t s);
 
 template <class C>
 struct ExpandParamsT {
@@ -173,6 +183,10 @@
 hipError_t launch_exclusive_scan_u64(const uint64_t* in, uint64_t* out, uint64_t n, uint64_t* block_tmp,
                                      hipStream_t s);
 size_t scan_tmp_entries(uint64_t n);
+constexpr unsigned SCAN_TILE = 2048;
+hipError_t launch_scan_tiles_sums_u64(const uint64_t* in, uint64_t* out, uint64_t n, uint64_t* block_tmp, hipStream_t s);
+hipError_t launch_exclusive_scan2(const uint32_t* in_a, const uint64_t* in_b, uint64_t* out_a, uint64_t* out_b, uint64_t n,
+                                  uint64_t* block_tmp, hipStream_t s);
 
 struct Cand {
   uint64_t ystart, yend, ylen;
@@ -419,7 +433,7 @@
   uint64_t heavy_cap;
 };
 hipError_t launch_compact(const CompactParams& p, hipStream_t s);
-hipError_t launch_counters_reduce(const unsigned long long* wave_counters, uint32_t n_rows, unsigned long long* counters, hipStream_t s);
+hipError_t launch_counters_reduce(unsigned long long* wave_counters, uint32_t n_rows, unsigned long long* counters, hipStream_t s);
 
 template <class C>
 struct SeedHitParamsT {
@@ -452,7 +466,6 @@
 
 hipError_t launch_calib_gather(const uint8_t* table, uint64_t span, uint64_t n_threads, int pattern, unsigned long long* sink,
                                hipStream_t s);
-hipError_t launch_widen_u32_to_u64(const uint32_t* in, uint64_t* out, uint64_t n, hipStream_t s);
 
 struct CigarSum {
   uint64_t ref_len;
diff --git a/thermite_amd/csrc/pipeline.hip b/thermite_amd/csrc/pipeline.hip
--- a/thermite_amd/csrc/pipeline.hip
+++ b/thermite_amd/csrc/pipeline.hip
@@ -56,23 +56,30 @@
 }
 
 template <class C>
-int enqueue_seed_t(thm_aligner* a, uint32_t min_seed_len) {
+int enqueue_seed_t(thm_aligner* a, uint32_t min_seed_len, bool finish_scan) {
   const uint64_t n = a->n_reads;
   hipStream_t s = a->stream;
   HIPCHK(a, a->s_off.ensure((n + 1) * 8));
   HIPCHK(a, a->s_cnt.ensure((n + 1) * 4));
   HIPCHK(a, a->s_hits.ensure((n + 1) * 8));
   HIPCHK(a, a->s_cand_off.ensure((n + 2) * 8));
-  HIPCHK(a, a->scan_tmp.ensure(scan_tmp_entries(n + 1) * 8 + 64));
-  HIPCHK(a, a->r_status.ensure((n + 1) * 4));
-  HIPCHK(a, hipMemsetAsync(a->r_status.p, 0, (n + 1) * 4, s));
+  HIPCHK(a, a->scan_tmp.ensure(2 * scan_tmp_entries(n + 1) * 8 + 64));
+  HIPCHK(a, a->r_status.ensure((n + 1) * 4 + 16));
   const uint64_t smem_min = a->dbg_smem_cap ? a->dbg_smem_cap : n * 4 + (4u << 20);
   if (a->smem_cap < smem_min) a->smem_cap = smem_min;
   HIPCHK(a, a->s_smems.ensure(a->smem_cap * sizeof(SmemT<C>)));
   if (!a->dbg_smem_cap) a->smem_cap = std::max<uint64_t>(a->smem_cap, a->s_smems.cap / sizeof(SmemT<C>));
   HIPCHK(a, a->r_san.ensure(a->n_bases + 256 + 16));
-  HIPCHK(a, hipMemsetAsync(a->r_san.p, 0, 16, s));
-  HIPCHK(a, launch_sanitize(a->r_bases.as<uint8_t>(), a->r_san.as<uint8_t>() + 16, a->n_bases, a->n_bases + 128, s));
+  {
+    RunResetParams rp;
+    rp.ctl = a->d_ctl.as<uint4>();
+    rp.ctl_vec4 = (uint32_t)(thm_aligner::CTL_BYTES / 16);
+    rp.status = a->r_status.as<uint4>();
+    rp.status_vec4 = ((n + 1) * 4 + 15) / 16;
+    rp.san_head = a->r_san.as<uint4>();
+    rp.counters = a->d_counters.as<unsigned long long>();
+    HIPCHK(a, launch_sanitize_reset(a->r_bases.as<uint8_t>(), a->r_san.as<uint8_t>() + 16, a->n_bases, a->n_bases + 128, rp, s));
+  }
   uint64_t n_long = 0;
   uint32_t max_short = 0, max_long = 0;
   for (const auto& lc : a->len_hist) {
@@ -96,11 +103,6 @@
   HIPCHK(a, a->s_work_reads.ensure((n + 1) * 8));
   HIPCHK(a, a->s_work_long.ensure((n_long + 1) * 8));
   HIPCHK(a, a->s_work_cells.ensure((std::max(cells, n) + 1) * 8));
-  HIPCHK(a, a->s_work_counts.ensure(128));
-  HIPCHK(a, hipMemsetAsync(a->s_work_counts.p, 0, 128, s));
-  int rc = reset_queue(a);
-  if (rc != THM_OK) return rc;
-  HIPCHK(a, hipMemsetAsync(a->d_cursors.p, 0, 64, s));
   const int n_blocks = blocks_for(a, n, std::min(seed_select_lds_bytes(std::max(max_short, 1u)), SEED_SELECT_LDS_LIMIT));
   SeedParamsT<C> sp;
   sp.ix = dev_view<C>(a);
@@ -153,13 +155,33 @@
     sp.sel_scratch = a->s_sel_scratch.as<uint8_t>();
   }
   HIPCHK(a, launch_seed(sp, n_blocks, s));
-  HIPCHK(a, launch_exclusive_scan_u64(a->s_hits.as<uint64_t>(), a->s_cand_off.as<uint64_t>(), n,
-                                      a->scan_tmp.as<uint64_t>(), s));
-  return THM_OK;
-}
-
-int enqueue_seed(thm_aligner* a, uint32_t min_seed_len) {
-  return a->dix->wide ? enqueue_seed_t<uint64_t>(a, min_seed_len) : enqueue_seed_t<uint32_t>(a, min_seed_len);
+  if (finish_scan)
+    HIPCHK(a, launch_exclusive_scan_u64(a->s_hits.as<uint64_t>(), a->s_cand_off.as<uint64_t>(), n, a->scan_tmp.as<uint64_t>(), s));
+  else
+    HIPCHK(a, launch_scan_tiles_sums_u64(a->s_hits.as<uint64_t>(), a->s_cand_off.as<uint64_t>(), n, a->scan_tmp.as<uint64_t>(), s));
+  return THM_OK;
+}
+
+int enqueue_seed(thm_aligner* a, uint32_t min_seed_len, bool finish_scan) {
+  return a->dix->wide ? enqueue_seed_t<uint64_t>(a, min_seed_len, finish_scan) : enqueue_seed_t<uint32_t>(a, min_seed_len, finish_scan);
+}
+
+template <class C>
+int enqueue_plan_pack_t(thm_aligner* a, const PlanParams& pp) {
+  HIPCHK(a, a->e_recs.ensure((a->n_reads + 1) * sizeof(ReadRecT<C>)));
+  PackParamsT<C> pk;
+  pk.sa = dev_view<C>(a).sa;
+  pk.offsets = a->r_offsets.as<uint64_t>();
+  pk.n_reads = a->n_reads;
+  pk.smems = a->s_smems.as<SmemT<C>>();
+  pk.read_smem_off = a->s_off.as<uint64_t>();
+  pk.read_smem_cnt = a->s_cnt.as<uint32_t>();
+  pk.read_cand_off = a->s_cand_off.as<uint64_t>();
+  pk.tile_offs = a->scan_tmp.as<uint64_t>();
+  pk.fault_seed = a->d_fault.as<int>();
+  pk.recs = a->e_recs.as<ReadRecT<C>>();
+  HIPCHK(a, launch_plan_pack(pp, pk, a->stream));
+  return THM_OK;
 }
 
 struct ExtClasses {
@@ -201,20 +223,6 @@
   ep.reads.n_reads = n;
   ep.opts = a->opts;
   ep.smems = a->s_smems.as<SmemT<C>>();
-  HIPCHK(a, a->e_recs.ensure((n + 1) * sizeof(ReadRecT<C>)));
-  {
-    PackParamsT<C> pk;
-    pk.sa = ep.ix.sa;
-    pk.offsets = a->r_offsets.as<uint64_t>();
-    pk.n_reads = n;
-    pk.smems = ep.smems;
-    pk.read_smem_off = a->s_off.as<uint64_t>();
-    pk.read_smem_cnt = a->s_cnt.as<uint32_t>();
-    pk.read_cand_off = a->s_cand_off.as<uint64_t>();
-    pk.fault_seed = a->d_fault.as<int>();
-    pk.recs = a->e_recs.as<ReadRecT<C>>();
-    HIPCHK(a, launch_pack_reads(pk, s));
-  }
   ep.read_recs = a->e_recs.as<ReadRecT<C>>();
   ep.heavy = a->s_heavy.as<unsigned long long>();
   ep.heavy_count = a->s_work_counts.as<unsigned long long>() + 2;
@@ -234,7 +242,7 @@
   ep.retry_count = a->s_work_counts.as<unsigned long long>() + 5;
   ep.n_contract = a->s_work_counts.as<unsigned long long>() + 6;
   ep.counters = a->d_counters.as<unsigned long long>();
-  ep.queue = a->d_queue.as<unsigned int>();
+  ep.queue = a->d_queue_ext.as<unsigned int>();
   ep.fault = a->d_fault.as<int>() + 1;
   ep.fault_seed = a->d_fault.as<int>();
   ep.prof = a->d_counters.as<unsigned long long>() + 2 * THM_N_COUNTERS;
@@ -275,7 +283,8 @@
   const uint64_t tpr_rows = (uint64_t)ctl_blocks + (uint64_t)bail_blocks * 4;
   const uint64_t n_rows = main_rows + team_rows + slow_waves + tpr_rows;
   HIPCHK(a, a->e_wcnt.ensure(n_rows * THM_N_COUNTERS * 8 + 64));
-  HIPCHK(a, hipMemsetAsync(a->e_wcnt.p, 0, n_rows * THM_N_COUNTERS * 8, s));
+  if (a->wcnt_clean_cap != a->e_wcnt.cap) HIPCHK(a, hipMemsetAsync(a->e_wcnt.p, 0, a->e_wcnt.cap, s));
+  a->wcnt_clean_cap = 0;
   ep.wave_counters = a->e_wcnt.as<unsigned long long>();
   ep.skip_scan = 0;
   if (tpr) {
@@ -432,16 +441,15 @@
     HIPCHK(a, launch_extend(ep, 0, blocks, s));
   }
   HIPCHK(a, launch_counters_reduce(a->e_wcnt.as<unsigned long long>(), (uint32_t)n_rows, a->d_counters.as<unsigned long long>(), s));
+  a->wcnt_clean_cap = a->e_wcnt.cap;
   return THM_OK;
 }
 
 int enqueue_run(thm_aligner* a) {
   const uint64_t n = a->n_reads;
   hipStream_t s = a->stream;
-  HIPCHK(a, hipMemcpyAsync(a->d_counters.as<uint8_t>() + THM_N_COUNTERS * 8, a->d_counters.p, THM_N_COUNTERS * 8,
-                           hipMemcpyDeviceToDevice, s));
   HIPCHK(a, hipEventRecord(a->ev[0], s));
-  int rc = enqueue_seed(a, (uint32_t)a->opts.min_seed_len);
+  int rc = enqueue_seed(a, (uint32_t)a->opts.min_seed_len, false);
   if (rc != THM_OK) return rc;
   HIPCHK(a, hipEventRecord(a->ev[1], s));
 
@@ -455,7 +463,6 @@
   HIPCHK(a, a->e_rel.ensure(a->cand_cap * 4));
   HIPCHK(a, a->e_ops.ensure(a->cand_ops_cap + 64));
   HIPCHK(a, a->e_nalns.ensure((n + 1) * 4));
-  HIPCHK(a, a->e_nalns64.ensure((n + 1) * 8));
   HIPCHK(a, a->e_opbytes.ensure((n + 1) * 8));
   HIPCHK(a, a->e_aln_off.ensure((n + 2) * 8));
   HIPCHK(a, a->e_ops_off.ensure((n + 2) * 8));
@@ -464,7 +471,6 @@
   HIPCHK(a, a->s_heavy.ensure((n + 1) * 8));
   HIPCHK(a, a->s_slow.ensure((n + 1) * 8));
   HIPCHK(a, a->s_team.ensure((n + 1) * 8));
-  HIPCHK(a, hipMemsetAsync(a->d_queue.p, 0, thm::QUEUE_BYTES, s));
 
   const uint32_t mk_cap_slow = std::max<uint32_t>(a->ix->max_tx_exons, 1);
   const bool retry_possible = a->ix->max_tx_exons > (uint32_t)FAST_MAX_YCLIPS + 1;
@@ -492,7 +498,8 @@
   pp.read_status = a->r_status.as<int32_t>();
   pp.read_n_alns = a->e_nalns.as<uint32_t>();
   pp.read_op_bytes = a->e_opbytes.as<uint64_t>();
-  HIPCHK(a, launch_plan(pp, s));
+  rc = a->dix->wide ? enqueue_plan_pack_t<uint64_t>(a, pp) : enqueue_plan_pack_t<uint32_t>(a, pp);
+  if (rc != THM_OK) return rc;
   HIPCHK(a, hipEventRecord(a->ev[2], s));
 
   rc = a->dix->wide ? enqueue_extend_t<uint64_t>(a, cls, mk_cap_slow, retry_possible)
@@ -500,11 +507,8 @@
   if (rc != THM_OK) return rc;
   HIPCHK(a, hipEventRecord(a->ev[3], s));
 
-  HIPCHK(a, launch_widen_u32_to_u64(a->e_nalns.as<uint32_t>(), a->e_nalns64.as<uint64_t>(), n, s));
-  HIPCHK(a, launch_exclusive_scan_u64(a->e_nalns64.as<uint64_t>(), a->e_aln_off.as<uint64_t>(), n,
-                                      a->scan_tmp.as<uint64_t>(), s));
-  HIPCHK(a, launch_exclusive_scan_u64(a->e_opbytes.as<uint64_t>(), a->e_ops_off.as<uint64_t>(), n,
-                                      a->scan_tmp.as<uint64_t>(), s));
+  HIPCHK(a, launch_exclusive_scan2(a->e_nalns.as<uint32_t>(), a->e_opbytes.as<uint64_t>(), a->e_aln_off.as<uint64_t>(),
+                                   a->e_ops_off.as<uint64_t>(), n, a->scan_tmp.as<uint64_t>(), s));
   CompactParams cp;
   cp.n_reads = n;
   cp.read_cand_off = a->s_cand_off.as<uint64_t>();
@@ -732,13 +736,10 @@
   hipStream_t s = a->stream;
   RunStatus st;
   for (int attempt = 0;; attempt++) {
-    if (attempt == 0)
-      HIPCHK(a, hipMemcpyAsync(a->d_counters.as<uint8_t>() + THM_N_COUNTERS * 8, a->d_counters.p, THM_N_COUNTERS * 8,
-                               hipMemcpyDeviceToDevice, s));
-    else
+    if (attempt > 0)
       HIPCHK(a, hipMemcpyAsync(a->d_counters.p, a->d_counters.as<uint8_t>() + THM_N_COUNTERS * 8, THM_N_COUNTERS * 8,
                                hipMemcpyDeviceToDevice, s));
-    rc = enqueue_seed(a, (uint32_t)min_seed_len);
+    rc = enqueue_seed(a, (uint32_t)min_seed_len, true);
     if (rc != THM_OK) return rc;
     rc = read_status(a, &st);
     if (rc != THM_OK) return rc;
```

Result: faster. 89.58 million (median of 6 runs) (+1.7%).
